# irenemizus/ArtStyleTransfer

Hardware: AMD Instinct MI355X
Metric: style-transfer iters/sec at L=2 (1024-px) (higher is better)
Workload: dtype f32 via f16x2 split (3 f16 MFMAs per product, f32 accumulate; the 14 large-channel conv launches of a closure as Winograd F(2,3) in that arithmetic); 1 GPU; pyramid style transfer, levels_num=3 (1536x1024+768x512+384x256), lbfgs as the reference constructs it (max_eval 1 under torch 2.10), content+noise init, seeded synthetic VGG19 weights, per-step image yield on; parallelism=1 GPU

## Files before the change

### artstyletransfer_amd/_lib.py

```python
from __future__ import annotations

import ctypes as C
import os
import subprocess
import threading

_HERE = os.path.dirname(os.path.abspath(__file__))
LIB_PATH = os.environ.get("NST_LIB") or os.path.join(_HERE, "libnst_hip.so")
CSRC = os.path.join(_HERE, "csrc")

NST_OK = 0
NST_E_ARG = -1
NST_E_STATE = -2
NST_E_UNAVAILABLE = -5
NST_VGG19_CONVS = 13
NST_MAX_LEVELS = 8
NST_LOSS_ROW = 4
NST_MAX_STYLES = 8
NST_OPT_ADAM = 0
NST_OPT_LBFGS = 1
NST_COLOR_RGB = 0
NST_COLOR_LUMINANCE = 1
NST_POOL_MAX = 0
NST_POOL_AVG = 1
NST_MAX_LAPLACIAN = 4
NST_MAX_FLOW_SCALES = 12
NST_MAX_ANCHOR_SOURCES = 8

c_float_p = C.POINTER(C.c_float)
REDUCE_HOOK = C.CFUNCTYPE(None, C.c_void_p)
c_void = C.c_void_p


NST_CONV_F32, NST_CONV_BF16X3, NST_CONV_F16X2 = 0, 1, 2
CONV_MODES = {"f32": NST_CONV_F32, "bf16x3": NST_CONV_BF16X3, "f16x2": NST_CONV_F16X2}
NST_COMM_ID_BYTES = 128


class StepInfo(C.Structure):
    _fields_ = [("closures", C.c_int), ("total_closures", C.c_int), ("accepted", C.c_int),
                ("loss", C.c_float), ("lr", C.c_float), ("t", C.c_float), ("history", C.c_int)]


class Options(C.Structure):
    _fields_ = [("struct_size", C.c_int), ("conv_mode", C.c_int), ("batched", C.c_int), ("single_stream", C.c_int),
                ("use_graph", C.c_int), ("h2_band_rows", C.c_int), ("lbfgs_gram", C.c_int), ("h2_mfma16", C.c_int),
                ("h2_wg256", C.c_int), ("h2_tile_rows", C.c_int), ("gram_overlap", C.c_int), ("h2_persist", C.c_int), ("level_split", C.c_int), ("h2_winograd", C.c_int)]


class LaunchInfo(C.Structure):
    _fields_ = [(n, C.c_int) for n in ("cls", "h", "w", "cin", "cout", "layer", "h2_rows", "h2_bn", "h2_ntw", "h2_chunk",
                                       "h2_mfma16", "h2_persist", "h2_second", "h2_unpool", "h2_bands")]


SYMBOLS = {
    "nst_version": (C.c_int, []),
    "nst_last_error": (C.c_char_p, [c_void]),
    "nst_device_count": (C.c_int, [C.POINTER(C.c_int)]),
    "nst_ctx_create": (C.c_int, [C.c_int, C.POINTER(c_void), C.POINTER(c_void), C.POINTER(c_void)]),
    "nst_options_default": (None, [C.POINTER(Options)]),
    "nst_ctx_create_ex": (C.c_int, [C.c_int, C.POINTER(c_void), C.POINTER(c_void), C.POINTER(Options), C.POINTER(c_void)]),
    "nst_ctx_destroy": (None, [c_void]),
    "nst_job_configure": (C.c_int, [c_void, C.c_int, C.c_int, C.c_int]),
    "nst_job_set_taps": (C.c_int, [c_void, C.c_int, C.c_uint, C.c_int]),
    "nst_job_set_color": (C.c_int, [c_void, C.c_int]),
    "nst_job_color": (C.c_int, [c_void]),
    "nst_job_set_pooling": (C.c_int, [c_void, C.c_int]),
    "nst_job_pooling": (C.c_int, [c_void]),
    "nst_job_set_laplacian": (C.c_int, [c_void, C.c_int, C.POINTER(C.c_int), c_float_p]),
    "nst_job_laplacian": (C.c_int, [c_void, C.POINTER(C.c_int), C.POINTER(C.c_int), c_float_p]),
    "nst_job_laplacian_losses": (C.c_int, [c_void, c_void, c_void]),
    "nst_laplacian_loss": (C.c_int, [c_void, c_void, c_void, C.c_int, C.c_int, C.c_int, C.c_int, c_void, c_void, c_void]),
    "nst_job_set_matting": (C.c_int, [c_void, C.c_float, C.c_double]),
    "nst_job_matting": (C.c_int, [c_void, c_float_p, C.POINTER(C.c_double)]),
    "nst_job_matting_losses": (C.c_int, [c_void, c_void, c_void]),
    "nst_matting_loss": (C.c_int, [c_void, c_void, c_void, C.c_int, C.c_int, C.c_int, C.c_double, c_void, c_void, c_void]),
    "nst_level_set_anchor": (C.c_int, [c_void, C.c_int, c_void, c_void, C.c_float, c_void]),
    "nst_level_anchor": (C.c_int, [c_void, C.c_int, c_float_p, C.POINTER(C.c_int)]),
    "nst_job_temporal_losses": (C.c_int, [c_void, c_void, c_void]),
    "nst_anchor_loss": (C.c_int, [c_void, c_void, c_void, c_void, C.c_int, C.c_int, C.c_int, c_void, c_void, c_void]),
    "nst_anchor_geometry": (C.c_int, [C.POINTER(C.c_int), C.POINTER(C.c_int)]),
    "nst_level_set_patches": (C.c_int, [c_void, C.c_int, c_void, C.c_int, C.c_int, c_float_p, C.c_int, C.c_double, c_void]),
    "nst_level_patches": (C.c_int, [c_void, C.c_int, c_float_p, C.POINTER(C.c_int), C.POINTER(C.c_double)]),
    "nst_job_patch_losses": (C.c_int, [c_void, c_void, c_void]),
    "nst_level_patch_matches": (C.c_int, [c_void, C.c_int, C.c_int, c_void, c_void]),
    "nst_patch_match": (C.c_int, [c_void, c_void, C.c_int, C.c_int, C.c_int, c_void, C.c_int, C.c_int, C.c_int, C.c_double, c_void,
                                  c_void, c_void]),
    "nst_patch_term": (C.c_int, [c_void, c_void, C.c_int, C.c_int, C.c_int, c_void, C.c_int, C.c_int, C.c_int, c_void, C.c_float,
                                 c_void, c_void, c_void]),
    "nst_warp_bilinear": (C.c_int, [c_void, c_void, c_void, C.c_int, C.c_int, C.c_int, c_void, c_void, c_void]),
    "nst_flow_weights": (C.c_int, [c_void, c_void, c_void, C.c_int, C.c_int, c_void, c_void]),
    "nst_anchor_fold": (C.c_int, [c_void, C.c_int, C.POINTER(c_void), C.POINTER(c_void), C.c_int, C.c_int, C.c_int, c_void, c_void,
                                  c_void, c_void]),
    "nst_flow_workspace": (C.c_int, [C.c_int, C.c_int, C.c_int, C.POINTER(C.c_size_t), C.POINTER(C.c_int)]),
    "nst_flow_estimate": (C.c_int, [c_void, c_void, c_void, C.c_int, C.c_int, C.c_float, C.c_int, C.c_int, C.c_int, c_void, c_void,
                                    C.c_size_t, c_void]),
    "nst_flow_reduce": (C.c_int, [c_void, c_void, C.c_int, C.c_int, c_void, c_void]),
    "nst_flow_prolong": (C.c_int, [c_void, c_void, C.c_int, C.c_int, c_void, c_void]),
    "nst_flow_linearize": (C.c_int, [c_void, c_void, c_void, c_void, C.c_int, C.c_int, c_void, c_void, c_void, c_void]),
    "nst_flow_sweeps": (C.c_int, [c_void, c_void, c_void, c_void, c_void, C.c_int, C.c_int, C.c_float, C.c_int, c_void, c_void,
                                  c_void]),
    "nst_flow_tvl1_workspace": (C.c_int, [C.c_int, C.c_int, C.c_int, C.POINTER(C.c_size_t), C.POINTER(C.c_int)]),
    "nst_flow_tvl1_estimate": (C.c_int, [c_void, c_void, c_void, C.c_int, C.c_int, C.c_float, C.c_float, C.c_float, C.c_int, C.c_int,
                                         C.c_int, c_void, c_void, C.c_size_t, c_void]),
    "nst_flow_tvl1_iterations": (C.c_int, [c_void, c_void, c_void, c_void, c_void, c_void, C.c_int, C.c_int, C.c_float, C.c_float,
                                           C.c_float, C.c_int, c_void, c_void, c_void, c_void]),
    "nst_job_set_gram_shift": (C.c_int, [c_void, c_float_p, C.c_uint]),
    "nst_job_gram_shift": (C.c_int, [c_void, c_float_p, C.POINTER(C.c_uint)]),
    "nst_level_gram_offsets": (C.c_int, [c_void, C.c_int, C.c_int, c_void, c_void]),
    "nst_gram_shifted": (C.c_int, [c_void, c_void, C.c_int, C.c_int, C.c_int, C.c_int, C.c_int, C.c_float, c_void, c_void, c_void]),
    "nst_job_set_moments": (C.c_int, [c_void, c_float_p, c_float_p, C.c_float]),
    "nst_job_moments": (C.c_int, [c_void, c_float_p, c_float_p, c_float_p]),
    "nst_job_moment_losses": (C.c_int, [c_void, c_void, c_void]),
    "nst_moments": (C.c_int, [c_void, c_void, C.c_int, C.c_int, C.c_int, C.c_float, c_void, c_void, c_void]),
    "nst_job_set_style_weights": (C.c_int, [c_void, c_float_p]),
    "nst_job_style_weights": (C.c_int, [c_void, c_float_p]),
    "nst_color_stats": (C.c_int, [c_void, c_void, C.c_int, C.c_int, C.POINTER(C.c_double), C.POINTER(C.c_double), c_void]),
    "nst_color_transfer_matrix": (C.c_int, [C.POINTER(C.c_double)] * 6),
    "nst_color_affine": (C.c_int, [c_void, c_void, C.c_int, C.c_int, C.POINTER(C.c_double), C.POINTER(C.c_double), c_void, c_void]),
    "nst_luminance": (C.c_int, [c_void, c_void, C.c_int, C.c_int, C.c_double, C.c_double, c_void, c_void]),
    "nst_luminance_recombine": (C.c_int, [c_void, c_void, c_void, C.c_int, C.c_int, c_void, c_void]),
    "nst_level_set_targets": (C.c_int, [c_void, C.c_int, c_void, c_void, C.c_int, C.c_int, c_void]),
    "nst_level_set_targets_blend": (C.c_int, [c_void, C.c_int, c_void, C.c_int, C.POINTER(c_void), C.POINTER(C.c_int),
                                              C.POINTER(C.c_int), c_float_p, c_void]),
    "nst_level_set_guidance": (C.c_int, [c_void, C.c_int, C.c_int, c_void, c_float_p, c_void]),
    "nst_level_set_targets_guided": (C.c_int, [c_void, C.c_int, c_void, c_void, C.c_int, C.c_int, c_void, c_void]),
    "nst_level_guidance": (C.c_int, [c_void, C.c_int, C.POINTER(C.c_int), c_float_p, C.POINTER(C.c_double)]),
    "nst_level_guidance_planes": (C.c_int, [c_void, C.c_int, C.c_int, c_void, c_void]),
    "nst_closure": (C.c_int, [c_void, c_void, C.c_float, C.c_float, C.c_float, c_void, c_void, c_void]),
    "nst_closure_levels": (C.c_int, [c_void, c_void, C.c_float, C.c_float, C.c_float, C.c_uint, c_void, c_void, c_void]),
    "nst_closure_forward": (C.c_int, [c_void, c_void, C.c_float, C.c_float, C.c_float, C.c_uint, c_void, c_void]),
    "nst_closure_backward": (C.c_int, [c_void, c_void, C.c_float, C.c_float, C.c_float, C.c_uint, c_void, c_void]),
    "nst_opt_shard_levels": (C.c_int, [c_void, C.c_uint, c_void, c_void, c_void, c_void]),
    "nst_opt_shard_levels_comm": (C.c_int, [c_void, C.c_uint, c_void]),
    "nst_opt_history": (C.c_int, [c_void, C.POINTER(C.c_int), C.POINTER(C.c_int)]),
    "nst_opt_set_closure_reuse": (C.c_int, [c_void, C.c_int]),
    "nst_opt_closure_stats": (C.c_int, [c_void, C.POINTER(C.c_long), C.POINTER(C.c_long)]),
    "nst_opt_set_lazy_backward": (C.c_int, [c_void, C.c_int]),
    "nst_opt_backward_stats": (C.c_int, [c_void, C.POINTER(C.c_long), C.POINTER(C.c_long)]),
    "nst_comm_unique_id": (C.c_int, [c_void]),
    "nst_comm_create": (C.c_int, [C.c_int, C.c_int, C.c_int, c_void, C.POINTER(c_void)]),
    "nst_comm_destroy": (None, [c_void]),
    "nst_comm_info": (C.c_int, [c_void, C.POINTER(C.c_int), C.POINTER(C.c_int), C.POINTER(C.c_long), C.POINTER(C.c_double)]),
    "nst_comm_allreduce_sum": (C.c_int, [c_void, c_void, C.c_size_t, c_void]),
    "nst_adam_step": (C.c_int, [c_void, c_void, c_void, c_void, c_void, C.c_size_t, C.c_int, C.c_double, c_void]),
    "nst_lbfgs_direction": (C.c_int, [c_void, c_void, C.POINTER(c_void), C.POINTER(c_void), C.POINTER(C.c_float), C.c_int,
                                      C.c_float, C.c_size_t, C.c_int, c_void, c_void]),
    "nst_opt_create": (C.c_int, [c_void, C.c_int, C.c_float, C.c_int, C.POINTER(c_void)]),
    "nst_opt_destroy": (None, [c_void]),
    "nst_opt_step": (C.c_int, [c_void, c_void, C.c_float, C.c_float, C.c_float, c_void, C.c_int,
                               C.POINTER(StepInfo), c_void]),
    "nst_vgg_features": (C.c_int, [c_void, c_void, C.c_int, C.c_int, C.POINTER(c_void), c_void]),
    "nst_vgg_features_backward": (C.c_int, [c_void, c_void, C.c_int, C.c_int, C.POINTER(c_void), c_void, c_void]),
    "nst_vgg_activations": (C.c_int, [c_void, c_void, C.c_int, C.c_int, C.POINTER(c_void), c_void]),
    "nst_level_activation": (C.c_int, [c_void, C.c_int, C.c_int, c_void, c_void]),
    "nst_job_map_stats": (C.c_int, [c_void, C.c_int, C.POINTER(C.c_uint)]),
    "nst_ctx_set_keep_all_maps": (C.c_int, [c_void, C.c_int]),
    "nst_ctx_keep_all_maps": (C.c_int, [c_void]),
    "nst_ctx_set_forward_pack": (C.c_int, [c_void, C.c_int]),
    "nst_ctx_forward_pack": (C.c_int, [c_void]),
    "nst_ctx_set_gram_pack": (C.c_int, [c_void, C.c_int]),
    "nst_ctx_gram_pack": (C.c_int, [c_void]),
    "nst_level_image": (C.c_int, [c_void, C.c_int, c_void, c_void]),
    "nst_gram": (C.c_int, [c_void, c_void, C.c_int, C.c_int, C.c_int, C.c_int, c_void, c_void]),
    "nst_guided_gram_backward": (C.c_int, [c_void, c_void, C.c_size_t, C.c_int, C.c_int, c_void, c_void, c_void, c_void, c_void,
                                            c_void, c_void]),
    "nst_total_variation": (C.c_int, [c_void, c_void, C.c_int, C.c_int, C.c_int, c_void, c_void, c_void]),
    "nst_bicubic_half": (C.c_int, [c_void, c_void, C.c_int, C.c_int, C.c_int, c_void, c_void]),
    "nst_bicubic_half_backward": (C.c_int, [c_void, c_void, C.c_int, C.c_int, C.c_int, c_void, c_void]),
    "nst_prepare_img": (C.c_int, [c_void, c_void, C.c_int, C.c_int, c_void, c_void]),
    "nst_unprepare_img": (C.c_int, [c_void, c_void, C.c_int, C.c_int, c_void, c_void]),
    "nst_resize_bicubic": (C.c_int, [c_void, c_void, C.c_int, C.c_int, C.c_int, c_void, C.c_int, C.c_int, c_void]),
    "nst_gather_rows": (C.c_int, [c_void, c_void, c_void, C.c_size_t, C.c_int, c_void, c_void]),
    "nst_gaussian_mask_accumulate": (C.c_int, [c_void, c_void, c_void, C.c_int, C.c_int, C.c_int, C.c_double, C.c_double,
                                               C.c_double, c_void]),
    "nst_noise_blend": (C.c_int, [c_void, c_void, c_void, C.c_int, C.c_int, C.c_int, C.c_double, c_void, c_void]),
    "nst_scale": (C.c_int, [c_void, c_void, C.c_float, C.c_size_t, c_void, c_void]),
    "nst_window_sums_count": (C.c_int, [C.POINTER(C.c_size_t)]),
    "nst_window_begin": (C.c_int, [c_void, c_void, C.c_int, C.c_int, C.c_int, c_void, c_void]),
    "nst_window_end": (C.c_int, [c_void, c_void, C.c_int, C.c_int, C.c_int, C.c_float, C.c_float, C.c_float, c_void, c_void,
                                 c_void, c_void]),
    "nst_conv_mode": (C.c_int, [c_void]),
    "nst_ctx_bytes": (C.c_int, [c_void, C.POINTER(C.c_size_t)]),
    "nst_set_timing": (C.c_int, [c_void, C.c_int]),
    "nst_last_closure_ms": (C.c_int, [c_void, C.POINTER(C.c_float)]),
    "nst_last_closure_class": (C.c_int, [c_void, C.c_int, C.POINTER(C.c_float), C.POINTER(C.c_int),
                                         C.POINTER(C.c_double)]),
    "nst_last_closure_launches": (C.c_int, [c_void, C.POINTER(LaunchInfo), C.c_int, C.POINTER(C.c_int)]),
    "nst_last_closure_schedule": (C.c_int, [c_void, C.POINTER(C.c_int), C.POINTER(C.c_int), C.POINTER(C.c_int)]),
    "nst_dump_last_closure": (C.c_int, [c_void]),
    "nst_timing_totals": (C.c_int, [c_void, C.c_int, C.POINTER(C.c_double), C.POINTER(C.c_long),
                                    C.POINTER(C.c_double), C.c_int]),
    "nst_timing_mfma_flops": (C.c_int, [c_void, C.c_int, C.POINTER(C.c_double)]),
}

_lib = None
_lock = threading.Lock()


class NstError(RuntimeError):
    pass


def build(force: bool = False) -> str:
    if force:
        subprocess.run(["make", "-C", CSRC, "clean"], check=True, stdout=subprocess.DEVNULL)
    subprocess.run(["make", "-C", CSRC, "-j8"], check=True)
    return LIB_PATH


def load():
    global _lib
    with _lock:
        if _lib is not None:
            return _lib
        if not os.path.exists(LIB_PATH):
            raise NstError(
                f"{LIB_PATH} is missing: the HIP extension is the only implementation of the style-transfer "
                f"hot path (no CPU fallback). Build it with `python -c 'import __graft_entry__ as g; g.build()'` "
                f"or `make -C {CSRC}`.")
        try:
            lib = C.CDLL(LIB_PATH)
        except OSError as e:
            raise NstError(f"cannot load {LIB_PATH}: {e}") from e
        for name, (res, args) in SYMBOLS.items():
            try:
                fn = getattr(lib, name)
            except AttributeError as e:
                raise NstError(f"{LIB_PATH} does not export {name}; rebuild it") from e
            fn.restype = res
            fn.argtypes = args
        _lib = lib
        return lib


def check(ctx, code: int, what: str) -> None:
    if code != NST_OK:
        msg = load().nst_last_error(ctx)
        raise NstError(f"{what} failed ({code}): {msg.decode() if msg else '?'}")
```

### artstyletransfer_amd/csrc/conv_h2.hip

```cpp
#include <hip/hip_runtime.h>

#include <cstdlib>
#include <type_traits>

#include "nst_kernels.h"

namespace nst {

typedef float f32x4 __attribute__((ext_vector_type(4)));
typedef float f32x2 __attribute__((ext_vector_type(2)));
typedef float f32x16 __attribute__((ext_vector_type(16)));
typedef unsigned int u32x2 __attribute__((ext_vector_type(2)));
typedef unsigned int u32x4 __attribute__((ext_vector_type(4)));
typedef _Float16 f16x2 __attribute__((ext_vector_type(2)));
typedef _Float16 f16x8 __attribute__((ext_vector_type(8)));

namespace {

#ifndef NST_H2_DEEP_WEIGHT_PREFETCH
#define NST_H2_DEEP_WEIGHT_PREFETCH 1
#endif
#ifndef NST_H2_WEIGHT_SETS4
#define NST_H2_WEIGHT_SETS4 1
#endif
#ifndef NST_H2_ABLATE
#define NST_H2_ABLATE 0
#endif
constexpr unsigned ABL_IN = (NST_H2_ABLATE & 1) ? 0u : 1u, ABL_W = (NST_H2_ABLATE & 2) ? 0u : 1u, ABL_ST = (NST_H2_ABLATE & 4) ? 0u : 1u,
                   ABL_EL = (NST_H2_ABLATE & 8) ? 0u : 1u, ABL_G = (NST_H2_ABLATE & 16) ? 0u : 1u;
constexpr float LO_UP = 2048.f;
constexpr float LO_DOWN = 1.f / 2048.f;

template <int TH, int BN, int NTW, int KC_>
struct H2Cfg {
    static constexpr int KC = KC_;
    static constexpr int KS = KC / 16;
    static constexpr int QP = KC / 4;
    static constexpr int PIECEB = KC * 2;
    static constexpr int ROWB = 2 * PIECEB + 16;
    static constexpr int WROWB = 2 * PIECEB;
    static constexpr int TW = 16;
    static constexpr int PH = TH + 2, PW = TW + 2;
    static constexpr int WM = TH / 4;
    static constexpr int WN = BN / (32 * NTW);
    static constexpr int NT = 64 * WM * WN;
    static constexpr int A_UNITS = PH * PW * QP;
    static constexpr int A_PER_T = (A_UNITS + NT - 1) / NT;
    static constexpr int B_UNITS = BN * QP;
    static constexpr int B_PER_T = (B_UNITS + NT - 1) / NT;
    static constexpr int PROWB = ((PW * ROWB + 255) / 256) * 256;
    static constexpr int A_BYTES = PH * PROWB;
    static constexpr int B_BYTES = BN * ROWB;
    static constexpr int LDS_BYTES = 2 * A_BYTES + 3 * B_BYTES;
    static_assert(KC == 16 || KC == 32, "one or two k-steps per stage");
    static_assert(NT == 512 || NT == 256, "eight or four waves per workgroup");
    static_assert(B_UNITS % NT == 0, "every lane stages the same number of weight units (no predication)");
    static_assert(LDS_BYTES <= ((NT == 512 || TH == 4 || NTW == 4) ? 160 : 80) * 1024, "LDS budget (two 256-thread workgroups share a CU)");
    static constexpr int WAVES_PER_EU = (NTW == 4) ? 1 : 2;
};

__device__ __forceinline__ void tensor_scale(const unsigned* __restrict__ slots, int lane, float& s, float& inv) {
    unsigned m = slots[lane];
#pragma unroll
    for (int off = 32; off > 0; off >>= 1) {
        const unsigned o = (unsigned)__shfl_xor((int)m, off);
        m = o > m ? o : m;
    }
    int e = (int)((m >> 23) & 0xFFu);
    e = e < 32 ? 32 : (e > 250 ? 250 : e);
    s = __uint_as_float((unsigned)(268 - e) << 23);
    inv = __uint_as_float((unsigned)(e - 14) << 23);
}

__device__ __forceinline__ void cut2x4(const f32x4 v, const float s, u32x2& hi, u32x2& lo) {
    const f32x2 x01 = {v[0] * s, v[1] * s}, x23 = {v[2] * s, v[3] * s};
    const f16x2 h01 = __builtin_convertvector(x01, f16x2), h23 = __builtin_convertvector(x23, f16x2);
    const f32x2 b01 = __builtin_convertvector(h01, f32x2), b23 = __builtin_convertvector(h23, f32x2);
    const f32x2 r01 = (x01 - b01) * LO_UP, r23 = (x23 - b23) * LO_UP;
    const f16x2 l01 = __builtin_convertvector(r01, f16x2), l23 = __builtin_convertvector(r23, f16x2);
    hi = u32x2{__builtin_bit_cast(unsigned, h01), __builtin_bit_cast(unsigned, h23)};
    lo = u32x2{__builtin_bit_cast(unsigned, l01), __builtin_bit_cast(unsigned, l23)};
}

}

template <int TH, int BN, int NTW, int KC, bool UNPOOL, bool M16, class Tiles>
__device__ __forceinline__ void conv_h2_body(const Tiles& tiles, const int slot_seed) {
    static_assert(!M16 || KC == 32, "the 16x16x32 form takes a whole 32-channel chunk per MFMA");
    using C = H2Cfg<TH, BN, NTW, KC>;
    constexpr int ROWB = C::ROWB, WROWB = C::WROWB, QP = C::QP, PIECEB = C::PIECEB, KS = C::KS;
    extern __shared__ __attribute__((aligned(16))) unsigned char smem[];
    unsigned char* ldsB = smem;
    unsigned char* ldsA = smem + 3 * C::B_BYTES;

    const int tid = threadIdx.x;
    const int lane = tid & 63;
    const int wave = tid >> 6;
    const int wm = wave % C::WM;
    const int wn = wave / C::WM;
    const int half = lane >> 5;
    const int l31 = lane & 31;

    u32x4 rb[C::B_PER_T];
    constexpr bool DEEPB = (KC == 16) && NST_H2_DEEP_WEIGHT_PREFETCH;
    u32x4 rb2[DEEPB ? C::B_PER_T : 1];
    constexpr bool DEEPB4 = DEEPB && C::B_PER_T == 1 && NST_H2_WEIGHT_SETS4;
    u32x4 rb3[DEEPB4 ? C::B_PER_T : 1], rb4[DEEPB4 ? C::B_PER_T : 1];

    ConvParams p;
    int sp = 0, ct = 0;
    (void)tiles.get(0, p, sp, ct);
    bool primed = false;
  for (int tile_k = 0;; ++tile_k) {
    const int ty_rel = sp / p.tiles_x;
    const int tx = sp - ty_rel * p.tiles_x;
    const int ty = ty_rel + p.ty0;
    const int y0 = ty * TH;
    const int x0 = tx * C::TW;
    const int n0 = ct * BN;
    auto opaque_s = [](int v) { asm volatile("" : "+s"(v)); return v; };
    float nx_sa = 1.f;
    bool chain = false;
    {
        ConvParams pn;
        int spn = 0, ctn = 0;
        if (tiles.get(tile_k + 1, pn, spn, ctn) && p.Cin > 0 && !p.in2 && !pn.in2) {
            chain = true;
            float unused_inv;
            tensor_scale(pn.amax_in, lane, nx_sa, unused_inv);
        }
    }

    f32x4 ra[C::A_PER_T];

    auto a_lds_of = [&](int i, int to) -> int {
        const int u = to + i * C::NT;
        const int pix = u / QP;
        const int pr = pix / C::PW;
        const int pc = pix - pr * C::PW;
        return (u < C::A_UNITS) ? pr * C::PROWB + pc * ROWB + (u % QP) * 8 : -1;
    };
    auto a_voff_of = [&](int i, int to, int cin, const bool pooled, const int gH, const int gW, const int gy0, const int gx0) -> unsigned {
        const int u = to + i * C::NT;
        const int pix = u / QP;
        const int pr = pix / C::PW;
        const int pc = pix - pr * C::PW;
        const int gy = gy0 - 1 + pr;
        const int gx = gx0 - 1 + pc;
        bool ok = (u < C::A_UNITS) & ((unsigned)gy < (unsigned)gH) & ((unsigned)gx < (unsigned)gW);
        if (!pooled) return ok ? ((unsigned)(gy * gW + gx) * (unsigned)cin + (unsigned)(u % QP) * 4u) * 4u : 0xFFFFFF00u;
        const int PH2 = gH >> 1, PW2 = gW >> 1;
        ok = ok & ((gy >> 1) < PH2) & ((gx >> 1) < PW2);
        return ok ? ((unsigned)((gy >> 1) * PW2 + (gx >> 1)) * (unsigned)cin + (unsigned)(u % QP) * 4u) * 4u : 0xFFFFFF00u;
    };
    auto a_coff_of = [&](int i, int to, int cin, const int gH, const int gW, const int gy0, const int gx0) -> unsigned {
        const int u = to + i * C::NT;
        const int pix = u / QP;
        const int pr = pix / C::PW;
        const int pc = pix - pr * C::PW;
        const int gy = gy0 - 1 + pr;
        const int gx = gx0 - 1 + pc;
        const int PH2 = gH >> 1, PW2 = gW >> 1;
        const bool ok = (u < C::A_UNITS) & ((unsigned)gy < (unsigned)gH) & ((unsigned)gx < (unsigned)gW) &
                        ((gy >> 1) < PH2) & ((gx >> 1) < PW2);
        return ok ? (((unsigned)((gy >> 1) * PW2 + (gx >> 1)) * (unsigned)(cin >> 5)) * 4u + (unsigned)((gy & 1) * 2 + (gx & 1))) * 4u : 0xFFFFFF00u;
    };
    auto b_ok = [&](int, int) -> bool { return true; };
    auto b_lds_of = [&](int i, int to) -> int { const int u = to + i * C::NT; return (u / QP) * ROWB + (u % QP) * 16; };

    auto store_a = [&](unsigned char* dstA, const float s, const f32x4* r, const int i0, const int i1, const int to,
                       const unsigned* code = nullptr, const int bit0 = 0) {
#pragma unroll
        for (int i = i0; i < i1; ++i) {
            const int off = a_lds_of(i, to);
            if (off >= 0) {
                u32x2 hi, lo;
                f32x4 v = r[i - i0];
                if (code) {
                    const unsigned bits = code[i - i0] >> (bit0 + ((to + i * C::NT) % QP) * 4);
#pragma unroll
                    for (int k = 0; k < 4; ++k) v[k] = ((bits >> k) & 1u) ? v[k] : 0.f;
                }
                cut2x4(v, s, hi, lo);
                unsigned char* row = dstA + off;
                *reinterpret_cast<u32x2*>(row) = hi;
                *reinterpret_cast<u32x2*>(row + PIECEB) = lo;
            }
        }
    };
    auto store_b = [&](unsigned char* dst, const u32x4 (&r)[C::B_PER_T], const int to) {
#pragma unroll
        for (int i = 0; i < C::B_PER_T; ++i)
            if (b_ok(i, to)) *reinterpret_cast<u32x4*>(dst + b_lds_of(i, to)) = r[i];
    };
    auto store_b_f32 = [&](unsigned char* dst, const float s, const int to) {
#pragma unroll
        for (int i = 0; i < C::B_PER_T; ++i)
            if (b_ok(i, to)) {
                u32x2 hi, lo;
                cut2x4(__builtin_bit_cast(f32x4, rb[i]), s, hi, lo);
                const int u = to + i * C::NT;
                unsigned char* row = dst + (u / QP) * ROWB + (u % QP) * 8;
                *reinterpret_cast<u32x2*>(row) = hi;
                *reinterpret_cast<u32x2*>(row + PIECEB) = lo;
            }
    };
    auto opaque = [](int v) { asm volatile("" : "+v"(v)); return v; };

    f32x16 accm[2][NTW], accx[2][NTW];
#pragma unroll
    for (int a = 0; a < 2; ++a)
#pragma unroll
        for (int b = 0; b < NTW; ++b)
#pragma unroll
            for (int r = 0; r < 16; ++r) { accm[a][b][r] = 0.f; accx[a][b][r] = 0.f; }

    const int prow = wm * 4 + (l31 >> 4);
    const int pcol = l31 & 15;
    const int a_off0 = (prow + 0) * C::PROWB + pcol * ROWB + half * 16;
    const int a_off1 = (prow + 2) * C::PROWB + pcol * ROWB + half * 16;
    const int b_off0 = (wn * 32 * NTW + l31) * ROWB + half * 16;

    struct Frags { f16x8 a[2][2]; f16x8 b[NTW][2]; };
    auto request = [&](Frags& f, const unsigned char* abase, const unsigned char* bbase, const int ks) {
#pragma unroll
        for (int s = 0; s < 2; ++s) {
            f.a[0][s] = *reinterpret_cast<const f16x8*>(abase + a_off0 + s * PIECEB + ks * 32);
            f.a[1][s] = *reinterpret_cast<const f16x8*>(abase + a_off1 + s * PIECEB + ks * 32);
#pragma unroll
            for (int nt = 0; nt < NTW; ++nt)
                f.b[nt][s] = *reinterpret_cast<const f16x8*>(bbase + b_off0 + nt * 32 * ROWB + s * PIECEB + ks * 32);
        }
    };
    auto multiply = [&](const Frags& f) {
#pragma unroll
        for (int mt = 0; mt < 2; ++mt)
#pragma unroll
            for (int nt = 0; nt < NTW; ++nt) {
                accx[mt][nt] = __builtin_amdgcn_mfma_f32_32x32x16_f16(f.a[mt][1], f.b[nt][0], accx[mt][nt], 0, 0, 0);
                accm[mt][nt] = __builtin_amdgcn_mfma_f32_32x32x16_f16(f.a[mt][0], f.b[nt][0], accm[mt][nt], 0, 0, 0);
                accx[mt][nt] = __builtin_amdgcn_mfma_f32_32x32x16_f16(f.a[mt][0], f.b[nt][1], accx[mt][nt], 0, 0, 0);
            }
    };
    constexpr int READS = 4 + 2 * NTW, MFMAS = 6 * NTW;
    auto pin_kstep = [&]() {
#pragma unroll
// ... 40 lines not shown
#pragma unroll
                for (int j = 0; j < 2; ++j)
                    ax16[2 * mp + i][2 * np + j] = __builtin_amdgcn_mfma_f32_16x16x32_f16(a.v[i][1], b.v[j][0], ax16[2 * mp + i][2 * np + j], 0, 0, 0);
#pragma unroll
            for (int i = 0; i < 2; ++i)
#pragma unroll
                for (int j = 0; j < 2; ++j)
                    am16[2 * mp + i][2 * np + j] = __builtin_amdgcn_mfma_f32_16x16x32_f16(a.v[i][0], b.v[j][0], am16[2 * mp + i][2 * np + j], 0, 0, 0);
#pragma unroll
            for (int i = 0; i < 2; ++i)
#pragma unroll
                for (int j = 0; j < 2; ++j)
                    ax16[2 * mp + i][2 * np + j] = __builtin_amdgcn_mfma_f32_16x16x32_f16(a.v[i][0], b.v[j][1], ax16[2 * mp + i][2 * np + j], 0, 0, 0);
        }
    };
    auto pin_quad = [&](const int reads) {
        if (reads == 4) {
#pragma unroll
            for (int g = 0; g < 4; ++g) {
                __builtin_amdgcn_sched_group_barrier(0x008, 3, 0);
                __builtin_amdgcn_sched_group_barrier(0x100, 1, 0);
            }
        } else {
#pragma unroll
            for (int g = 0; g < 8; ++g) {
                __builtin_amdgcn_sched_group_barrier(0x008, 1, 0);
                __builtin_amdgcn_sched_group_barrier(0x100, 1, 0);
            }
            __builtin_amdgcn_sched_group_barrier(0x008, 4, 0);
        }
    };
    Pair RA[2], RB[2];

    auto gram_source = [&](const float* src, const int cin, const float* wts, const float sa, const float sw) {
        const int nch = cin / KC;
        const __amdgpu_buffer_rsrc_t rsrc_in = __builtin_amdgcn_make_buffer_rsrc(
            const_cast<float*>(src), 0, (unsigned)((size_t)p.H * p.W * cin * 4) * ABL_G, 0x00020000);
        const __amdgpu_buffer_rsrc_t rsrc_w = __builtin_amdgcn_make_buffer_rsrc(
            const_cast<float*>(wts), 0, (unsigned)((size_t)p.Cout * cin * 4) * ABL_G, 0x00020000);
        constexpr int G_PER_T = TH * C::TW * QP / C::NT;
        static_assert(TH * C::TW * QP % C::NT == 0 && G_PER_T <= C::A_PER_T, "centre units divide evenly");
        unsigned a_voff[G_PER_T], b_voff[C::B_PER_T];
        int g_lds[G_PER_T];
#pragma unroll
        for (int i = 0; i < G_PER_T; ++i) {
            const int u = tid + i * C::NT;
            const int pix = u / QP, q = u % QP;
            const int py = pix >> 4, px = pix & 15;
            const int gy = y0 + py, gx = x0 + px;
            bool ok = (gy < p.H) & (gx < p.W);
            if (p.in2_rows > 0) ok = ok & ((unsigned)(gy - p.in2_row0) < (unsigned)p.in2_rows);
            a_voff[i] = ok ? ((unsigned)(gy * p.W + gx) * (unsigned)cin + (unsigned)q * 4u) * 4u : 0xFFFFFF00u;
            g_lds[i] = (py + 1) * C::PROWB + (px + 1) * ROWB + q * 8;
        }
#pragma unroll
        for (int i = 0; i < C::B_PER_T; ++i) {
            const int u = tid + i * C::NT;
            b_voff[i] = b_ok(i, tid) ? (unsigned)(((u / QP) * cin + (u % QP) * 4) * 4) : 0xFFFFFF00u;
        }
        auto load = [&](int chunk) {
#pragma unroll
            for (int i = 0; i < G_PER_T; ++i)
                ra[i] = __builtin_bit_cast(f32x4, __builtin_amdgcn_raw_buffer_load_b128(rsrc_in, a_voff[i], chunk * KC * 4, 0));
#pragma unroll
            for (int i = 0; i < C::B_PER_T; ++i)
                rb[i] = __builtin_amdgcn_raw_buffer_load_b128(rsrc_w, b_voff[i], (n0 * cin + chunk * KC) * 4, 0);
        };
        auto store_centre = [&](unsigned char* dstA) {
#pragma unroll
            for (int i = 0; i < G_PER_T; ++i) {
                u32x2 hi, lo;
                cut2x4(ra[i], sa, hi, lo);
                unsigned char* row = dstA + g_lds[i];
                *reinterpret_cast<u32x2*>(row) = hi;
                *reinterpret_cast<u32x2*>(row + PIECEB) = lo;
            }
        };
        load(0);
        store_centre(ldsA);
        store_b_f32(ldsB, sw, tid);
        if (nch > 1) load(1);
        __syncthreads();
        for (int c = 0; c < nch; ++c) {
            const int cb = c & 1;
            if (c + 1 < nch) {
                store_centre(ldsA + (cb ^ 1) * C::A_BYTES);
                store_b_f32(ldsB + (cb ^ 1) * C::B_BYTES, sw, tid);
                if (c + 2 < nch) load(c + 2);
            }
            const unsigned char* centre = ldsA + cb * C::A_BYTES + C::PROWB + ROWB;
            const unsigned char* bcur = ldsB + cb * C::B_BYTES;
            if constexpr (M16) {
                read_a(RA[0], centre, 0);
                read_a(RA[1], centre, 1);
#pragma unroll
                for (int np = 0; np < NP; ++np) {
                    read_b(RB[0], bcur, np);
                    quad(RA[0], RB[0], 0, np);
                    quad(RA[1], RB[0], 1, np);
                }
            } else {
#pragma unroll
                for (int ks = 0; ks < KS; ++ks) request(F[ks], centre, bcur, ks);
#pragma unroll
                for (int ks = 0; ks < KS; ++ks) multiply(F[ks]);
            }
            __syncthreads();
        }
    };

    auto main_source = [&](const float* src, const int cin, const void* wts, const float sa) {
        const int nch = cin / KC;
        const size_t in_px = UNPOOL ? (size_t)(p.H >> 1) * (p.W >> 1) : (size_t)p.H * p.W;
        const __amdgpu_buffer_rsrc_t rsrc_in = __builtin_amdgcn_make_buffer_rsrc(
            const_cast<float*>(src), 0, (unsigned)(in_px * cin * 4) * ABL_IN, 0x00020000);
        const __amdgpu_buffer_rsrc_t rsrc_w = __builtin_amdgcn_make_buffer_rsrc(
            const_cast<void*>(wts), 0, (unsigned)((size_t)9 * p.Cout * nch * WROWB) * ABL_W, 0x00020000);
        const __amdgpu_buffer_rsrc_t rsrc_code = __builtin_amdgcn_make_buffer_rsrc(
            const_cast<unsigned*>(UNPOOL ? p.pcode_in : nullptr), 0, UNPOOL ? (unsigned)(in_px * (cin >> 5) * 16) : 0u, 0x00020000);
        struct Look { __amdgpu_buffer_rsrc_t rs_in, rs_code; int H, W, y0, x0, n0; float sa; };
        const Look here{rsrc_in, rsrc_code, p.H, p.W, y0, x0, n0, sa};
        auto there = [&]() -> Look {
            ConvParams pn;
            int spn = 0, ctn = 0;
            (void)tiles.get(opaque_s(tile_k + 1), pn, spn, ctn);
            const size_t px = UNPOOL ? (size_t)(pn.H >> 1) * (pn.W >> 1) : (size_t)pn.H * pn.W;
            const int tyn = spn / pn.tiles_x;
            return Look{__builtin_amdgcn_make_buffer_rsrc(const_cast<float*>(pn.in), 0, (unsigned)(px * cin * 4), 0x00020000),
                        __builtin_amdgcn_make_buffer_rsrc(const_cast<unsigned*>(UNPOOL ? pn.pcode_in : nullptr), 0,
                                                          UNPOOL ? (unsigned)(px * (cin >> 5) * 16) : 0u, 0x00020000),
                        pn.H, pn.W, (tyn + pn.ty0) * TH, (spn - tyn * pn.tiles_x) * C::TW, ctn * BN, nx_sa};
        };
        unsigned rc[UNPOOL ? C::A_PER_T : 1];
        auto load_a = [&](f32x4* r, const Look& k, int chunk, const int i0, const int i1, const int to) {
#pragma unroll
            for (int i = i0; i < i1; ++i) {
                r[i - i0] = __builtin_bit_cast(f32x4, __builtin_amdgcn_raw_buffer_load_b128(
                                                          k.rs_in, a_voff_of(i, to, cin, UNPOOL, k.H, k.W, k.y0, k.x0), chunk * KC * 4, 0));
                if (UNPOOL)
                    rc[i - i0] = __builtin_amdgcn_raw_buffer_load_b32(k.rs_code, a_coff_of(i, to, cin, k.H, k.W, k.y0, k.x0), ((chunk * KC) >> 5) * 16, 0);
            }
        };
        auto bit0_of = [&](int chunk) { return (chunk * KC) & 31; };
        auto load_b = [&](u32x4 (&r)[C::B_PER_T], int chunk, int tap, const int to, const int cout0) {
            const int soff = ((tap * p.Cout + cout0) * nch + chunk) * WROWB;
#pragma unroll
            for (int i = 0; i < C::B_PER_T; ++i) {
                const int u = to + i * C::NT;
                const unsigned voff = b_ok(i, to) ? (unsigned)((u / QP) * nch * WROWB + (u % QP) * 16) : 0xFFFFFF00u;
                r[i] = __builtin_amdgcn_raw_buffer_load_b128(rsrc_w, voff, soff, 0);
            }
        };
        auto tap_off = [](int t) { return (t / 3) * C::PROWB + (t % 3) * ROWB; };

        if (!primed) {
            u32x4 r0[C::B_PER_T], r1[C::B_PER_T];
            load_a(ra, here, 0, 0, C::A_PER_T, tid);
            load_b(r0, 0, 0, tid, n0);
            load_b(r1, 0, 1, tid, n0);
            load_b(rb, 0, 2, tid, n0);
            if constexpr (DEEPB) load_b(rb2, 0, 3, tid, n0);
            if constexpr (DEEPB4) { load_b(rb3, 0, 4, tid, n0); load_b(rb4, 0, 5, tid, n0); }
            __syncthreads();
            store_a(ldsA, sa, ra, 0, C::A_PER_T, tid, UNPOOL ? rc : nullptr, bit0_of(0));
            store_b(ldsB, r0, tid);
            store_b(ldsB + C::B_BYTES, r1, tid);
            __syncthreads();
        }
        if constexpr (M16) {
            read_a(RA[0], ldsA + tap_off(0), 0);
            read_b(RB[0], ldsB, 0);
        } else {
            request(F[0], ldsA + tap_off(0), ldsB, 0);
        }
        if (C::NT == 512 && __builtin_amdgcn_readfirstlane(threadIdx.x) >= 256) __builtin_amdgcn_s_setprio(1);

        auto chunk = [&](const int c, auto par_c) {
            constexpr int PAR = decltype(par_c)::value;
            unsigned char* acur = ldsA + (c & 1) * C::A_BYTES;
            unsigned char* anext = ldsA + ((c + 1) & 1) * C::A_BYTES;
            const bool last = (c + 1 >= nch);
            const int cn = last ? (chain ? 0 : c) : c + 1;
            Look ahead = here;
            if (last && chain) ahead = there();
            const int to = opaque(tid);
#ifndef NST_H2_THIRDS_ALL
#define NST_H2_THIRDS_ALL 0
#endif
            constexpr int PARTS = ((NST_H2_THIRDS_ALL || (M16 && NTW == 2)) && C::A_PER_T % 3 == 0) ? 3 : 2;
            constexpr int AP = (C::A_PER_T + PARTS - 1) / PARTS;
            auto part_lo = [](int j) { return j * AP < C::A_PER_T ? j * AP : C::A_PER_T; };
#pragma unroll
            for (int t = 0; t < 9; ++t) {
                if constexpr (DEEPB4) {
                    store_b(ldsB + ((t + 2) % 3) * C::B_BYTES, rb, to);
#pragma unroll
                    for (int i = 0; i < C::B_PER_T; ++i) { rb[i] = rb2[i]; rb2[i] = rb3[i]; rb3[i] = rb4[i]; }
                    if (t + 6 < 9) load_b(rb4, c, t + 6, to, n0);
                    else load_b(rb4, cn, t + 6 - 9, to, ahead.n0);
                } else if constexpr (DEEPB) {
                    if (((PAR + t) & 1) == 0) {
                        store_b(ldsB + ((t + 2) % 3) * C::B_BYTES, rb, to);
                        if (t + 4 < 9) load_b(rb, c, t + 4, to, n0);
                        else load_b(rb, cn, t + 4 - 9, to, ahead.n0);
                    } else {
                        store_b(ldsB + ((t + 2) % 3) * C::B_BYTES, rb2, to);
                        if (t + 4 < 9) load_b(rb2, c, t + 4, to, n0);
                        else load_b(rb2, cn, t + 4 - 9, to, ahead.n0);
                    }
                } else {
                    store_b(ldsB + ((t + 2) % 3) * C::B_BYTES, rb, to);
                    if (t + 3 < 9) load_b(rb, c, t + 3, to, n0);
                    else load_b(rb, cn, t + 3 - 9, to, ahead.n0);
                }
                if constexpr (PARTS == 2) {
                    if (t == 0) load_a(ra, ahead, cn, 0, AP, to);
                    if (t == 4) load_a(ra, ahead, cn, AP, C::A_PER_T, to);
                } else {
                    if (t % 3 == 0) load_a(ra, ahead, cn, part_lo(t / 3), part_lo(t / 3 + 1), to);
                }
                __builtin_amdgcn_sched_barrier(0);
                if constexpr (PARTS == 2) {
                    if (t == 3) store_a(anext, ahead.sa, ra, 0, AP, to, UNPOOL ? rc : nullptr, bit0_of(cn));
                    if (t == 7) store_a(anext, ahead.sa, ra, AP, C::A_PER_T, to, UNPOOL ? rc : nullptr, bit0_of(cn));
                } else {
                    if (t % 3 == 2) store_a(anext, ahead.sa, ra, part_lo(t / 3), part_lo(t / 3 + 1), to, UNPOOL ? rc : nullptr, bit0_of(cn));
                }
                const unsigned char* bcur = ldsB + (t % 3) * C::B_BYTES;
                const unsigned char* anxt = (t + 1 < 9) ? acur + tap_off(t + 1) : anext + tap_off(0);
                const unsigned char* bnxt = ldsB + ((t + 1) % 3) * C::B_BYTES;
                if constexpr (M16) {
                    const unsigned char* aptr = acur + tap_off(t);
                    const int sp_ = (PAR + t) & 1;
                    if (NP == 2) {
                        const int b0 = sp_, b1 = sp_ ^ 1;
                        read_b(RB[b1], bcur, b1);
                        quad(RA[0], RB[b0], 0, b0);
                        pin_quad(4);
                        read_a(RA[1], aptr, 1);
                        quad(RA[0], RB[b1], 0, b1);
                        pin_quad(4);
                        read_a(RA[0], anxt, 0);
                        quad(RA[1], RB[b1], 1, b1);
                        pin_quad(4);
                        read_b(RB[b1], bnxt, b1);
                        quad(RA[1], RB[b0], 1, b0);
                        pin_quad(4);
                    } else {
                        read_a(RA[1], aptr, 1);
                        quad(RA[0], RB[sp_], 0, 0);
                        pin_quad(4);
                        read_a(RA[0], anxt, 0);
                        read_b(RB[sp_ ^ 1], bnxt, 0);
                        quad(RA[1], RB[sp_], 1, 0);
                        pin_quad(8);
                    }
                } else if (KS == 2) {
                    request(F[1], acur + tap_off(t), bcur, 1);
                    multiply(F[0]);
                    pin_kstep();
                    request(F[0], anxt, bnxt, 0);
                    multiply(F[1]);
                    pin_kstep();
                } else {
                    const int cur = (PAR + t) & 1;
                    request(F[cur ^ 1], anxt, bnxt, 0);
                    multiply(F[cur]);
                    pin_kstep();
                }
                __syncthreads();
            }
        };
        if (KS == 2 && !M16) {
            for (int c = 0; c < nch; ++c) chunk(c, std::integral_constant<int, 0>{});
        } else {
            for (int c = 0; c < nch; c += 2) {
                chunk(c, std::integral_constant<int, 0>{});
                chunk(c + 1, std::integral_constant<int, 1>{});
            }
        }
    };

    const bool has_main = p.Cin > 0;
    float sa1 = 1.f, ia1 = 1.f;
    if (has_main) tensor_scale(p.amax_in, lane, sa1, ia1);
    const float w1_inv = has_main ? p.wt_h2_inv : 1.f;
    const float inv = ia1 * w1_inv;
    if (p.in2) {
        float sa2, ia2, sw2, iw2;
        tensor_scale(p.amax_in2, lane, sa2, ia2);
        tensor_scale(p.amax_w2, lane, sw2, iw2);
        gram_source(p.in2, p.Cin2, p.wt2_f32, sa2, sw2);
        const float ratio = (ia2 * sa1) * (iw2 * (1.f / w1_inv));
        if constexpr (M16) {
#pragma unroll
            for (int a = 0; a < 4; ++a)
#pragma unroll
                for (int b = 0; b < NT16; ++b)
#pragma unroll
                    for (int r = 0; r < 4; ++r) { am16[a][b][r] *= ratio; ax16[a][b][r] *= ratio; }
        } else {
#pragma unroll
            for (int a = 0; a < 2; ++a)
#pragma unroll
                for (int b = 0; b < NTW; ++b)
#pragma unroll
                    for (int r = 0; r < 16; ++r) { accm[a][b][r] *= ratio; accx[a][b][r] *= ratio; }
        }
    }
    if (has_main) main_source(p.in, p.Cin, p.wt_h2, sa1);

    auto epilogue = [&, &p_loop = p]() {
    ConvParams p;
    {
        int sp_again, ct_again;
        if (Tiles::REFETCH) (void)tiles.get(opaque_s(tile_k), p, sp_again, ct_again);
        else p = p_loop;
    }
    const int words = p.Cout >> 5;
    const bool avg = p.pool_avg != 0;
    float amax = 0.f;
    auto record_amax = [&]() {
        if (p.amax_out) {
#pragma unroll
            for (int off = 32; off > 0; off >>= 1) amax = fmaxf(amax, __shfl_xor(amax, off));
            if (lane == 0) atomicMax(p.amax_out + ((slot_seed * (C::NT / 64) + wave) & (NST_AMAX_SLOTS - 1)), __float_as_uint(amax));
        }
    };

    if constexpr (M16) {
        const int cg0 = n0 + wn * 32 * NTW;
        const float lo_clamp = p.relu ? 0.f : -__builtin_inff();
        auto word_of = [&](const unsigned long long b_even, const unsigned long long b_odd) -> unsigned {
            return (unsigned)((b_even >> (16 * kg)) & 0xFFFFull) | ((unsigned)((b_odd >> (16 * kg)) & 0xFFFFull) << 16);
        };
        const bool interior = (y0 + TH <= p.H) && (x0 + C::TW <= p.W);
        const bool fwd_like = !p.bits_in && !p.addend;
        const bool bwd_like = p.bits_in && !p.bits_out && !p.pool_out && !p.pcode_out;
        if (interior && !p.mask && (fwd_like || bwd_like) && (size_t)p.H * p.W * p.Cout * 4 < 0xFFFFFF00ull) {
            const unsigned out_bytes = (unsigned)((size_t)p.H * p.W * p.Cout * 4);
            const unsigned bit_bytes = (unsigned)((size_t)p.H * p.W * words * 4);
            const int colB = p.Cout * 4, rowB = p.W * colB;
            const int wcolB = words * 4, wrowB = p.W * wcolB;
            const int pix0 = (y0 + wm * 4) * p.W + x0 + 4 * kg;
            const unsigned vbase = (unsigned)pix0 * (unsigned)colB + (unsigned)(cg0 + l15) * 4u;
            const unsigned wbase = (unsigned)pix0 * (unsigned)wcolB + (unsigned)(cg0 >> 5) * 4u;
            const __amdgpu_buffer_rsrc_t rs_out = __builtin_amdgcn_make_buffer_rsrc(p.out, 0, out_bytes * ABL_ST, 0x00020000);
            if (bwd_like) {
                const __amdgpu_buffer_rsrc_t rs_bits = __builtin_amdgcn_make_buffer_rsrc(const_cast<unsigned*>(p.bits_in), 0, bit_bytes * ABL_EL, 0x00020000);
                const __amdgpu_buffer_rsrc_t rs_add = __builtin_amdgcn_make_buffer_rsrc(const_cast<float*>(p.addend), 0, p.addend ? out_bytes * ABL_EL : 0u, 0x00020000);
                unsigned wv[4][4][NTW];
#pragma unroll
                for (int mt = 0; mt < 4; ++mt)
#pragma unroll
                    for (int i = 0; i < 4; ++i) {
                        if (NTW == 2) {
                            const u32x2 w2 = __builtin_bit_cast(u32x2, __builtin_amdgcn_raw_buffer_load_b64(rs_bits, wbase, mt * wrowB + i * wcolB, 0));
                            wv[mt][i][0] = w2[0];
                            wv[mt][i][NTW - 1] = w2[1];
                        } else {
                            wv[mt][i][0] = __builtin_amdgcn_raw_buffer_load_b32(rs_bits, wbase, mt * wrowB + i * wcolB, 0);
                        }
                    }
#pragma unroll
                for (int nt = 0; nt < NT16; ++nt) {
                    const float bv = p.bias ? p.bias[cg0 + nt * 16 + l15] : 0.f;
#pragma unroll
                    for (int mt = 0; mt < 4; ++mt) {
                        float ad[4] = {0.f, 0.f, 0.f, 0.f};
                        if (p.addend) {
#pragma unroll
                            for (int i = 0; i < 4; ++i)
                                ad[i] = __builtin_bit_cast(float, __builtin_amdgcn_raw_buffer_load_b32(rs_add, vbase, mt * rowB + i * colB + nt * 64, 0));
                        }
#pragma unroll
                        for (int i = 0; i < 4; ++i) {
                            float v = fmaf(ax16[mt][nt][i], LO_DOWN, am16[mt][nt][i]) * inv + bv;
                            v = fmaxf(v + ad[i], lo_clamp);
                            v = ((wv[mt][i][nt >> 1] >> ((nt & 1) * 16 + l15)) & 1u) ? v : 0.f;
                            __builtin_amdgcn_raw_buffer_store_b32(__builtin_bit_cast(unsigned, v), rs_out, vbase, mt * rowB + i * colB + nt * 64, 0);
                            amax = fmaxf(amax, fabsf(v));
                        }
                    }
                }
            } else {
                const int PW2 = p.W >> 1;
                const unsigned pool_bytes = (unsigned)((size_t)(p.H >> 1) * PW2 * p.Cout * 4);
                const __amdgpu_buffer_rsrc_t rs_bits = __builtin_amdgcn_make_buffer_rsrc(p.bits_out, 0, p.bits_out ? bit_bytes * ABL_ST : 0u, 0x00020000);
                const __amdgpu_buffer_rsrc_t rs_pool = __builtin_amdgcn_make_buffer_rsrc(p.pool_out, 0, p.pool_out ? pool_bytes * ABL_ST : 0u, 0x00020000);
                const __amdgpu_buffer_rsrc_t rs_code = __builtin_amdgcn_make_buffer_rsrc(
                    p.pcode_out, 0, p.pcode_out ? (unsigned)((size_t)(p.H >> 1) * PW2 * words * 16) * ABL_ST : 0u, 0x00020000);
                const unsigned wlane = (l15 == 0) ? wbase : 0xFFFFFF00u;
                const int ppix0 = ((y0 + wm * 4) >> 1) * PW2 + ((x0 + 4 * kg) >> 1);
                const unsigned pbase = (unsigned)ppix0 * (unsigned)colB + (unsigned)(cg0 + l15) * 4u;
                const unsigned cbase = (l15 == 0) ? ((unsigned)ppix0 * (unsigned)words + (unsigned)(cg0 >> 5)) * 16u : 0xFFFFFF00u;
                const bool full = UNPOOL || p.out != nullptr;
#pragma unroll
                for (int nt = 0; nt < NT16; ++nt) {
                    const float bv = p.bias ? p.bias[cg0 + nt * 16 + l15] : 0.f;
#pragma unroll
                    for (int mt = 0; mt < 4; ++mt)
#pragma unroll
                        for (int i = 0; i < 4; ++i) {
                            float v = fmaf(ax16[mt][nt][i], LO_DOWN, am16[mt][nt][i]) * inv + bv;
                            v = fmaxf(v, lo_clamp);
                            am16[mt][nt][i] = v;
                            if (full) __builtin_amdgcn_raw_buffer_store_b32(__builtin_bit_cast(unsigned, v), rs_out, vbase, mt * rowB + i * colB + nt * 64, 0);
                            amax = fmaxf(amax, fabsf(v));
                        }
                }
                if (p.bits_out) {
#pragma unroll
                    for (int mt = 0; mt < 4; ++mt)
#pragma unroll
                        for (int i = 0; i < 4; ++i)
#pragma unroll
                            for (int w = 0; w < NTW; ++w) {
                                const unsigned long long b0 = __ballot(am16[mt][2 * w][i] > 0.f), b1 = __ballot(am16[mt][2 * w + 1][i] > 0.f);
                                __builtin_amdgcn_raw_buffer_store_b32(word_of(b0, b1), rs_bits, wlane, mt * wrowB + i * wcolB + w * 4, 0);
                            }
                }
                if (p.pool_out) {
#pragma unroll
                    for (int mt = 0; mt < 4; mt += 2)
#pragma unroll
                        for (int i = 0; i < 4; i += 2) {
                            const int poff = (mt >> 1) * PW2 + (i >> 1);
                            unsigned long long code[NTW][4][2];
#pragma unroll
                            for (int nt = 0; nt < NT16; ++nt) {
                                const float e0 = am16[mt][nt][i], e1 = am16[mt][nt][i + 1], e2 = am16[mt + 1][nt][i], e3 = am16[mt + 1][nt][i + 1];
                                const float mx = avg ? (((e0 + e1) + e2) + e3) * 0.25f : fmaxf(fmaxf(e0, e1), fmaxf(e2, e3));
                                __builtin_amdgcn_raw_buffer_store_b32(__builtin_bit_cast(unsigned, mx), rs_pool, pbase, poff * colB + nt * 64, 0);
                                if (p.pcode_out) {
                                    if (avg) {
                                        code[nt >> 1][0][nt & 1] = __ballot(e0 > 0.f);
                                        code[nt >> 1][1][nt & 1] = __ballot(e1 > 0.f);
                                        code[nt >> 1][2][nt & 1] = __ballot(e2 > 0.f);
                                        code[nt >> 1][3][nt & 1] = __ballot(e3 > 0.f);
                                    } else {
                                        int pos = 0;
// ... 206 lines not shown
                        accm[mt][nt][r] = v;
                        if (full) __builtin_amdgcn_raw_buffer_store_b32(__builtin_bit_cast(unsigned, v), rs_out, vbase, soff(mt, r, rowB, colB) + nt * 128, 0);
                        amax = fmaxf(amax, fabsf(v));
                        if (p.bits_out) {
                            const unsigned long long bal = __ballot(v > 0.f);
                            __builtin_amdgcn_raw_buffer_store_b32(half ? (unsigned)(bal >> 32) : (unsigned)bal, rs_bits, wlane,
                                                                  soff(mt, r, wrowB, wcolB) + nt * 4, 0);
                        }
                    }
                    if (p.pool_out) {
#pragma unroll
                        for (int j = 0; j < 4; ++j) {
                            const int r = 2 * j;
                            const int pcol = (j & 1) + 4 * (j >> 1);
                            const float mx = avg ? (((accm[mt][nt][r] + accm[mt][nt][r + 1]) + accm[mt][nt][r + 8]) + accm[mt][nt][r + 9]) * 0.25f
                                                 : fmaxf(fmaxf(accm[mt][nt][r], accm[mt][nt][r + 1]),
                                                         fmaxf(accm[mt][nt][r + 8], accm[mt][nt][r + 9]));
                            __builtin_amdgcn_raw_buffer_store_b32(__builtin_bit_cast(unsigned, mx), rs_pool, pbase,
                                                                  (mt * PW2 + pcol) * colB + nt * 128, 0);
                            if (p.pcode_out) {
                                int pos = 0;
                                float best = accm[mt][nt][r];
                                if (accm[mt][nt][r + 1] > best) { best = accm[mt][nt][r + 1]; pos = 1; }
                                if (accm[mt][nt][r + 8] > best) { best = accm[mt][nt][r + 8]; pos = 2; }
                                if (accm[mt][nt][r + 9] > best) { best = accm[mt][nt][r + 9]; pos = 3; }
                                const bool live = best > 0.f;
                                constexpr int roff[4] = {0, 1, 8, 9};
#pragma unroll
                                for (int q = 0; q < 4; ++q) {
                                    const unsigned long long bal = __ballot(avg ? accm[mt][nt][r + roff[q]] > 0.f : (live && pos == q));
                                    __builtin_amdgcn_raw_buffer_store_b32(half ? (unsigned)(bal >> 32) : (unsigned)bal, rs_code, cbase,
                                                                          ((mt * PW2 + pcol) * words + nt) * 16 + q * 4, 0);
                                }
                            }
                        }
                    }
                }
            }
        }
        record_amax();
        return;
    }

#pragma unroll
    for (int nt = 0; nt < NTW; ++nt) {
        const int co = n0 + wn * 32 * NTW + nt * 32 + l31;
        const int cw = (n0 + wn * 32 * NTW + nt * 32) >> 5;
        const float bv = p.bias ? p.bias[co] : 0.f;
#pragma unroll
        for (int mt = 0; mt < 2; ++mt) {
#pragma unroll
            for (int r = 0; r < 16; ++r) {
                const int m = (r & 3) + 8 * (r >> 2) + 4 * half;
                const int y = y0 + wm * 4 + mt * 2 + (m >> 4);
                const int x = x0 + (m & 15);
                const bool inb = (y < p.H && x < p.W);
                const size_t pix = (size_t)y * p.W + x;
                const size_t idx = pix * p.Cout + co;
                float v = fmaf(accx[mt][nt][r], LO_DOWN, accm[mt][nt][r]) * inv + bv;
                if (p.addend && inb) v += p.addend[idx];
                if (p.relu) v = fmaxf(v, 0.f);
                if (p.bits_in) {
                    const unsigned wv = inb ? p.bits_in[pix * words + cw] : 0u;
                    v = ((wv >> l31) & 1u) ? v : 0.f;
                } else if (p.mask) {
                    v = (inb && p.mask[idx] > 0.f) ? v : 0.f;
                }
                if (p.bits_out) {
                    const unsigned long long bal = __ballot(v > 0.f);
                    if (l31 == 0 && inb) p.bits_out[pix * words + cw] = half ? (unsigned)(bal >> 32) : (unsigned)bal;
                }
                accm[mt][nt][r] = v;
                if (inb) {
                    if (UNPOOL || p.out) p.out[idx] = v;
                    amax = fmaxf(amax, fabsf(v));
                }
            }
            if (p.pool_out) {
                const int py = (y0 + wm * 4 + mt * 2) >> 1;
                const int PH2 = p.H >> 1, PW2 = p.W >> 1;
#pragma unroll
                for (int j = 0; j < 4; ++j) {
                    const int r = 2 * j;
                    const float mx = avg ? (((accm[mt][nt][r] + accm[mt][nt][r + 1]) + accm[mt][nt][r + 8]) + accm[mt][nt][r + 9]) * 0.25f
                                         : fmaxf(fmaxf(accm[mt][nt][r], accm[mt][nt][r + 1]),
                                                 fmaxf(accm[mt][nt][r + 8], accm[mt][nt][r + 9]));
                    const int mcol = (r & 3) + 8 * (r >> 2) + 4 * half;
                    const int px = (x0 + mcol) >> 1;
                    const bool inw = (py < PH2 && px < PW2);
                    if (inw) p.pool_out[((size_t)py * PW2 + px) * p.Cout + co] = mx;
                    if (p.pcode_out) {
                        int pos = 0;
                        float best = accm[mt][nt][r];
                        if (accm[mt][nt][r + 1] > best) { best = accm[mt][nt][r + 1]; pos = 1; }
                        if (accm[mt][nt][r + 8] > best) { best = accm[mt][nt][r + 8]; pos = 2; }
                        if (accm[mt][nt][r + 9] > best) { best = accm[mt][nt][r + 9]; pos = 3; }
                        const bool live = best > 0.f;
                        constexpr int roff[4] = {0, 1, 8, 9};
#pragma unroll
                        for (int q = 0; q < 4; ++q) {
                            const unsigned long long bal = __ballot(avg ? accm[mt][nt][r + roff[q]] > 0.f : (live && pos == q));
                            if (l31 == 0 && inw)
                                p.pcode_out[(((size_t)py * PW2 + px) * words + cw) * 4 + q] = half ? (unsigned)(bal >> 32) : (unsigned)bal;
                        }
                    }
                }
            }
        }
    }
    record_amax();
    };
    epilogue();
    if (!tiles.get(tile_k + 1, p, sp, ct)) break;
    primed = chain;
  }
}

__device__ __forceinline__ int xcd_contiguous(const int b, const int grid) {
#ifdef NST_NO_XCD_MAP
    return b;
#else
    const int x = b & 7, k = b >> 3;
    const int q = grid >> 3, r = grid & 7;
    return x * q + (x < r ? x : r) + k;
#endif
}

template <bool PERSIST>
struct H2BatchTiles {
    static constexpr bool REFETCH = PERSIST;
    const ConvBatch& b;
    int n_ct;
    __device__ __forceinline__ bool get(const int k, ConvParams& p, int& sp, int& ct) const {
        int t;
        if (!PERSIST) {
            if (k > 0) return false;
            t = xcd_contiguous((int)blockIdx.x, (int)gridDim.x);
        } else {
            const int x = (int)blockIdx.x & 7, j = ((int)blockIdx.x >> 3) + k * ((int)gridDim.x >> 3);
            const int q = b.total_tiles >> 3, r = b.total_tiles & 7;
            if (j >= q + (x < r ? 1 : 0)) return false;
            t = x * q + (x < r ? x : r) + j;
        }
        const int sp_all = t / n_ct;
        ct = t - sp_all * n_ct;
        int i = 0;
        while (i + 1 < b.n && sp_all >= b.img[i].tile_end) ++i;
        const ConvImage& im = b.img[i];
        p.in = im.in; p.wt = nullptr; p.wt_bf = nullptr; p.bias = im.bias ? im.bias : b.bias; p.addend = im.addend; p.mask = im.mask; p.out = im.out;
        p.H = im.H; p.W = im.W; p.Cin = b.Cin; p.Cout = b.Cout; p.relu = b.relu;
        p.tiles_x = im.tiles_x; p.tiles_y = 0; p.partial = nullptr; p.partial_floats = 0; p.ksplit = 1;
        p.in2 = im.in2; p.Cin2 = b.Cin2; p.wt2_bf = nullptr; p.bits_out = im.bits_out; p.bits_in = im.bits_in;
        p.pool_out = im.pool_out;
        p.wt_h2 = b.wt_h2; p.wt_h2_inv = b.wt_h2_inv; p.wt2_f32 = im.wt2_f32;
        p.amax_in = im.amax_in; p.amax_in2 = im.amax_in2; p.amax_w2 = im.amax_w2; p.amax_out = im.amax_out;
        p.pcode_in = im.pcode_in; p.pcode_out = im.pcode_out; p.pool_avg = b.pool_avg;
        p.in2_row0 = im.in2_row0; p.in2_rows = im.in2_rows; p.ty0 = im.ty0;
        sp = sp_all - (i ? b.img[i - 1].tile_end : 0);
        return true;
    }
};

template <int TH, int BN, int NTW, int KC, bool UNPOOL, bool M16, bool PERSIST>
__global__ __launch_bounds__((H2Cfg<TH, BN, NTW, KC>::NT), (H2Cfg<TH, BN, NTW, KC>::WAVES_PER_EU)) void conv_h2_batch_kernel(ConvBatch b) {
    conv_h2_body<TH, BN, NTW, KC, UNPOOL, M16>(H2BatchTiles<PERSIST>{b, b.Cout / BN}, blockIdx.x);
}
template <int TH, int BN, int NTW, int KC>
constexpr bool h2_persist_shape = (KC == 16) || (TH == 16 && NTW == 2 && KC == 32);
template <int NTW, int KC>
constexpr bool h2_m16_built = (KC == 32 && NTW <= 2);

template <int TH, int BN, int NTW, int KC, bool UNPOOL, bool M16>
static hipError_t init_form() {
    constexpr int lds = H2Cfg<TH, BN, NTW, KC>::LDS_BYTES;
    hipError_t e = hipFuncSetAttribute(reinterpret_cast<const void*>(&conv_h2_batch_kernel<TH, BN, NTW, KC, UNPOOL, M16, false>),
                                       hipFuncAttributeMaxDynamicSharedMemorySize, lds);
    if constexpr (h2_persist_shape<TH, BN, NTW, KC> && !M16) {
        if (e == hipSuccess)
            e = hipFuncSetAttribute(reinterpret_cast<const void*>(&conv_h2_batch_kernel<TH, BN, NTW, KC, UNPOOL, false, true>),
                                    hipFuncAttributeMaxDynamicSharedMemorySize, lds);
    }
    return e;
}
template <int TH, int BN, int NTW, int KC, bool UNPOOL>
static hipError_t init_one() {
    hipError_t e = init_form<TH, BN, NTW, KC, UNPOOL, false>();
    if constexpr (h2_m16_built<NTW, KC>) {
        if (e == hipSuccess) e = init_form<TH, BN, NTW, KC, UNPOOL, true>();
    }
    return e;
}

hipError_t conv_h2_init_device() {
    hipError_t e = init_one<16, 128, 2, 32, false>();
    if (e == hipSuccess) e = init_one<8, 128, 1, 32, false>();
    if (e == hipSuccess) e = init_one<16, 64, 2, 16, false>();
    if (e == hipSuccess) e = init_one<16, 128, 2, 32, true>();
    if (e == hipSuccess) e = init_one<8, 128, 1, 32, true>();
    if (e == hipSuccess) e = init_one<16, 64, 2, 16, true>();
    if (e == hipSuccess) e = init_one<8, 128, 2, 16, false>();
    if (e == hipSuccess) e = init_one<8, 128, 2, 16, true>();
    if (e == hipSuccess) e = init_one<4, 128, 1, 32, false>();
    if (e == hipSuccess) e = init_one<4, 128, 1, 32, true>();
    if (e == hipSuccess) e = init_one<16, 128, 4, 32, false>();
    if (e == hipSuccess) e = init_one<16, 128, 4, 32, true>();
    return e;
}

static int h2_tile_rows(int Cout, long blocks16, int forced = 0) {
    if (Cout % 128 != 0) return 16;
    if (forced == 4 || forced == 8 || forced == 16) return forced;
    if (blocks16 < 100) return 4;
    return blocks16 < 400 ? 8 : 16;
}

static bool h2_use_m16(int mfma16, int th, int ntw, bool unpool) {
    if (mfma16 >= 3) return true;
    if (mfma16 == 2) return th == 8 || (th == 16 && ntw == 2 && !unpool);
    return mfma16 == 1 && th == 8;
}
static int h2_resident(const H2Shape& sh) { return 256 * ((sh.chunk == 16 || sh.rows == 4) ? 2 : 1); }

static H2Shape h2_launch_shape(const int* H, const int* W, int n, int Cin, int Cout, bool unpool, bool second, int tile_rows,
                               int mfma16, int wg256, int persist_opt, int* blocks) {
    H2Shape sh{};
    const bool wide = (Cout % 128 == 0);
    long blocks16 = 0;
    for (int i = 0; i < n; ++i) blocks16 += (long)((H[i] + 15) / 16) * ((W[i] + 15) / 16) * (Cout / 128);
    const bool shortk = wide && Cin > 0 && Cin <= NST_H2_SHORTK_CIN;
    sh.rows = shortk ? 8 : h2_tile_rows(Cout, blocks16, tile_rows);
    sh.bn = wide ? 128 : 64;
    sh.chunk = (!wide || shortk) ? 16 : 32;
    sh.ntw = (sh.chunk == 16) ? 2 : (sh.rows < 16 ? 1 : (wg256 ? 4 : 2));
    sh.m16 = (sh.chunk == 32 && sh.ntw <= 2 && h2_use_m16(mfma16, sh.rows, sh.ntw, unpool)) ? 1 : 0;
    sh.second = second ? 1 : 0;
    sh.unpool = unpool ? 1 : 0;
    sh.bands = 1;
    int tiles = 0;
    for (int i = 0; i < n; ++i) tiles += ((W[i] + 15) / 16) * ((H[i] + sh.rows - 1) / sh.rows);
    *blocks = tiles * (Cout / sh.bn);
    const bool pshape = sh.chunk == 16 || (sh.rows == 16 && sh.ntw == 2);
    sh.persist = (persist_opt && !second && Cin > 0 && *blocks > h2_resident(sh) && pshape && !sh.m16) ? 1 : 0;
    return sh;
}

template <int TH, int BN, int NTW, int KC>
static void launch_batch_cfg(const ConvBatch& b, const H2Shape& sh, int blocks, hipStream_t stream) {
    constexpr int lds = H2Cfg<TH, BN, NTW, KC>::LDS_BYTES;
    constexpr int nt = H2Cfg<TH, BN, NTW, KC>::NT;
    if constexpr (h2_m16_built<NTW, KC>) {
        if (sh.m16) {
            if (b.unpool) hipLaunchKernelGGL((conv_h2_batch_kernel<TH, BN, NTW, KC, true, true, false>), dim3(blocks), dim3(nt), lds, stream, b);
            else hipLaunchKernelGGL((conv_h2_batch_kernel<TH, BN, NTW, KC, false, true, false>), dim3(blocks), dim3(nt), lds, stream, b);
            return;
        }
    }
    if constexpr (h2_persist_shape<TH, BN, NTW, KC>) {
        if (sh.persist) {
            if (b.unpool) hipLaunchKernelGGL((conv_h2_batch_kernel<TH, BN, NTW, KC, true, false, true>), dim3(blocks), dim3(nt), lds, stream, b);
            else hipLaunchKernelGGL((conv_h2_batch_kernel<TH, BN, NTW, KC, false, false, true>), dim3(blocks), dim3(nt), lds, stream, b);
            return;
        }
    }
    if (b.unpool) hipLaunchKernelGGL((conv_h2_batch_kernel<TH, BN, NTW, KC, true, false, false>), dim3(blocks), dim3(nt), lds, stream, b);
    else hipLaunchKernelGGL((conv_h2_batch_kernel<TH, BN, NTW, KC, false, false, false>), dim3(blocks), dim3(nt), lds, stream, b);
}
static bool h2_operands_ok(const void* wt, const unsigned* amax_in, int Cin, int Cout, const float* in2, const float* wt2,
                           const unsigned* a2, const unsigned* w2, int Cin2) {
    if (Cin % 32 != 0 || Cout % 64 != 0) return false;
    if (Cin > 0 ? (!wt || !amax_in) : !in2) return false;
    if (in2 && (!wt2 || !a2 || !w2 || Cin2 % 32 != 0 || Cin2 != Cout)) return false;
    return true;
}

template <int TH, int BN, int NTW, int KC>
struct H2Tag { static constexpr int th = TH, bn = BN, ntw = NTW, kc = KC; };
template <typename Launch>
static void h2_dispatch(const H2Shape& sh, Launch&& go) {
    if (sh.bn == 64) go(H2Tag<16, 64, 2, 16>{});
    else if (sh.chunk == 16) go(H2Tag<8, 128, 2, 16>{});
    else if (sh.rows == 4) go(H2Tag<4, 128, 1, 32>{});
    else if (sh.rows == 8) go(H2Tag<8, 128, 1, 32>{});
    else if (sh.ntw == 4) go(H2Tag<16, 128, 4, 32>{});
    else go(H2Tag<16, 128, 2, 32>{});
}

hipError_t launch_conv_h2_batch(const ConvBatch& b0, hipStream_t stream, H2Shape* shape) {
    if (b0.n < 1 || b0.n > 8) return hipErrorInvalidValue;
    ConvBatch b = b0;
    int H[8], W[8];
    bool second = false;
    for (int i = 0; i < b.n; ++i) {
        const ConvImage& im = b.img[i];
        if (!h2_operands_ok(b.wt_h2, im.amax_in, b.Cin, b.Cout, im.in2, im.wt2_f32, im.amax_in2, im.amax_w2, b.Cin2))
            return hipErrorInvalidValue;
        if ((size_t)im.H * im.W * (b.Cin > b.Cin2 ? b.Cin : b.Cin2) * 4 >= 0xFFFFFF00ull) return hipErrorInvalidValue;
        if ((b.unpool != 0) != (im.pcode_in != nullptr)) return hipErrorInvalidValue;
        if (!im.out && !im.pool_out) return hipErrorInvalidValue;
        H[i] = im.H; W[i] = im.W;
        second = second || (im.in2 != nullptr);
    }
    int blocks = 0;
    const H2Shape sh = h2_launch_shape(H, W, b.n, b.Cin, b.Cout, b.unpool != 0, second, b.tile_rows, b.mfma16, b.wg256, b.persist, &blocks);
    int tiles = 0;
    for (int i = 0; i < b.n; ++i) {
        b.img[i].tiles_x = (b.img[i].W + 15) / 16;
        b.img[i].ty0 = 0;
        tiles += b.img[i].tiles_x * ((b.img[i].H + sh.rows - 1) / sh.rows);
        b.img[i].tile_end = tiles;
    }
    b.total_tiles = blocks;
    b.persist = sh.persist;
    if (sh.persist) blocks = h2_resident(sh);
    if (shape) *shape = sh;
    h2_dispatch(sh, [&](auto cfg) { launch_batch_cfg<decltype(cfg)::th, decltype(cfg)::bn, decltype(cfg)::ntw, decltype(cfg)::kc>(b, sh, blocks, stream); });
    return hipGetLastError();
}

hipError_t launch_conv_h2(const ConvParams& p, hipStream_t stream, H2Shape* shape) {
    if (!h2_operands_ok(p.wt_h2, p.amax_in, p.Cin, p.Cout, p.in2, p.wt2_f32, p.amax_in2, p.amax_w2, p.Cin2))
        return hipErrorInvalidValue;
    if (!p.out && !p.pool_out) return hipErrorInvalidValue;
    int all_blocks = 0;
    H2Shape sh = h2_launch_shape(&p.H, &p.W, 1, p.Cin, p.Cout, p.pcode_in != nullptr, p.in2 != nullptr, p.tile_rows, p.mfma16, p.wg256, 0, &all_blocks);
    const int th = sh.rows;
    const int cmax = p.Cin > p.Cout ? (p.Cin > p.Cin2 ? p.Cin : p.Cin2) : (p.Cout > p.Cin2 ? p.Cout : p.Cin2);
    const size_t row_bytes = (size_t)p.W * cmax * 4;
    int band_rows = p.H;
    if ((size_t)p.H * row_bytes >= 0xFFFFFF00ull) {
        const long fit = (long)(0xFFFFFF00ull / row_bytes) - 32;
        band_rows = (int)(fit / 16) * 16;
        if (band_rows < 16) return hipErrorInvalidValue;
    }
    const int forced_band = p.band_rows;
    if (forced_band >= 16 && forced_band / 16 * 16 < band_rows) band_rows = forced_band / 16 * 16;
    const int PW2 = p.W >> 1, wi = p.Cin >> 5, wo = p.Cout >> 5;
    ConvBatch b{};
    b.n = 1;
    b.bias = p.bias;
    b.Cin = p.Cin; b.Cout = p.Cout; b.Cin2 = p.Cin2; b.relu = p.relu;
    b.wt_h2 = p.wt_h2; b.wt_h2_inv = p.wt_h2_inv;
    b.unpool = (p.pcode_in != nullptr);
    b.persist = 0;
    b.pool_avg = p.pool_avg;
    int bands = 0;
    for (int r0 = 0; r0 < p.H; r0 += band_rows) {
        const int r1 = (r0 + band_rows < p.H) ? r0 + band_rows : p.H;
        const int b0 = (r0 >= 16) ? r0 - 16 : 0, b1 = (r1 + 16 < p.H) ? r1 + 16 : p.H;
        const size_t px0 = (size_t)b0 * p.W, pp0 = (size_t)(b0 >> 1) * PW2;
        ConvImage& q = b.img[0];
        q = ConvImage{};
        if (p.pcode_in) { q.in = p.in + pp0 * p.Cin; q.pcode_in = p.pcode_in + pp0 * wi * 4; }
        else if (p.in) q.in = p.in + px0 * p.Cin;
        q.in2_row0 = p.in2_row0; q.in2_rows = p.in2_rows;
        if (p.in2) { q.in2 = p.in2 + px0 * p.Cin2; if (q.in2_rows > 0) q.in2_row0 -= b0; }
        if (p.out) q.out = p.out + px0 * p.Cout;
        if (p.addend) q.addend = p.addend + px0 * p.Cout;
        if (p.mask) q.mask = p.mask + px0 * p.Cout;
        if (p.bits_in) q.bits_in = p.bits_in + px0 * wo;
        if (p.bits_out) q.bits_out = p.bits_out + px0 * wo;
        if (p.pool_out) q.pool_out = p.pool_out + pp0 * p.Cout;
        if (p.pcode_out) q.pcode_out = p.pcode_out + pp0 * wo * 4;
        q.wt2_f32 = p.wt2_f32;
        q.amax_in = p.amax_in; q.amax_in2 = p.amax_in2; q.amax_w2 = p.amax_w2; q.amax_out = p.amax_out;
        q.H = b1 - b0; q.W = p.W;
        q.ty0 = (r0 - b0) / th;
        const int tiles_y = (r1 - r0 + th - 1) / th;
        q.tiles_x = (p.W + 15) / 16;
        q.tile_end = q.tiles_x * tiles_y;
        const int blocks = q.tile_end * (p.Cout / sh.bn);
        b.total_tiles = blocks;
        h2_dispatch(sh, [&](auto cfg) { launch_batch_cfg<decltype(cfg)::th, decltype(cfg)::bn, decltype(cfg)::ntw, decltype(cfg)::kc>(b, sh, blocks, stream); });
        const hipError_t e = hipGetLastError();
        if (e != hipSuccess) return e;
        ++bands;
    }
    sh.bands = bands;
    if (shape) *shape = sh;
    return hipSuccess;
}

__global__ __launch_bounds__(256) void absmax_slots_kernel(const float* __restrict__ x, size_t n, unsigned* __restrict__ slots) {
    float m = 0.f;
    const size_t n4 = n / 4;
    for (size_t i = (size_t)blockIdx.x * blockDim.x + threadIdx.x; i < n4; i += (size_t)gridDim.x * blockDim.x) {
        const f32x4 v = reinterpret_cast<const f32x4*>(x)[i];
        m = fmaxf(fmaxf(m, fmaxf(fabsf(v[0]), fabsf(v[1]))), fmaxf(fabsf(v[2]), fabsf(v[3])));
    }
    if (blockIdx.x == 0 && threadIdx.x < (n & 3)) m = fmaxf(m, fabsf(x[n4 * 4 + threadIdx.x]));
#pragma unroll
    for (int off = 32; off > 0; off >>= 1) m = fmaxf(m, __shfl_xor(m, off));
    if ((threadIdx.x & 63) == 0)
        atomicMax(slots + ((blockIdx.x * 4 + (threadIdx.x >> 6)) & (NST_AMAX_SLOTS - 1)), __float_as_uint(m));
}
hipError_t launch_absmax_slots(const float* x, size_t n, unsigned* slots, hipStream_t stream) {
    size_t blocks = (n / 4 + 255) / 256;
    if (blocks > 1024) blocks = 1024;
    if (blocks < 1) blocks = 1;
    hipLaunchKernelGGL(absmax_slots_kernel, dim3((unsigned)blocks), dim3(256), 0, stream, x, n, slots);
    return hipGetLastError();
}

}
```

### artstyletransfer_amd/csrc/nst_closure.cpp

```cpp
#include <algorithm>
#include <cmath>
#include <cstring>

#include "nst_ctx.h"

using namespace nst;

namespace {

double conv_flops(int h, int w, int cin, int cout, int taps) { return 2.0 * h * w * (double)cin * cout * taps; }

bool uses_pieces(const nst_ctx* ctx, const ConvParams& p) {
    if (ctx->conv_mode == 2) return true;
    return ctx->conv_mode != 0 && (size_t)p.H * p.W * p.Cin * 4 < 0xFFFFFF00ull;
}
hipError_t launch_conv3(nst_ctx* ctx, const ConvParams& p, Timer& t) {
    hipStream_t s = t.s;
    if (uses_pieces(ctx, p)) {
        if (ctx->conv_mode != 2) return launch_conv_bf3(p, s);
        H2Shape sh{};
        const hipError_t e = launch_conv_h2(p, s, &sh);
        t.shape(sh);
        return e;
    }
    hipError_t e = launch_conv_mfma(p, 9, s);
    if (e == hipSuccess && ctx->conv_mode == 2 && p.amax_out)
        e = launch_absmax_slots(p.out, (size_t)p.H * p.W * p.Cout, p.amax_out, s);
    return e;
}
bool bf3_unsplit(const nst_ctx* ctx, const ConvParams& p) {
    if (!uses_pieces(ctx, p)) return false;
    if (ctx->conv_mode == 2) return true;
    const int S = conv_bf3_ksplit(p.H, p.W, p.Cin, p.Cout);
    return !(p.partial && S > 1 && (size_t)S * p.H * p.W * p.Cout <= p.partial_floats);
}

void conv_setup(const nst_ctx* ctx, ConvParams& p, const ActSet& a, int l, bool dgrad) {
    p.wt = dgrad ? ctx->wd[l] : ctx->wf[l]; p.wt_bf = dgrad ? ctx->wd_bf[l] : ctx->wf_bf[l];
    p.partial = a.splitk; p.partial_floats = a.splitk_floats;
    if (ctx->conv_mode != 2) return;
    p.wt_h2 = dgrad ? ctx->wd_h2[l] : ctx->wf_h2[l]; p.wt_h2_inv = dgrad ? ctx->wd_h2_inv[l] : ctx->wf_h2_inv[l];
    p.band_rows = ctx->band_rows; p.mfma16 = ctx->mfma16; p.wg256 = ctx->wg256; p.tile_rows = ctx->tile_rows;
}
void conv_setup(const nst_ctx* ctx, ConvBatch& b, int l, bool dgrad) {
    b.mfma16 = ctx->mfma16; b.wg256 = ctx->wg256; b.tile_rows = ctx->tile_rows; b.persist = ctx->persist;
    if (l < 1) { b.wt_h2_inv = 1.f; return; }
    b.wt_bf = dgrad ? ctx->wd_bf[l] : ctx->wf_bf[l];
    b.wt_h2 = dgrad ? ctx->wd_h2[l] : ctx->wf_h2[l]; b.wt_h2_inv = dgrad ? ctx->wd_h2_inv[l] : ctx->wf_h2_inv[l];
    b.wt_wino = dgrad ? ctx->wd_wino[l] : ctx->wf_wino[l]; b.wt_wino_inv = dgrad ? ctx->wd_wino_inv[l] : ctx->wf_wino_inv[l];
}
int launch_conv_batch(nst_ctx* ctx, const ConvBatch& b, hipStream_t s, Timer* t, bool allow_wino) {
    const bool h2 = ctx->conv_mode == 2;
    if (h2 && allow_wino && b.wt_wino && conv_wino_eligible(b)) { if (t) t->mfma_factor(2.0); HIPCHK(ctx, launch_conv_wino_batch(b, s)); }
    else if (h2) {
        H2Shape sh{};
        const hipError_t e = launch_conv_h2_batch(b, s, &sh);
        if (t) t->shape(sh);
        HIPCHK(ctx, e);
    } else HIPCHK(ctx, launch_conv_bf3_batch(b, s));
    return NST_OK;
}
int launch_conv_batch(nst_ctx* ctx, const ConvBatch& b, Timer& t, bool allow_wino) { return launch_conv_batch(ctx, b, t.s, &t, allow_wino); }

hipError_t launch_pool_fwd(const nst_ctx* ctx, const float* in, int H, int W, int C, float* out, hipStream_t s) {
    return (ctx->pool_avg ? launch_avgpool_fwd : launch_maxpool_fwd)(in, H, W, C, out, s);
}
hipError_t launch_pool_bwd_relu(const nst_ctx* ctx, const float* a, const float* gpool, int H, int W, int C, float* gin, hipStream_t s) {
    return (ctx->pool_avg ? launch_avgpool_bwd_relu : launch_maxpool_bwd_relu)(a, gpool, H, W, C, gin, s);
}

struct StyleTerm { int C; size_t N; double divisor; float coef; };
StyleTerm style_term(const Taps& tp, int q, const ActSet& a, float sw, float w, int norm_rows = 0) {
    const int l = tp.style[q], C = kCout[l];
    const size_t N = (size_t)(norm_rows > 0 ? norm_rows >> kScale[l] : a.h[l]) * a.w[l];
    const double chw = (double)C * (double)N;
    return {C, N, chw, (float)((double)sw * (double)w * 4.0 / ((double)tp.nstyle * (double)C * C * chw))};
}
float content_coef(float cw, double n) { return (float)((double)cw * 2.0 / n); }

constexpr bool taps_avoid_pools() {
    for (int t : kTapLayer)
        for (int p : kPoolAfter) if (t == p) return false;
    return true;
}
static_assert(taps_avoid_pools(), "a map in front of a pooling layer became a tap: map_stored must keep it where a job reads it");
bool map_stored(const nst_ctx* ctx, int l) {
    if (ctx->conv_mode != 2 || ctx->keep_all_maps || ctx->use_graph) return true;
    return pool_index_after(l) < 0;
}

size_t gram_part_offset(const Taps& tp, int h, int w, int k) {
    size_t off = 0;
    for (int q = 0; q < k; ++q) {
        const int l = tp.style[q];
        const size_t N = (size_t)(h >> kScale[l]) * (w >> kScale[l]);
        off += (size_t)gram_nsplit(kCout[l], N) * kCout[l] * kCout[l];
    }
    return off;
}

StyleTerm guided_term(const Taps& tp, int q, const ActSet& a, float sw, float w, const Guidance& g, int r) {
    const int l = tp.style[q], C = kCout[l];
    const size_t N = (size_t)a.h[l] * a.w[l];
    const double cn = (double)C * g.mass[kScale[l]][r];
    return {C, N, cn, (float)((double)sw * (double)w * (double)g.lambda[r] * 4.0 / ((double)tp.nstyle * (double)C * C * cn))};
}
bool guided_levels(const nst_ctx* ctx, const int* lv, int n) { return n > 0 && ctx->lv[lv[0]].guide.R > 0; }
GuidedBwd guided_bwd_of(const nst_ctx* ctx, const LevelWs& L, int q) {
    const int l = ctx->taps.style[q], C = kCout[l];
    GuidedBwd gb{};
    gb.R = L.guide.R; gb.C = C; gb.N = (size_t)L.acts.h[l] * L.acts.w[l]; gb.F = L.acts.act[l];
    for (int r = 0; r < gb.R; ++r) {
        gb.t[r] = L.guide.plane(kScale[l], r, L.h, L.w);
        gb.S[r] = L.guide.S[q] + (size_t)r * C * C;
    }
    return gb;
}
int launch_guided_backward(nst_ctx* ctx, const GuidedBwd& gb, hipStream_t s) {
    Timer t(ctx, s, K_GRAM, 2.0 * (double)gb.N * gb.C * gb.C * gb.R);
    HIPCHK(ctx, launch_guided_bwd(gb, s));
    return NST_OK;
}
int guided_fold(nst_ctx* ctx, LevelWs& L, int q, hipStream_t s) {
    Timer t(ctx, s, K_OTHER, 0);
    HIPCHK(ctx, launch_guided_fold(L.guide.partial[q], L.guide.R, gram_finish_blocks(kCout[ctx->taps.style[q]]), L.guide.lambda,
                                   L.style_partial[q], s));
    return NST_OK;
}

int lap_forward(nst_ctx* ctx, LevelWs& L, const float* y, bool as_target, hipStream_t s) {
    for (int k = 0; k < ctx->lap_k; ++k) {
        const int p = ctx->lap_pool[k];
        {
            Timer t(ctx, s, K_OTHER, 0);
            HIPCHK(ctx, launch_lap_pool(y, ctx->channels, L.h, L.w, p, L.lap.s[k], s));
        }
        Timer t(ctx, s, K_OTHER, 0);
        if (as_target) HIPCHK(ctx, launch_lap_stencil(L.lap.s[k], L.h / p, L.w / p, nullptr, L.lap.target[k], nullptr, nullptr, s));
        else HIPCHK(ctx, launch_lap_stencil(L.lap.s[k], L.h / p, L.w / p, L.lap.target[k], nullptr, L.lap.r[k], L.lap.partial[k], s));
    }
    return NST_OK;
}
double lap_n(const LevelWs& L, int p) { return (double)(L.h / p - 2) * (double)(L.w / p - 2); }
float lap_coef(float gamma, double n, int p, int channels) {
    return (float)((double)gamma * 2.0 * (channels == 1 ? 3.0 : 1.0) / (n * (double)p * (double)p));
}
int lap_backward(nst_ctx* ctx, LevelWs& L, float* grad, hipStream_t s) {
    if (ctx->lap_k < 1) return NST_OK;
    LapBackward lb{};
    lb.K = ctx->lap_k;
    for (int k = 0; k < lb.K; ++k) {
        lb.p[k] = ctx->lap_pool[k];
        lb.coef[k] = lap_coef(ctx->lap_gamma[k], lap_n(L, lb.p[k]), lb.p[k], ctx->channels);
        lb.r[k] = L.lap.r[k];
    }
    Timer t(ctx, s, K_OTHER, 0);
    HIPCHK(ctx, launch_lap_backward(lb, ctx->channels, L.h, L.w, grad, 1, s));
    return NST_OK;
}

double mat_n(const nst_ctx* ctx, const LevelWs& L) { return (ctx->channels == 1 ? 1.0 : 3.0) * (double)(L.h - 2) * (double)(L.w - 2); }
float mat_coef(float gamma, double n) { return (float)((double)gamma * 2.0 / (255.0 * n)); }
int mat_forward(nst_ctx* ctx, LevelWs& L, const float* y, hipStream_t s) {
    if (!(ctx->mat_gamma > 0.f)) return NST_OK;
    Timer t(ctx, s, K_OTHER, 0);
    HIPCHK(ctx, launch_mat_forward(y, L.mat.guide, ctx->channels, L.h, L.w, 1.0 / 255.0, ctx->mat_eps, L.mat.partial, s));
    return NST_OK;
}
int mat_backward(nst_ctx* ctx, LevelWs& L, const float* y, float* grad, hipStream_t s) {
    if (!(ctx->mat_gamma > 0.f)) return NST_OK;
    Timer t(ctx, s, K_OTHER, 0);
    HIPCHK(ctx, launch_mat_backward(y, L.mat.guide, ctx->channels, L.h, L.w, 1.0 / 255.0, ctx->mat_eps,
                                    mat_coef(ctx->mat_gamma, mat_n(ctx, L)), grad, 1, s));
    return NST_OK;
}
int mat_set_guide(nst_ctx* ctx, LevelWs& L, const float* content, hipStream_t s) {
    if (!(ctx->mat_gamma > 0.f)) return NST_OK;
    HIPCHK(ctx, hipMemcpyAsync(L.mat.guide, content, (size_t)ctx->channels * L.h * L.w * sizeof(float), hipMemcpyDeviceToDevice, s));
    return NST_OK;
}

double anchor_n(const nst_ctx* ctx, const LevelWs& L) { return (double)ctx->channels * (double)L.h * (double)L.w; }
float anchor_coef(float gamma, double n) { return (float)((double)gamma * 2.0 / n); }
int anchor_forward(nst_ctx* ctx, LevelWs& L, const float* y, hipStream_t s) {
    if (!(L.anc.gamma > 0.f)) return NST_OK;
    Timer t(ctx, s, K_OTHER, 0);
    HIPCHK(ctx, launch_anchor_forward(y, L.anc.anchor, L.anc.weights, ctx->channels, L.h, L.w, L.anc.partial, s));
    return NST_OK;
}
int anchor_backward(nst_ctx* ctx, LevelWs& L, const float* y, float* grad, hipStream_t s) {
    if (!(L.anc.gamma > 0.f)) return NST_OK;
    Timer t(ctx, s, K_OTHER, 0);
    HIPCHK(ctx, launch_anchor_backward(y, L.anc.anchor, L.anc.weights, ctx->channels, L.h, L.w,
                                       anchor_coef(L.anc.gamma, anchor_n(ctx, L)), grad, 1, s));
    return NST_OK;
}

PatchTerm patch_term_of(const LevelWs& L, int i) {
    const int l = kTapLayer[i];
    return PatchTerm{L.acts.act[l], L.acts.h[l], L.acts.w[l], L.pm.nn[i], L.pm.d[i]};
}
double patch_denom(const LevelWs& L, int i) {
    const int l = kTapLayer[i];
    return 9.0 * (double)kCout[l] * (double)(L.acts.h[l] - 2) * (double)(L.acts.w[l] - 2);
}
float patch_coef(float w, double denom) { return (float)((double)w * 2.0 / denom); }
int patch_forward(nst_ctx* ctx, LevelWs& L, hipStream_t s) {
    for (int i = 0; i < 6 && L.pm.on(); ++i) {
        if (!(L.pm.w[i] > 0.f)) continue;
        const int l = kTapLayer[i];
// ... 1389 lines not shown
```

### artstyletransfer_amd/csrc/nst_ctx.cpp

```cpp
#include <algorithm>
#include <atomic>
#include <climits>
#include <cmath>
#include <cstdint>
#include <cstdio>
#include <cstdlib>
#include <cstring>

#include "nst_ctx.h"

using namespace nst;

namespace {
thread_local std::string g_err;
}

int nst::fail(nst_ctx* ctx, int code, const std::string& msg) {
    if (ctx) ctx->err = msg; else g_err = msg;
    return code;
}

namespace nst {

void poison_if_asked(void* p, size_t bytes) {
    static const char* spec = getenv("NST_POISON_ALLOC");
    static std::atomic<long> seq{0};
    if (!spec || !*spec) return;
    const long k = seq++;
    long lo = 0, hi = -1;
    if (strcmp(spec, "all") == 0) hi = LONG_MAX;
    else if (sscanf(spec, "%ld-%ld", &lo, &hi) != 2) return;
    if (k >= lo && k <= hi) { (void)hipMemset(p, 0xFF, bytes); (void)hipStreamSynchronize(nullptr); }
    if (getenv("NST_POISON_TRACE")) fprintf(stderr, "nst alloc #%ld: %zu bytes%s\n", k, bytes, (k >= lo && k <= hi) ? " (poisoned)" : "");
}
int zero_now(void* p, size_t bytes) {
    hipStream_t zs = nullptr;
    hipError_t e = hipStreamCreateWithFlags(&zs, hipStreamNonBlocking);
    if (e != hipSuccess) return 1;
    e = hipMemsetAsync(p, 0, bytes, zs);
    if (e == hipSuccess) e = hipStreamSynchronize(zs);
    (void)hipStreamDestroy(zs);
    return e == hipSuccess ? 0 : 1;
}

int dev_alloc(nst_ctx* ctx, void** p, size_t bytes, size_t* charged) {
    if (bytes == 0) bytes = 16;
    hipError_t e = hipMalloc(p, bytes);
    if (e != hipSuccess) return fail(ctx, NST_E_NOMEM, std::string("hipMalloc(") + std::to_string(bytes) + "): " + hipGetErrorString(e));
    poison_if_asked(*p, bytes);
    ctx->bytes += bytes;
    if (charged) *charged = bytes;
    return NST_OK;
}
void dev_release(nst_ctx* ctx, void* p, size_t bytes) {
    (void)hipFree(p);
    ctx->bytes -= bytes;
}

int alloc_acts(nst_ctx* ctx, ActSet& a, int h, int w) {
    for (int l = 0; l < NL; ++l) {
        a.h[l] = h >> kScale[l];
        a.w[l] = w >> kScale[l];
        if (a.h[l] < 1 || a.w[l] < 1) return fail(ctx, NST_E_ARG, "image too small for VGG19 (needs >= 16 px per side)");
        const size_t n = (size_t)a.h[l] * a.w[l] * kCout[l];
        NSTCHK(a.mem.alloc(ctx, &a.act[l], n));
    }
    for (int k = 0; k < 4; ++k) {
        const int l = kPoolAfter[k];
        const size_t n = (size_t)(a.h[l] / 2) * (a.w[l] / 2) * kCout[l];
        NSTCHK(a.mem.alloc(ctx, &a.pool[k], n));
        NSTCHK(a.mem.alloc(ctx, &a.pcode[k], n / 8));
    }
    size_t need = 0;
    for (int l = 1; l < NL; ++l) {
        const size_t px = (size_t)a.h[l] * a.w[l];
        const int sf = std::max(conv_ksplit(a.h[l], a.w[l], kCin[l], kCout[l]), conv_bf3_ksplit(a.h[l], a.w[l], kCin[l], kCout[l]));
        const int sb = std::max(conv_ksplit(a.h[l], a.w[l], kCout[l], kCin[l]), conv_bf3_ksplit(a.h[l], a.w[l], kCout[l], kCin[l]));
        const size_t fwd = (size_t)sf * px * kCout[l];
        const size_t bwd = (size_t)sb * px * kCin[l];
        if (fwd > px * kCout[l] && fwd > need) need = fwd;
        if (bwd > px * kCin[l] && bwd > need) need = bwd;
    }
    const int mask_layers[9] = {0, 2, 4, 5, 6, 8, 9, 10, 12};
    for (int k = 0; k < 9; ++k) {
        const int m = mask_layers[k];
        const size_t nw = (size_t)a.h[m] * a.w[m] * (kCout[m] / 32);
        NSTCHK(a.mem.alloc(ctx, &a.bits[m], nw));
    }
    NSTCHK(a.mem.alloc(ctx, &a.amax, (size_t)AMAX_IDS * NST_AMAX_SLOTS));
    if (zero_now(a.amax, (size_t)AMAX_IDS * NST_AMAX_SLOTS * 4)) return fail(ctx, NST_E_HIP, "hipMemset failed");
    a.splitk_floats = need;
    if (need) NSTCHK(a.mem.alloc(ctx, &a.splitk, need));
    return NST_OK;
}

}

namespace {

void cut3_host(float a, uint16_t& h, uint16_t& m, uint16_t& l) {
    uint32_t u; std::memcpy(&u, &a, 4);
    const uint32_t uh = u & 0xFFFF0000u;
    float fh; std::memcpy(&fh, &uh, 4);
    const float r1 = a - fh;
    uint32_t u1; std::memcpy(&u1, &r1, 4);
    const uint32_t um = u1 & 0xFFFF0000u;
    float fm; std::memcpy(&fm, &um, 4);
    const float r2 = r1 - fm;
    uint32_t u2; std::memcpy(&u2, &r2, 4);
    h = (uint16_t)(uh >> 16); m = (uint16_t)(um >> 16); l = (uint16_t)(u2 >> 16);
}
void make_bf3(const float* w, int taps, int rows, int K, std::vector<uint16_t>& out) {
    const int nch = K / 32;
    out.assign((size_t)taps * rows * nch * 96, 0);
    for (int t = 0; t < taps; ++t)
        for (int r = 0; r < rows; ++r)
            for (int k = 0; k < K; ++k) {
                uint16_t h, m, l;
                cut3_host(w[((size_t)t * rows + r) * K + k], h, m, l);
                const size_t base = (((size_t)t * rows + r) * nch + k / 32) * 96 + (k % 32);
                out[base] = h; out[base + 32] = m; out[base + 64] = l;
            }
}

static inline uint16_t f32_to_f16(float f) {
    uint32_t x; std::memcpy(&x, &f, 4);
    const uint32_t sign = (x >> 16) & 0x8000u;
    x &= 0x7FFFFFFFu;
    uint32_t o;
    if (x >= 0x47800000u) {
        o = (x > 0x7F800000u) ? 0x7E00u : 0x7C00u;
    } else if (x < 0x38800000u) {
        float a; std::memcpy(&a, &x, 4);
        const uint32_t magic_bits = (uint32_t)((127 - 15) + (23 - 10) + 1) << 23;
        float magic; std::memcpy(&magic, &magic_bits, 4);
        a += magic;
        uint32_t ab; std::memcpy(&ab, &a, 4);
        o = ab - magic_bits;
    } else {
        const uint32_t odd = (x >> 13) & 1u;
        x += 0xC8000FFFu + odd;
        o = x >> 13;
    }
    return (uint16_t)(sign | o);
}
static inline float f16_to_f32(uint16_t h) {
    const uint32_t sign = (uint32_t)(h & 0x8000u) << 16, e = (h >> 10) & 31u, m = h & 0x3FFu;
    uint32_t b;
    if (e == 0) { const float f = (float)m * 5.9604644775390625e-8f; std::memcpy(&b, &f, 4); b |= sign; }
    else if (e == 31) b = sign | 0x7F800000u | (m << 13);
    else b = sign | ((e + 112u) << 23) | (m << 13);
    float r; std::memcpy(&r, &b, 4);
    return r;
}

void make_h2(const float* w, int taps, int rows, int K, std::vector<uint16_t>& out, float* inv) {
    const int kc = (rows % 128 == 0 && K > NST_H2_SHORTK_CIN) ? 32 : 16;
    const size_t n = (size_t)taps * rows * K;
    float mx = 0.f;
    for (size_t i = 0; i < n; ++i) mx = std::max(mx, std::fabs(w[i]));
    int ex = 0;
    if (mx > 0.f) (void)std::frexp(mx, &ex);
    const float s = std::ldexp(1.f, 15 - ex);
    *inv = std::ldexp(1.f, ex - 15);
    const int nch = K / kc;
    out.assign((size_t)taps * rows * nch * 2 * kc, 0);
    for (int t = 0; t < taps; ++t)
        for (int r = 0; r < rows; ++r)
            for (int k = 0; k < K; ++k) {
                const float x = w[((size_t)t * rows + r) * K + k] * s;
                const uint16_t uh = f32_to_f16(x);
                const uint16_t ul = f32_to_f16((x - f16_to_f32(uh)) * 2048.f);
                const size_t base = (((size_t)t * rows + r) * nch + k / kc) * 2 * kc + (k % kc);
                out[base] = uh; out[base + kc] = ul;
            }
}

void make_wino(const float* w, int rows, int K, std::vector<uint16_t>& out, float* inv) {
    const int nct = rows / 128, nch = K / 32;
    std::vector<float> U((size_t)12 * rows * K);
    float mx = 0.f;
    for (int ky = 0; ky < 3; ++ky)
        for (int o = 0; o < rows; ++o) {
            const float* g0 = w + ((size_t)(ky * 3 + 0) * rows + o) * K;
            const float* g1 = w + ((size_t)(ky * 3 + 1) * rows + o) * K;
            const float* g2 = w + ((size_t)(ky * 3 + 2) * rows + o) * K;
            float* u0 = U.data() + ((size_t)(ky * 4 + 0) * rows + o) * K;
            float* u1 = U.data() + ((size_t)(ky * 4 + 1) * rows + o) * K;
            float* u2 = U.data() + ((size_t)(ky * 4 + 2) * rows + o) * K;
            float* u3 = U.data() + ((size_t)(ky * 4 + 3) * rows + o) * K;
            for (int c = 0; c < K; ++c) {
                const double a = g0[c], b = g1[c], d = g2[c];
                u0[c] = (float)a;
                u1[c] = (float)(0.5 * (a + b + d));
                u2[c] = (float)(0.5 * (a - b + d));
                u3[c] = (float)d;
                mx = std::max(std::max(mx, std::fabs(u0[c])), std::max(std::fabs(u1[c]), std::max(std::fabs(u2[c]), std::fabs(u3[c]))));
            }
        }
    int ex = 0;
    if (mx > 0.f) (void)std::frexp(mx, &ex);
    const float s = std::ldexp(1.f, 15 - ex);
    *inv = std::ldexp(1.f, ex - 15);
    out.assign((size_t)nct * nch * 3 * 8 * 2 * 2 * 2 * 64 * 8, 0);
    for (int ct = 0; ct < nct; ++ct)
        for (int ch = 0; ch < nch; ++ch)
            for (int ky = 0; ky < 3; ++ky)
                for (int wave = 0; wave < 8; ++wave)
                    for (int ks = 0; ks < 2; ++ks)
                        for (int nt = 0; nt < 2; ++nt) {
                            const int x = wave & 3, wn = wave >> 2;
                            const size_t unit0 = ((((((size_t)(ct * nch + ch) * 3 + ky) * 8 + wave) * 2 + ks) * 2 + nt) * 2) * 64;
                            for (int lane = 0; lane < 64; ++lane) {
                                const int r = lane & 31, h = lane >> 5;
                                const int o = ct * 128 + wn * 64 + nt * 32 + r;
                                const float* src = U.data() + ((size_t)(ky * 4 + x) * rows + o) * K + ch * 32 + ks * 16 + 8 * h;
                                uint16_t* hi_dst = out.data() + (unit0 + lane) * 8;
                                uint16_t* lo_dst = out.data() + (unit0 + 64 + lane) * 8;
                                for (int j = 0; j < 8; ++j) {
                                    const float v = src[j] * s;
                                    hi_dst[j] = f32_to_f16(v);
                                    lo_dst[j] = f32_to_f16((v - f16_to_f32(hi_dst[j])) * 2048.f);
                                }
                            }
                        }
}

void free_tap_buffers(LevelWs& L) {
    L.tap_mem.release();
    L.content_t = nullptr; L.content_n = 0;
    for (int k = 0; k < kMaxStyle; ++k) { L.gram_t[k] = nullptr; L.S[k] = nullptr; L.S_bf[k] = nullptr; L.style_partial[k] = nullptr; }
    L.gram_part = nullptr; L.gram_part_floats = 0;
}
int alloc_tap_buffers(nst_ctx* ctx, LevelWs& L) {
    const Taps& tp = ctx->taps;
    const int m = tp.content;
    L.content_n = (size_t)L.acts.h[m] * L.acts.w[m] * kCout[m];
    NSTCHK(L.tap_mem.alloc(ctx, &L.content_t, L.content_n));
    for (int k = 0; k < tp.nstyle; ++k) {
        const int C = kCout[tp.style[k]];
        NSTCHK(L.tap_mem.alloc(ctx, &L.gram_t[k], (size_t)C * C));
        NSTCHK(L.tap_mem.alloc(ctx, &L.S[k], (size_t)C * C));
        NSTCHK(L.tap_mem.alloc(ctx, &L.S_bf[k], (size_t)C * C * 3));
        NSTCHK(L.tap_mem.alloc(ctx, &L.style_partial[k], gram_finish_blocks(C)));
    }
    L.gram_part_floats = gram_part_floats_for(tp, L.h, L.w);
    NSTCHK(L.tap_mem.alloc(ctx, &L.gram_part, L.gram_part_floats));
    return NST_OK;
}

int alloc_level_image(nst_ctx* ctx, LevelImage& im, int channels, int h, int w) {
    const size_t n = (size_t)channels * h * w;
    NSTCHK(im.mem.alloc(ctx, &im.xl, n));
    NSTCHK(im.mem.alloc(ctx, &im.gxl, n));
    return NST_OK;
}

void free_level(LevelWs& L) {
    if (L.stream) (void)hipStreamDestroy(L.stream);
    if (L.done) (void)hipEventDestroy(L.done);
    L = LevelWs();
}

}

namespace nst {

void drop_closure_state(nst_ctx* ctx, bool drop_targets) {
    if (ctx->gexec) { (void)hipGraphExecDestroy(ctx->gexec); ctx->gexec = nullptr; }
    ctx->gkey = {}; ctx->glast = {};
    for (int i = 0; drop_targets && i < ctx->levels; ++i) { ctx->lv[i].targets = false; ctx->lv[i].guide.targets = false; }
    if (drop_targets) forget_forward_pass(ctx);
}
void forget_forward_pass(nst_ctx* ctx) {
    for (int i = 0; i < NST_MAX_LEVELS; ++i) {
        ctx->lv[i].acts.pass = 0; ctx->lv[i].acts.pass_n = 0;
        for (bool& st : ctx->lv[i].acts.stored) st = false;
    }
}

int fold_timed(nst_ctx* ctx) {
    if (!ctx->timed_valid) return NST_OK;
    HIPCHK(ctx, hipEventSynchronize(ctx->t1));
    float ms = 0.f;
    HIPCHK(ctx, hipEventElapsedTime(&ms, ctx->t0, ctx->t1));
    ctx->acc_closure_ms += ms;
    if (!ctx->timed_backward) {
        ctx->acc_closures += 1;
        if (!ctx->timed.empty()) ctx->acc_sampled += 1;
    }
    ctx->timed_backward = false;
    for (const TimedLaunch& t : ctx->timed) {
        float d = 0.f;
        HIPCHK(ctx, hipEventSynchronize(t.b));
        HIPCHK(ctx, hipEventElapsedTime(&d, t.a, t.b));
        ctx->acc_ms[t.cls] += d;
        ctx->acc_flops[t.cls] += t.flops;
        {
            const double mode = (t.cls == K_CONV3 || t.cls == K_GRAM) ? (ctx->conv_mode == 2 ? 3.0 : ctx->conv_mode == 1 ? 6.0 : 1.0) : 1.0;
            ctx->acc_mfma[t.cls] += t.flops * (t.mfma_factor >= 0.0 ? t.mfma_factor : mode);
        }
        ctx->acc_launches[t.cls] += 1;
    }
    ctx->timed.clear();
    ctx->ev_used = 0;
    ctx->timed_valid = false;
    return NST_OK;
}

int bind(nst_ctx* ctx) {
    if (!ctx) return fail(nullptr, NST_E_ARG, "null context");
    HIPCHK(ctx, hipSetDevice(ctx->device));
    return NST_OK;
}

void mark(nst_ctx* ctx, hipStream_t s) {
    if (ctx && ctx->tail && hipEventRecord(ctx->tail, s) == hipSuccess) { ctx->tail_stream = s; ctx->tail_set = true; }
}
hipStream_t enter(nst_ctx* ctx, void* stream) {
    hipStream_t s = static_cast<hipStream_t>(stream);
    if (ctx->tail_set && s != ctx->tail_stream) (void)hipStreamWaitEvent(s, ctx->tail, 0);
    return s;
}
void quiesce(nst_ctx* ctx) {
    if (ctx->tail) (void)hipEventSynchronize(ctx->tail);
    for (int i = 0; i < NST_MAX_LEVELS; ++i)
        if (ctx->lv[i].stream) (void)hipStreamSynchronize(ctx->lv[i].stream);
    if (ctx->gstream) (void)hipStreamSynchronize(ctx->gstream);
    if (ctx->side) (void)hipStreamSynchronize(ctx->side);
}

}

namespace {

int env_flag(const char* name, int dflt) {
    const char* e = getenv(name);
    if (!e || !e[0]) return dflt;
    return std::atoi(e);
}

unsigned positive_weight_mask(const float* w) {
    unsigned m = 0;
    for (int i = 0; i < 6; ++i) if (w[i] > 0.f) m |= 1u << i;
    return m;
}
unsigned style_mask_of(const Taps& tp) {
    unsigned m = 0;
    for (int q = 0; q < tp.nstyle; ++q) m |= 1u << tap_index_of(tp.style[q]);
    return m;
}

template <typename Block, typename Fill>
int replace_term(nst_ctx* ctx, Block LevelWs::*member, Fill fill) {
    return replace_blocks(ctx->lv, ctx->levels, member, fill, [&] { quiesce(ctx); drop_closure_state(ctx, true); });
}

}

extern "C" {

int nst_version(void) { return 200; }

const char* nst_last_error(const nst_ctx* ctx) { return ctx ? ctx->err.c_str() : g_err.c_str(); }

int nst_device_count(int* count) {
    if (!count) return fail(nullptr, NST_E_ARG, "count is null");
    int n = 0;
    hipError_t e = hipGetDeviceCount(&n);
    if (e != hipSuccess) { *count = 0; return fail(nullptr, NST_E_HIP, hipGetErrorString(e)); }
    *count = n;
    return NST_OK;
}

void nst_options_default(nst_options* o) {
    if (!o) return;
    o->struct_size = (int)sizeof(nst_options);
    o->conv_mode = -1; o->batched = -1; o->single_stream = -1; o->use_graph = -1; o->h2_band_rows = -1; o->lbfgs_gram = -1;
    o->h2_mfma16 = -1; o->h2_wg256 = -1; o->h2_tile_rows = -1; o->gram_overlap = -1; o->h2_persist = -1; o->level_split = -1; o->h2_winograd = -1;
}

int nst_ctx_create(int device, const float* const* weights, const float* const* biases, nst_ctx** out) {
    return nst_ctx_create_ex(device, weights, biases, nullptr, out);
}

int nst_ctx_create_ex(int device, const float* const* weights, const float* const* biases, const nst_options* opts_in,
                      nst_ctx** out) {
    if (!weights || !biases || !out) return fail(nullptr, NST_E_ARG, "null argument");
    nst_options opts;
    nst_options_default(&opts);
    if (opts_in) {
        if (opts_in->struct_size != (int)sizeof(nst_options)) return fail(nullptr, NST_E_ARG, "nst_options.struct_size mismatch (use nst_options_default)");
        opts = *opts_in;
    }
    for (int l = 0; l < NL; ++l)
        if (!weights[l] || !biases[l]) return fail(nullptr, NST_E_ARG, "null weight/bias pointer");
    int ndev = 0;
    if (hipGetDeviceCount(&ndev) != hipSuccess || ndev < 1) return fail(nullptr, NST_E_HIP, "no HIP device visible");
    if (device < 0 || device >= ndev) return fail(nullptr, NST_E_ARG, "device index out of range");
    nst_ctx* ctx = new (std::nothrow) nst_ctx();
    if (!ctx) return fail(nullptr, NST_E_NOMEM, "out of host memory");
    ctx->device = device;
    auto bail = [&](int code) { g_err = ctx->err; nst_ctx_destroy(ctx); return code; };
    if (hipSetDevice(device) != hipSuccess) { ctx->err = "hipSetDevice failed"; return bail(NST_E_HIP); }
    hipError_t e = conv_mfma_init_device();
    if (e == hipSuccess) e = conv_bf3_init_device();
    if (e == hipSuccess) e = conv_h2_init_device();
    if (e == hipSuccess) e = conv_wino_init_device();
    if (e == hipSuccess) e = gram_init_device();
    if (e == hipSuccess) e = pm_init_device();
    if (opts.conv_mode >= 0) {
        if (opts.conv_mode > NST_CONV_F16X2) { ctx->err = "nst_options.conv_mode must be NST_CONV_F32, NST_CONV_BF16X3 or NST_CONV_F16X2"; return bail(NST_E_ARG); }
        ctx->conv_mode = opts.conv_mode;
    } else {
        const char* cm = getenv("NST_CONV");
        if (cm && std::strcmp(cm, "f32") == 0) ctx->conv_mode = 0;
        else if (cm && std::strcmp(cm, "bf16x3") == 0) ctx->conv_mode = 1;
        else if (cm && std::strcmp(cm, "f16x2") == 0) ctx->conv_mode = 2;
        else if (cm && cm[0]) { ctx->err = "NST_CONV must be f32, bf16x3 or f16x2"; return bail(NST_E_ARG); }
    }
    ctx->batched = (opts.batched >= 0 ? opts.batched : env_flag("NST_BATCH", 1)) ? 1 : 0;
    ctx->use_graph = (opts.use_graph >= 0 ? opts.use_graph : env_flag("NST_GRAPH", 0)) ? 1 : 0;
    ctx->single_stream = (opts.single_stream >= 0 ? opts.single_stream : env_flag("NST_SINGLE_STREAM", 0)) != 0;
    ctx->band_rows = opts.h2_band_rows >= 0 ? opts.h2_band_rows : env_flag("NST_H2_BAND_ROWS", 0);
    ctx->lbfgs_gram = (opts.lbfgs_gram >= 0 ? opts.lbfgs_gram : env_flag("NST_LBFGS_GRAM", 1)) ? 1 : 0;
    ctx->mfma16 = opts.h2_mfma16 >= 0 ? opts.h2_mfma16 : env_flag("NST_H2_MFMA16", 1);
    ctx->wg256 = (opts.h2_wg256 >= 0 ? opts.h2_wg256 : env_flag("NST_H2_WG256", 0)) ? 1 : 0;
    ctx->tile_rows = opts.h2_tile_rows >= 0 ? opts.h2_tile_rows : env_flag("NST_H2_TILE_ROWS", 0);
    ctx->persist = (opts.h2_persist >= 0 ? opts.h2_persist : env_flag("NST_H2_PERSIST", 0)) ? 1 : 0;
    ctx->winograd = (opts.h2_winograd >= 0 ? opts.h2_winograd : env_flag("NST_H2_WINOGRAD", 1)) ? 1 : 0;
    ctx->level_split = (opts.level_split >= 0 ? opts.level_split : env_flag("NST_LEVEL_SPLIT", 0)) ? 1 : 0;
    ctx->gram_overlap = (opts.gram_overlap >= 0 ? opts.gram_overlap : env_flag("NST_GRAM_OVERLAP", 0)) ? 1 : 0;
    ctx->keep_all_maps = env_flag("NST_KEEP_ALL_MAPS", 0) ? 1 : 0;
    ctx->forward_pack = env_flag("NST_FORWARD_PACK", 1) ? 1 : 0;
    ctx->gram_pack = env_flag("NST_GRAM_PACK", 1) ? 1 : 0;
    if (ctx->use_graph && hipStreamCreateWithFlags(&ctx->gstream, hipStreamNonBlocking) != hipSuccess) { ctx->err = "stream creation failed"; return bail(NST_E_HIP); }
    if (e != hipSuccess) { ctx->err = std::string("kernel attribute setup: ") + hipGetErrorString(e); return bail(NST_E_HIP); }

    std::vector<float> tmp;
    std::vector<uint16_t> tmp16;
    auto upload = [&](auto& dst, const void* src, size_t bytes, const char* what) -> int {
        if (ctx->mem.alloc_bytes(ctx, reinterpret_cast<void**>(&dst), bytes) != NST_OK) return NST_E_NOMEM;
        if (hipMemcpy(dst, src, bytes, hipMemcpyHostToDevice) != hipSuccess) { ctx->err = std::string(what) + " upload failed"; return NST_E_HIP; }
        return NST_OK;
    };
    auto pieces = [&](int rows, int K, void*& bf, void*& h2, float& h2_inv, void*& wino, float& wino_inv) -> int {
        if (ctx->conv_mode == 1) {
            make_bf3(tmp.data(), 9, rows, K, tmp16);
            return upload(bf, tmp16.data(), tmp16.size() * 2, "weight");
        }
        if (ctx->conv_mode != 2) return NST_OK;
        make_h2(tmp.data(), 9, rows, K, tmp16, &h2_inv);
        NSTCHK(upload(h2, tmp16.data(), tmp16.size() * 2, "weight"));
        if (ctx->winograd && K >= 256 && K % 64 == 0 && rows % 128 == 0) {
            make_wino(tmp.data(), rows, K, tmp16, &wino_inv);
            NSTCHK(upload(wino, tmp16.data(), tmp16.size() * 2, "weight"));
        }
        return NST_OK;
    };
    for (int l = 0; l < NL; ++l) {
        const int ci = kCin[l], co = kCout[l];
        const float* W = weights[l];
        if (int r = upload(ctx->bias[l], biases[l], co * 4, "bias")) return bail(r);
        if (l == 0) {
            tmp.assign(28 * 64, 0.f);
            for (int o = 0; o < 64; ++o)
                for (int c = 0; c < 3; ++c)
                    for (int t = 0; t < 9; ++t) tmp[(c * 9 + t) * 64 + o] = W[(o * 3 + c) * 9 + t];
            if (int r = upload(ctx->w11k, tmp.data(), tmp.size() * 4, "weight")) return bail(r);
            tmp.assign(9 * 64 * 4, 0.f);
            for (int t = 0; t < 9; ++t) {
                const int ky = 2 - t / 3, kx = 2 - t % 3;
                for (int o = 0; o < 64; ++o)
                    for (int c = 0; c < 3; ++c) tmp[(t * 64 + o) * 4 + c] = W[(o * 3 + c) * 9 + ky * 3 + kx];
            }
            if (int r = upload(ctx->w11d, tmp.data(), tmp.size() * 4, "weight")) return bail(r);
            continue;
        }
        const size_t n = (size_t)9 * ci * co;
        tmp.resize(n);
        for (int t = 0; t < 9; ++t)
            for (int o = 0; o < co; ++o)
                for (int c = 0; c < ci; ++c) tmp[((size_t)t * co + o) * ci + c] = W[((size_t)o * ci + c) * 9 + t];
        if (int r = upload(ctx->wf[l], tmp.data(), n * 4, "weight")) return bail(r);
        if (int r = pieces(co, ci, ctx->wf_bf[l], ctx->wf_h2[l], ctx->wf_h2_inv[l], ctx->wf_wino[l], ctx->wf_wino_inv[l])) return bail(r);
        for (int t = 0; t < 9; ++t) {
            const int ky = 2 - t / 3, kx = 2 - t % 3;
            for (int c = 0; c < ci; ++c)
                for (int o = 0; o < co; ++o) tmp[((size_t)t * ci + c) * co + o] = W[((size_t)o * ci + c) * 9 + ky * 3 + kx];
        }
        if (int r = upload(ctx->wd[l], tmp.data(), n * 4, "weight")) return bail(r);
        if (int r = pieces(ci, co, ctx->wd_bf[l], ctx->wd_h2[l], ctx->wd_h2_inv[l], ctx->wd_wino[l], ctx->wd_wino_inv[l])) return bail(r);
    }
    if (ctx->level_split) ctx->gram_overlap = 0;
    if ((ctx->gram_overlap || ctx->level_split) && ctx->conv_mode == 2 &&
        (hipStreamCreateWithFlags(&ctx->side, hipStreamNonBlocking) != hipSuccess ||
         hipEventCreateWithFlags(&ctx->side_fork, hipEventDisableTiming) != hipSuccess ||
         hipEventCreateWithFlags(&ctx->side_join, hipEventDisableTiming) != hipSuccess)) {
        ctx->err = "side stream creation failed";
        return bail(NST_E_HIP);
    }
    if (hipEventCreateWithFlags(&ctx->fork, hipEventDisableTiming) != hipSuccess ||
        hipEventCreateWithFlags(&ctx->tail, hipEventDisableTiming) != hipSuccess ||
        hipEventCreate(&ctx->t0) != hipSuccess || hipEventCreate(&ctx->t1) != hipSuccess) {
        ctx->err = "event creation failed";
        return bail(NST_E_HIP);
    }
    *out = ctx;
    return NST_OK;
}

void nst_ctx_destroy(nst_ctx* ctx) {
    if (!ctx) return;
    (void)hipSetDevice(ctx->device);
    quiesce(ctx);
    for (int i = 0; i < NST_MAX_LEVELS; ++i) free_level(ctx->lv[i]);
    if (ctx->tail) (void)hipEventDestroy(ctx->tail);
    ctx->mem.release();
    drop_closure_state(ctx, false);
    if (ctx->gstream) (void)hipStreamDestroy(ctx->gstream);
    if (ctx->side) (void)hipStreamDestroy(ctx->side);
    if (ctx->side_fork) (void)hipEventDestroy(ctx->side_fork);
    if (ctx->side_join) (void)hipEventDestroy(ctx->side_join);
    if (ctx->fork) (void)hipEventDestroy(ctx->fork);
    if (ctx->t0) (void)hipEventDestroy(ctx->t0);
    if (ctx->t1) (void)hipEventDestroy(ctx->t1);
    for (hipEvent_t e : ctx->ev_pool) (void)hipEventDestroy(e);
    delete ctx;
}

int nst_conv_mode(const nst_ctx* ctx) { return ctx ? ctx->conv_mode : -1; }

int nst_ctx_bytes(const nst_ctx* ctx, size_t* bytes) {
    if (!ctx || !bytes) return fail(nullptr, NST_E_ARG, "null argument");
    *bytes = ctx->bytes;
    return NST_OK;
}

int nst_job_configure(nst_ctx* ctx, int levels_num, int H0, int W0) {
    if (ctx) { ++ctx->closure_epoch; ++ctx->ws_seq; }
    NSTCHK(bind(ctx));
    if (levels_num < 1 || levels_num > NST_MAX_LEVELS) return fail(ctx, NST_E_ARG, "levels_num out of range");
    if ((H0 >> (levels_num - 1)) < 16 || (W0 >> (levels_num - 1)) < 16)
        return fail(ctx, NST_E_ARG, "coarsest pyramid level must be at least 16x16");
    quiesce(ctx);
    for (int i = 0; i < NST_MAX_LEVELS; ++i) free_level(ctx->lv[i]);
    drop_closure_state(ctx, false);
    forget_forward_pass(ctx);
    ctx->levels = 0;
    ctx->lap_k = 0;
    ctx->mat_gamma = 0.f; ctx->mat_eps = 1e-7;
    for (float& v : ctx->gs_shift) v = 0.f;
    ctx->gs_center = 0u;
    for (int i = 0; i < 6; ++i) { ctx->mom_wm[i] = 0.f; ctx->mom_ws[i] = 0.f; }
    ctx->mom_eps = 1e-5f;
    int h = H0, w = W0;
    for (int i = 0; i < levels_num; ++i) {
        LevelWs& L = ctx->lv[i];
        L.h = h; L.w = w;
        NSTCHK(alloc_acts(ctx, L.acts, h, w));
        L.gbuf_floats = (size_t)h * w * 64;
        NSTCHK(L.mem.alloc(ctx, &L.gbuf[0], L.gbuf_floats));
        NSTCHK(L.mem.alloc(ctx, &L.gbuf[1], L.gbuf_floats));
        if (i > 0) NSTCHK(alloc_level_image(ctx, L.img, ctx->channels, h, w));
        NSTCHK(alloc_tap_buffers(ctx, L));
        NSTCHK(L.mem.alloc(ctx, &L.content_partial, MSE_BLOCKS));
        NSTCHK(L.mem.alloc(ctx, &L.tv_partial, 2 * TV_BLOCKS));
        NSTCHK(L.mem.alloc(ctx, &L.tv_means, 2));
        h /= 2; w /= 2;
    }
    ctx->levels = levels_num;
    return NST_OK;
}

int nst_job_set_taps(nst_ctx* ctx, int content_index, unsigned style_mask, int use_relu) {
    if (ctx) { ++ctx->closure_epoch; ++ctx->ws_seq; }
    NSTCHK(bind(ctx));
    if (content_index < 0 || content_index > 5) return fail(ctx, NST_E_ARG, "content_index must be 0 .. 5");
    if (style_mask == 0u || (style_mask & ~0x3Fu) != 0u)
        return fail(ctx, NST_E_ARG, "style_mask must be a non-empty set of bits 0 .. 5");
    if (use_relu != 0 && use_relu != 1) return fail(ctx, NST_E_ARG, "use_relu must be 0 or 1");
    Taps tp;
    tp.content = kTapLayer[content_index];
    tp.nstyle = 0;
    for (int i = 0; i < 6; ++i)
        if ((style_mask >> i) & 1u) tp.style[tp.nstyle++] = kTapLayer[i];
    tp.top = std::max(tp.content, tp.style[tp.nstyle - 1]);
    tp.use_relu = use_relu;
    tp.is_default = content_index == 4 && style_mask == 0x2Fu && use_relu == 1;
    if ((style_mask & positive_weight_mask(ctx->style_w)) == 0u)
        return fail(ctx, NST_E_ARG, "no map of style_mask has a positive style layer weight (nst_job_set_style_weights)");
    quiesce(ctx);
    drop_closure_state(ctx, true);
    ctx->taps = tp;
    for (int i = 0; i < ctx->levels; ++i) {
        LevelWs& L = ctx->lv[i];
        L.guide = Guidance();
        L.pm = PatchLevel();
        free_tap_buffers(L);
        NSTCHK(alloc_tap_buffers(ctx, L));
    }
    return NST_OK;
}

int nst_job_set_color(nst_ctx* ctx, int mode) {
    if (ctx) { ++ctx->closure_epoch; ++ctx->ws_seq; }
    NSTCHK(bind(ctx));
    if (mode != NST_COLOR_RGB && mode != NST_COLOR_LUMINANCE) return fail(ctx, NST_E_ARG, "mode must be NST_COLOR_RGB or NST_COLOR_LUMINANCE");
    const int channels = mode == NST_COLOR_LUMINANCE ? 1 : 3;
    quiesce(ctx);
    LevelWs* lv = ctx->lv + 1;
    NSTCHK(replace_blocks(lv, ctx->levels - 1, &LevelWs::img,
                          [&](int i, LevelImage& im) { return alloc_level_image(ctx, im, channels, lv[i].h, lv[i].w); },
                          [&] { drop_closure_state(ctx, true); }));
    for (int i = 0; i < ctx->levels && channels != ctx->channels; ++i) ctx->lv[i].anc = AnchorLevel();
    for (int i = 0; i < ctx->levels; ++i) ctx->lv[i].pm = PatchLevel();
    ctx->channels = channels;
    return NST_OK;
}

int nst_job_color(const nst_ctx* ctx) { return ctx ? (ctx->channels == 1 ? NST_COLOR_LUMINANCE : NST_COLOR_RGB) : -1; }

int nst_job_set_pooling(nst_ctx* ctx, int mode) {
    if (ctx) { ++ctx->closure_epoch; ++ctx->ws_seq; }
    NSTCHK(bind(ctx));
    if (mode != NST_POOL_MAX && mode != NST_POOL_AVG) return fail(ctx, NST_E_ARG, "mode must be NST_POOL_MAX or NST_POOL_AVG");
    quiesce(ctx);
    drop_closure_state(ctx, true);
    for (int i = 0; i < ctx->levels; ++i) ctx->lv[i].pm = PatchLevel();
    ctx->pool_avg = mode == NST_POOL_AVG ? 1 : 0;
    return NST_OK;
}

int nst_ctx_set_keep_all_maps(nst_ctx* ctx, int enabled) {
    NSTCHK(bind(ctx));
    ++ctx->ws_seq;
    drop_closure_state(ctx, false);
    ctx->keep_all_maps = enabled ? 1 : 0;
    return NST_OK;
}
int nst_ctx_keep_all_maps(const nst_ctx* ctx) { return ctx ? ctx->keep_all_maps : -1; }

int nst_ctx_set_forward_pack(nst_ctx* ctx, int enabled) {
    NSTCHK(bind(ctx));
    ++ctx->ws_seq;
    drop_closure_state(ctx, false);
    ctx->forward_pack = enabled ? 1 : 0;
    return NST_OK;
}
int nst_ctx_forward_pack(const nst_ctx* ctx) { return ctx ? ctx->forward_pack : -1; }

int nst_ctx_set_gram_pack(nst_ctx* ctx, int enabled) {
    NSTCHK(bind(ctx));
    ++ctx->ws_seq;
    drop_closure_state(ctx, false);
    ctx->gram_pack = enabled ? 1 : 0;
    return NST_OK;
}
int nst_ctx_gram_pack(const nst_ctx* ctx) { return ctx ? ctx->gram_pack : -1; }

int nst_job_map_stats(nst_ctx* ctx, int level, unsigned* stored_mask) {
    NSTCHK(bind(ctx));
    if (level < 0 || level >= ctx->levels) return fail(ctx, NST_E_STATE, "level not configured");
    if (!stored_mask) return fail(ctx, NST_E_ARG, "null argument");
    unsigned m = 0;
    for (int l = 0; l < NL; ++l) m |= (ctx->lv[level].acts.stored[l] ? 1u : 0u) << l;
    *stored_mask = m;
    return NST_OK;
}

int nst_job_pooling(const nst_ctx* ctx) { return ctx ? (ctx->pool_avg ? NST_POOL_AVG : NST_POOL_MAX) : -1; }

int nst_job_set_laplacian(nst_ctx* ctx, int K, const int* pool, const float* gamma) {
    if (ctx) { ++ctx->closure_epoch; ++ctx->ws_seq; }
    NSTCHK(bind(ctx));
    if (ctx->levels < 1) return fail(ctx, NST_E_STATE, "nst_job_configure has not been called");
    if (K < 0 || K > NST_MAX_LAPLACIAN) return fail(ctx, NST_E_ARG, "the number of Laplacian entries must be 0 .. NST_MAX_LAPLACIAN");
    if (K > 0 && (!pool || !gamma)) return fail(ctx, NST_E_ARG, "null argument");
    bool positive = false;
    for (int k = 0; k < K; ++k) {
        if (pool[k] < 1 || pool[k] > 32) return fail(ctx, NST_E_ARG, "a Laplacian pool size must be 1 .. 32");
        for (int j = 0; j < k; ++j)
            if (pool[j] == pool[k]) return fail(ctx, NST_E_ARG, "the Laplacian entries must have distinct pool sizes");
        if (!(gamma[k] >= 0.f) || std::isinf(gamma[k])) return fail(ctx, NST_E_ARG, "Laplacian weights must be finite and >= 0");
        positive = positive || gamma[k] > 0.f;
        for (int i = 0; i < ctx->levels; ++i)
            if (ctx->lv[i].h / pool[k] < 3 || ctx->lv[i].w / pool[k] < 3)
                return fail(ctx, NST_E_ARG, "level " + std::to_string(i) + " is too small for Laplacian pool size " + std::to_string(pool[k]) +
                                            ": the pooled image must be at least 3x3");
    }
    if (K > 0 && !positive) return fail(ctx, NST_E_ARG, "at least one Laplacian weight must be positive");
    NSTCHK(replace_term(ctx, &LevelWs::lap, [&](int i, LapLevel& q) {
        if (K > 0 && i == 0) NSTCHK(q.mem.alloc(ctx, &q.vals, (size_t)NST_MAX_LEVELS * NST_LAP_MAX));
        for (int k = 0; k < K; ++k) {
            const size_t hk = (size_t)(ctx->lv[i].h / pool[k]), wk = (size_t)(ctx->lv[i].w / pool[k]);
            NSTCHK(q.mem.alloc(ctx, &q.s[k], hk * wk));
            NSTCHK(q.mem.alloc(ctx, &q.r[k], (hk - 2) * (wk - 2)));
            NSTCHK(q.mem.alloc(ctx, &q.target[k], (hk - 2) * (wk - 2)));
            NSTCHK(q.mem.alloc(ctx, &q.partial[k], LAP_BLOCKS));
        }
        return NST_OK;
    }));
    ctx->lap_k = K;
    for (int k = 0; k < NST_LAP_MAX; ++k) {
        ctx->lap_pool[k] = k < K ? pool[k] : 0;
        ctx->lap_gamma[k] = k < K ? gamma[k] : 0.f;
    }
    if (K > 0) HIPCHK(ctx, hipMemset(ctx->lv[0].lap.vals, 0, (size_t)NST_MAX_LEVELS * NST_LAP_MAX * sizeof(float)));
    return NST_OK;
}

int nst_job_laplacian(const nst_ctx* ctx, int* K, int* pool, float* gamma) {
    if (!ctx) return fail(nullptr, NST_E_ARG, "null context");
    if (K) *K = ctx->lap_k;
    for (int k = 0; k < NST_LAP_MAX; ++k) {
        if (pool) pool[k] = ctx->lap_pool[k];
        if (gamma) gamma[k] = ctx->lap_gamma[k];
    }
    return NST_OK;
}

int nst_job_laplacian_losses(nst_ctx* ctx, float* out, void* stream) {
    NSTCHK(bind(ctx));
    if (ctx->levels < 1) return fail(ctx, NST_E_STATE, "nst_job_configure has not been called");
    if (!out) return fail(ctx, NST_E_ARG, "null argument");
    hipStream_t s = enter(ctx, stream);
    const size_t bytes = (size_t)ctx->levels * NST_LAP_MAX * sizeof(float);
    if (ctx->lap_k > 0) HIPCHK(ctx, hipMemcpyAsync(out, ctx->lv[0].lap.vals, bytes, hipMemcpyDeviceToDevice, s));
    else HIPCHK(ctx, hipMemsetAsync(out, 0, bytes, s));
    mark(ctx, s);
    return NST_OK;
}

int nst_job_set_matting(nst_ctx* ctx, float gamma, double epsilon) {
    if (ctx) { ++ctx->closure_epoch; ++ctx->ws_seq; }
    NSTCHK(bind(ctx));
    if (ctx->levels < 1) return fail(ctx, NST_E_STATE, "nst_job_configure has not been called");
    if (!(gamma >= 0.f) || std::isinf(gamma)) return fail(ctx, NST_E_ARG, "the matting weight must be finite and >= 0");
    if (!(epsilon > 0.0) || std::isinf(epsilon)) return fail(ctx, NST_E_ARG, "the matting epsilon must be finite and > 0");
    const bool on = gamma > 0.f;
    NSTCHK(replace_term(ctx, &LevelWs::mat, [&](int i, MatLevel& q) {
        if (!on) return NST_OK;
        if (i == 0) NSTCHK(q.mem.alloc(ctx, &q.vals, (size_t)NST_MAX_LEVELS));
        const size_t px = (size_t)ctx->lv[i].h * ctx->lv[i].w;
        q.tiles = mat_tiles(ctx->lv[i].h, ctx->lv[i].w);
        NSTCHK(q.mem.alloc(ctx, &q.guide, 3 * px));
        NSTCHK(q.mem.alloc(ctx, &q.partial, (size_t)q.tiles));
        return NST_OK;
    }));
    ctx->mat_gamma = gamma;
    ctx->mat_eps = epsilon;
    if (on) HIPCHK(ctx, hipMemset(ctx->lv[0].mat.vals, 0, (size_t)NST_MAX_LEVELS * sizeof(float)));
    return NST_OK;
}

int nst_job_matting(const nst_ctx* ctx, float* gamma, double* epsilon) {
    if (!ctx) return fail(nullptr, NST_E_ARG, "null context");
    if (gamma) *gamma = ctx->mat_gamma;
    if (epsilon) *epsilon = ctx->mat_eps;
    return NST_OK;
}

int nst_job_matting_losses(nst_ctx* ctx, float* out, void* stream) {
    NSTCHK(bind(ctx));
    if (ctx->levels < 1) return fail(ctx, NST_E_STATE, "nst_job_configure has not been called");
    if (!out) return fail(ctx, NST_E_ARG, "null argument");
    hipStream_t s = enter(ctx, stream);
    const size_t bytes = (size_t)ctx->levels * sizeof(float);
    if (ctx->mat_gamma > 0.f) HIPCHK(ctx, hipMemcpyAsync(out, ctx->lv[0].mat.vals, bytes, hipMemcpyDeviceToDevice, s));
    else HIPCHK(ctx, hipMemsetAsync(out, 0, bytes, s));
    mark(ctx, s);
    return NST_OK;
}

int nst_job_set_gram_shift(nst_ctx* ctx, const float* shift, unsigned center_mask) {
    if (ctx) { ++ctx->closure_epoch; ++ctx->ws_seq; }
    NSTCHK(bind(ctx));
    if (!shift) return fail(ctx, NST_E_ARG, "null argument");
    if ((center_mask & ~0x3Fu) != 0u) return fail(ctx, NST_E_ARG, "center_mask must be a set of bits 0 .. 5");
    bool on = center_mask != 0u;
    for (int i = 0; i < 6; ++i) {
        if (!std::isfinite(shift[i])) return fail(ctx, NST_E_ARG, "Gram shifts must be finite");
        if (((center_mask >> i) & 1u) && shift[i] != 0.f) return fail(ctx, NST_E_ARG, "a centred map takes no constant shift: its entry must be 0");
        on = on || shift[i] != 0.f;
    }
    if (on) {
        if (ctx->levels < 1) return fail(ctx, NST_E_STATE, "nst_job_configure has not been called");
        if (ctx->conv_mode != 2) return fail(ctx, NST_E_STATE, "the shifted Gram runs in the f16x2 arithmetic only (NST_CONV unset)");
        for (int i = 0; i < ctx->levels; ++i)
            if (ctx->lv[i].guide.R > 0)
                return fail(ctx, NST_E_STATE, "guided Gram matrices take the plain statistic only (nst_level_set_guidance(ctx, level, 0, ...) clears the guidance)");
    }
    NSTCHK(replace_term(ctx, &LevelWs::gs, [&](int, GramShiftLevel& q) {
        if (!on) return NST_OK;
        NSTCHK(q.mem.alloc(ctx, &q.words, (size_t)kMaxStyle * GS_STRIDE));
        if (center_mask) NSTCHK(q.mem.alloc(ctx, &q.sums, (size_t)kMaxStyle * GS_PART_DOUBLES));
        if (hipMemset(q.words, 0, (size_t)kMaxStyle * GS_STRIDE * sizeof(float)) != hipSuccess)
            return fail(ctx, NST_E_HIP, "hipMemset of the Gram offsets failed");
        return NST_OK;
    }));
    for (int i = 0; i < 6; ++i) ctx->gs_shift[i] = shift[i];
    ctx->gs_center = center_mask;
    return NST_OK;
}

int nst_job_gram_shift(const nst_ctx* ctx, float* shift, unsigned* center_mask) {
    if (!ctx) return fail(nullptr, NST_E_ARG, "null context");
    for (int i = 0; i < 6 && shift; ++i) shift[i] = ctx->gs_shift[i];
    if (center_mask) *center_mask = ctx->gs_center;
    return NST_OK;
}

// ... 377 lines not shown
```

### artstyletransfer_amd/csrc/nst_ctx.h

```cpp
#pragma once
#include <hip/hip_runtime.h>

#include <cstddef>
#include <optional>
#include <string>
#include <utility>
#include <vector>

#include "../../include/nst_hip.h"
#include "nst_kernels.h"

#pragma GCC visibility push(hidden)
#include "nst_devmem.h"
namespace nst {

constexpr int NL = NST_VGG19_CONVS;
constexpr int kCin[NL] = {3, 64, 64, 128, 128, 256, 256, 256, 256, 512, 512, 512, 512};
constexpr int kCout[NL] = {64, 64, 128, 128, 256, 256, 256, 256, 512, 512, 512, 512, 512};
constexpr int kScale[NL] = {0, 0, 1, 1, 2, 2, 2, 2, 3, 3, 3, 3, 4};
constexpr int kPoolAfter[4] = {1, 3, 7, 11};
constexpr int kTapLayer[6] = {0, 2, 4, 8, 9, 12};
constexpr int kMaxStyle = 6;
inline int tap_index_of(int layer) {
    for (int i = 0; i < 6; ++i) if (kTapLayer[i] == layer) return i;
// ... 60 lines not shown
    float* gram_t[kMaxStyle] = {};
    float* S[kMaxStyle] = {};
    double* partial[kMaxStyle] = {};
    float* part = nullptr;
    size_t part_floats_r = 0;
    bool targets = false;
    int targets_R = 0;
    DevMem mem;
    const float* plane(int scale, int r, int h, int w) const { return planes + plane_off[scale] + (size_t)r * (h >> scale) * (w >> scale); }
};

struct LapLevel {
    double* s[NST_LAP_MAX] = {};
    float* r[NST_LAP_MAX] = {};
    double* target[NST_LAP_MAX] = {};
    double* partial[NST_LAP_MAX] = {};
    float* vals = nullptr;
    DevMem mem;
};

struct MatLevel {
    float* guide = nullptr;
    double* partial = nullptr;
    int tiles = 0;
    float* vals = nullptr;
    DevMem mem;
};

constexpr int GS_MAX_C = 512;
constexpr int GS_STRIDE = 2 * GS_MAX_C + NST_AMAX_SLOTS;
constexpr bool maps_fit_gram_shift() {
    for (int c : kCout) if (c > GS_MAX_C) return false;
    return true;
}
static_assert(maps_fit_gram_shift(), "a map wider than GS_MAX_C: the per-slot buffers of GramShiftLevel are sized by it");
struct GramShiftLevel {
    float* words = nullptr;
    double* sums = nullptr;
    DevMem mem;
    float* offset(int q) const { return words + (size_t)q * GS_STRIDE; }
    float* row_bias(int q) const { return words + (size_t)q * GS_STRIDE + GS_MAX_C; }
    unsigned* amax(int q) const { return reinterpret_cast<unsigned*>(words + (size_t)q * GS_STRIDE + 2 * GS_MAX_C); }
    double* part(int q) const { return sums ? sums + (size_t)q * GS_PART_DOUBLES : nullptr; }
};

constexpr int MOM_STRIDE = 3 * GS_MAX_C;
constexpr int MOM_STAT_STRIDE = 2 * GS_MAX_C + 2;
struct MomentLevel {
    float* words = nullptr;
    double* stats = nullptr;
    double* sums = nullptr;
    float* vals = nullptr;
    DevMem mem;
    float* mean_t(int q) const { return words + (size_t)q * MOM_STRIDE; }
    float* std_t(int q) const { return words + (size_t)q * MOM_STRIDE + GS_MAX_C; }
    float* row_bias(int q) const { return words + (size_t)q * MOM_STRIDE + 2 * GS_MAX_C; }
    double* stat(int q) const { return stats + (size_t)q * MOM_STAT_STRIDE; }
    double* loss(int q) const { return stats + (size_t)q * MOM_STAT_STRIDE + 2 * GS_MAX_C; }
    double* part(int q) const { return sums + (size_t)q * MOM_PART_DOUBLES; }
};

struct AnchorLevel {
    float gamma = 0.f;
    float* anchor = nullptr;
    float* weights = nullptr;
    double* partial = nullptr;
    float* val = nullptr;
    DevMem mem;
};

struct PatchLevel {
    float w[6] = {};
    int stride = 1;
    double eps = 1e-5;
    PatchDict d[6] = {};
    unsigned long long* keys[6] = {};
    int* nn[6] = {};
    double* partial[6] = {};
    float* vals = nullptr;
    DevMem mem;
    bool on() const {
        for (float v : w) if (v > 0.f) return true;
        return false;
    }
};

struct LevelImage {
    float* xl = nullptr;
    float* gxl = nullptr;
    DevMem mem;
};

struct LevelWs {
    int h = 0, w = 0;
    Guidance guide;
    LapLevel lap;
    MatLevel mat;
    GramShiftLevel gs;
    MomentLevel mom;
    AnchorLevel anc;
    PatchLevel pm;
    ActSet acts;
    float* gbuf[2] = {};
    size_t gbuf_floats = 0;
    LevelImage img;
    float* content_t = nullptr;
    size_t content_n = 0;
    float* gram_t[kMaxStyle] = {};
    float* S[kMaxStyle] = {};
    unsigned short* S_bf[kMaxStyle] = {};
    float* gram_part = nullptr;
    size_t gram_part_floats = 0;
    double* style_partial[kMaxStyle] = {};
    DevMem tap_mem;
    double* content_partial = nullptr;
    double* tv_partial = nullptr;
    float* tv_means = nullptr;
    bool targets = false;
    hipStream_t stream = nullptr;
    hipEvent_t done = nullptr;
    DevMem mem;
};

}

struct nst_ctx {
    int device = 0;
    std::string err;
    float* wf[nst::NL] = {};
    float* wd[nst::NL] = {};
    void* wf_bf[nst::NL] = {};
    void* wd_bf[nst::NL] = {};
    void* wd_wino[nst::NL] = {};
    float wd_wino_inv[nst::NL] = {};
    void* wf_wino[nst::NL] = {};
    float wf_wino_inv[nst::NL] = {};
    int winograd = 0;
    void* wf_h2[nst::NL] = {};
    void* wd_h2[nst::NL] = {};
    float wf_h2_inv[nst::NL] = {};
    float wd_h2_inv[nst::NL] = {};
    int conv_mode = 2;
    int band_rows = 0;
    int lbfgs_gram = 1;
    int mfma16 = 1;
    int wg256 = 0;
    int tile_rows = 0;
    int gram_overlap = 0;
    int persist = 1;
    int level_split = 0;
    int keep_all_maps = 0;
    int forward_pack = 1;
    int gram_pack = 1;
    unsigned long long fwd_pass = 0;
    hipStream_t side = nullptr;
    hipEvent_t side_fork = nullptr, side_join = nullptr;
    hipStream_t tail_stream = nullptr;
    bool tail_set = false;
    hipEvent_t tail = nullptr;
    int batched = 1;
    int use_graph = 0;
    hipStream_t gstream = nullptr;
    hipGraphExec_t gexec = nullptr;
    struct GraphKey { const float* x; float* grad; float* losses; float cw, sw, tvw; unsigned mask; } gkey{}, glast{};
    float* bias[nst::NL] = {};
    float* w11k = nullptr;
    float* w11d = nullptr;
    int levels = 0;
    nst::Taps taps;
    int channels = 3;
    int pool_avg = 0;
    float style_w[6] = {1.f, 1.f, 1.f, 1.f, 1.f, 1.f};
    float style_weight(int q) const { return style_w[nst::tap_index_of(taps.style[q])]; }
    bool unit_style_weights() const {
        for (float w : style_w) if (w != 1.f) return false;
        return true;
    }
    int lap_k = 0;
    int lap_pool[nst::NST_LAP_MAX] = {};
    float lap_gamma[nst::NST_LAP_MAX] = {};
    float mat_gamma = 0.f;
    double mat_eps = 1e-7;
    float gs_shift[6] = {};
    unsigned gs_center = 0;
    bool gs_on() const {
        for (float v : gs_shift) if (v != 0.f) return true;
        return gs_center != 0u;
    }
    float gs_shift_of(int q) const { return gs_shift[nst::tap_index_of(taps.style[q])]; }
    int gs_center_of(int q) const { return (int)((gs_center >> nst::tap_index_of(taps.style[q])) & 1u); }
    float mom_wm[6] = {};
    float mom_ws[6] = {};
    float mom_eps = 1e-5f;
    bool mom_on() const {
        for (int i = 0; i < 6; ++i) if (mom_wm[i] > 0.f || mom_ws[i] > 0.f) return true;
        return false;
    }
    float mom_wm_of(int q) const { return mom_wm[nst::tap_index_of(taps.style[q])]; }
    float mom_ws_of(int q) const { return mom_ws[nst::tap_index_of(taps.style[q])]; }
    bool mom_slot(int q) const { return mom_wm_of(q) > 0.f || mom_ws_of(q) > 0.f; }
    const float* row_bias_of(const nst::LevelWs& L, int q) const {
        if (mom_on() && mom_slot(q)) return L.mom.row_bias(q);
        return gs_on() ? L.gs.row_bias(q) : nullptr;
    }
    unsigned long long closure_epoch = 0;
    unsigned long long ws_seq = 0;
    struct ForwardToken {
        bool valid = false;
        const float* x = nullptr;
        float cw = 0.f, sw = 0.f, tvw = 0.f;
        unsigned mask = 0;
        unsigned long long epoch = 0, seq = 0;
    } fwd_token;
    double* color_scratch = nullptr;
    nst::LevelWs lv[NST_MAX_LEVELS];
    hipEvent_t fork = nullptr;
    size_t bytes = 0;
    nst::DevMem mem;
    bool single_stream = false;
    struct ClosureSchedule { int side_forks = 0, level_streams = 0, graph_replay = 0; } sched;
    int timing = 0;
    hipEvent_t t0 = nullptr, t1 = nullptr;
    std::vector<hipEvent_t> ev_pool;
    size_t ev_used = 0;
    std::vector<nst::TimedLaunch> timed;
    bool timed_valid = false;
    bool timed_backward = false;
    double acc_ms[4] = {0, 0, 0, 0};
    double acc_flops[4] = {0, 0, 0, 0};
    double acc_mfma[4] = {0, 0, 0, 0};
    long acc_launches[4] = {0, 0, 0, 0};
    double acc_closure_ms = 0;
    long acc_closures = 0;
    long acc_sampled = 0;
    long closure_seq = 0;
    bool sample_now = true;
};

namespace nst {

int fail(nst_ctx* ctx, int code, const std::string& msg);

#define HIPCHK(ctx, expr)                                                                         \
    do {                                                                                          \
        hipError_t _e = (expr);                                                                   \
        if (_e != hipSuccess)                                                                     \
            return fail(ctx, NST_E_HIP, std::string(#expr) + ": " + hipGetErrorString(_e));       \
    } while (0)

#define NSTCHK(expr)                 \
    do {                             \
        int _r = (expr);             \
        if (_r != NST_OK) return _r; \
    } while (0)

struct Timer {
    nst_ctx* ctx; hipStream_t s; bool on; size_t slot;
    Timer(nst_ctx* c, hipStream_t st, int cls, double flops, int t0 = 0, int t1 = 0, int t2 = 0, int t3 = 0, int t4 = 0,
          int t5 = 0)
        : ctx(c), s(st), on(false), slot(0) {
        if (c->timing >= 2 && (c->timing < 3 || cls == K_CONV3) && c->sample_now && c->ev_used + 2 <= c->ev_pool.size()) {
            on = true;
            TimedLaunch t{c->ev_pool[c->ev_used], c->ev_pool[c->ev_used + 1], cls, flops, {t0, t1, t2, t3, t4, t5}, -1.0, H2Shape{}};
            c->ev_used += 2;
            slot = c->timed.size();
            c->timed.push_back(t);
            (void)hipEventRecord(t.a, st);
        }
    }
    ~Timer() { if (on) (void)hipEventRecord(ctx->timed[slot].b, s); }
    void mfma_factor(double f) { if (on) ctx->timed[slot].mfma_factor = f; }
    void shape(const H2Shape& sh) { if (on) ctx->timed[slot].shape = sh; }
};
int fold_timed(nst_ctx* ctx);

void poison_if_asked(void* p, size_t bytes);
int zero_now(void* p, size_t bytes);
int alloc_acts(nst_ctx* ctx, ActSet& a, int h, int w);
int bind(nst_ctx* ctx);
void drop_closure_state(nst_ctx* ctx, bool drop_targets);
hipStream_t enter(nst_ctx* ctx, void* stream);
void mark(nst_ctx* ctx, hipStream_t s);
void quiesce(nst_ctx* ctx);

struct Scratch {
    nst_ctx* ctx; hipStream_t s; ActSet acts; DevMem bufs; bool open = true;
    Scratch(nst_ctx* c, hipStream_t st) : ctx(c), s(st) {}
    ~Scratch() { (void)release(); }
    template <typename T>
    int alloc(T** p, size_t count) { return bufs.alloc(ctx, p, count); }
    hipError_t release() {
        if (!open) return hipSuccess;
        open = false;
        const hipError_t e = hipStreamSynchronize(s);
        acts = ActSet();
        bufs.release();
        return e;
    }
    int finish() { const hipError_t e = release(); HIPCHK(ctx, e); return NST_OK; }
};

struct Inject {
    const float* S = nullptr;
    const void* S_bf = nullptr;
    const unsigned* S_amax = nullptr;
    const float* direct = nullptr;
// ... 34 lines not shown
```

### artstyletransfer_amd/csrc/nst_kernels.h

```cpp
#pragma once
#include <hip/hip_runtime.h>
#include <stddef.h>

namespace nst {

struct ConvParams {
    const float* in;
    const float* wt;
    const void* wt_bf;
    const float* bias;
    const float* addend;
    const float* mask;
    float* out;
    int H, W, Cin, Cout;
    int relu;
    int tiles_x, tiles_y;
    float* partial;
    size_t partial_floats;
    int ksplit;
    const float* in2;
    int Cin2;
    const void* wt2_bf;
    unsigned* bits_out;
    const unsigned* bits_in;
    float* pool_out;
    const void* wt_h2;
    float wt_h2_inv;
    const float* wt2_f32;
    const unsigned* amax_in;
    const unsigned* amax_in2;
    const unsigned* amax_w2;
    unsigned* amax_out;
    const unsigned* pcode_in;
    unsigned* pcode_out;
    int in2_row0, in2_rows;
    int ty0;
    int band_rows;
    int mfma16;
    int wg256;
    int tile_rows;
    int pool_avg;
};

constexpr int NST_AMAX_SLOTS = 64;
#ifndef NST_H2_SHORTK_CIN_VALUE
#define NST_H2_SHORTK_CIN_VALUE 128
#endif
constexpr int NST_H2_SHORTK_CIN = NST_H2_SHORTK_CIN_VALUE;

struct ConvImage {
    const float* in;
    const float* addend;
    const float* mask;
    float* out;
    const float* in2;
    const void* wt2_bf;
    unsigned* bits_out;
    const unsigned* bits_in;
    float* pool_out;
    int H, W;
    int tiles_x, tile_end;
    int ty0;
    const float* wt2_f32;
    const unsigned* amax_in;
    const unsigned* amax_in2;
    const unsigned* amax_w2;
    unsigned* amax_out;
    const unsigned* pcode_in;
    unsigned* pcode_out;
    int in2_row0, in2_rows;
    const float* bias;
};
struct ConvBatch {
    ConvImage img[8];
    int n;
    const void* wt_bf;
    const float* bias;
    int Cin, Cout, Cin2, relu;
    const void* wt_h2;
    float wt_h2_inv;
    int unpool;
    int mfma16, wg256, tile_rows;
    int persist;
    int total_tiles;
    const void* wt_wino;
    float wt_wino_inv;
    int pool_avg;
};

hipError_t conv_wino_init_device();
bool conv_wino_eligible(const ConvBatch& b);
hipError_t launch_conv_wino_batch(const ConvBatch& b, hipStream_t stream);

hipError_t conv_mfma_init_device();
hipError_t launch_conv_mfma(const ConvParams& p, int taps, hipStream_t stream);
int conv_ksplit(int H, int W, int Cin, int Cout);

hipError_t launch_conv_splitk_finish(const ConvParams& p, hipStream_t stream);

hipError_t conv_bf3_init_device();
hipError_t launch_conv_bf3(const ConvParams& p, hipStream_t stream);
hipError_t launch_conv_bf3_batch(const ConvBatch& b, hipStream_t stream);
int conv_bf3_ksplit(int H, int W, int Cin, int Cout);

hipError_t conv_h2_init_device();
struct H2Shape {
    int rows, bn, ntw, chunk;
    int m16;
    int persist;
    int second, unpool;
    int bands;
};
hipError_t launch_conv_h2(const ConvParams& p, hipStream_t stream, H2Shape* shape = nullptr);
hipError_t launch_conv_h2_batch(const ConvBatch& b, hipStream_t stream, H2Shape* shape = nullptr);
hipError_t launch_absmax_slots(const float* x, size_t n, unsigned* slots, hipStream_t stream);

hipError_t launch_conv1_1_fwd(const float* x, int H, int W, const float* wk, const float* bias, float* out,
                              unsigned* bits_out, unsigned* amax_out, hipStream_t stream, int channels = 3);
struct Conv1Image {
    const float* x; float* out; unsigned* bits_out; unsigned* amax_out;
    int H, W;
    int tiles_x, tile_end;
};
struct Conv1Batch { Conv1Image img[8]; int n; const float* wk; const float* bias; int channels; };
hipError_t launch_conv1_1_fwd_batch(const Conv1Batch& b, hipStream_t stream);
hipError_t launch_conv1_1_dgrad(const float* g, int H, int W, const float* wd, const unsigned* amax_g, float* gx,
                                hipStream_t stream, int channels = 3);

hipError_t launch_maxpool_fwd(const float* in, int H, int W, int C, float* out, hipStream_t stream);
hipError_t launch_maxpool_bwd_relu(const float* a, const float* gpool, int H, int W, int C, float* gin,
                                   hipStream_t stream);
hipError_t launch_avgpool_fwd(const float* in, int H, int W, int C, float* out, hipStream_t stream);
hipError_t launch_avgpool_bwd_relu(const float* a, const float* gpool, int H, int W, int C, float* gin,
                                   hipStream_t stream);
hipError_t launch_chw_to_hwc(const float* src, int C, int H, int W, float* dst, hipStream_t stream);
hipError_t launch_hwc_to_chw(const float* src, int C, int H, int W, float* dst, hipStream_t stream);
hipError_t launch_relu_mask(const float* act, const float* g, size_t n, float* dst, hipStream_t stream);
hipError_t launch_add_inplace(float* dst, const float* src, size_t n, hipStream_t stream);

hipError_t launch_bicubic_down(const float* x, int C, int h, int w, int oh, int ow, float* y, hipStream_t stream);
hipError_t launch_bicubic_down_bwd(const float* gy, int C, int h, int w, int oh, int ow, float* gx, int accumulate,
                                   hipStream_t stream);

constexpr int TV_BLOCKS = 1024;
hipError_t launch_tv_partial(const float* y, int C, int h, int w, double* partial, hipStream_t stream, int row0 = 0,
                             int rows = 0);
struct TvBatch { const float* y[8]; int h[8], w[8]; double* partial[8]; float* means[8]; int n; int C; };
hipError_t launch_tv_partial_batch(const TvBatch& b, hipStream_t stream);
hipError_t launch_tv_means_batch(const TvBatch& b, hipStream_t stream);
hipError_t launch_tv_finish(const float* y, int C, int h, int w, const double* partial, float weight, float* grad,
                            int accumulate, float* means, hipStream_t stream, int row0 = 0, int rows = 0,
                            const float* given_means = nullptr, double nx = 0, double ny = 0);

constexpr int MSE_BLOCKS = 256;
hipError_t launch_mse_grad(const float* a, const float* t, size_t n, float coef, float* g, double* partial,
                           hipStream_t stream);

struct MseBatch { const float* a[8]; const float* t[8]; size_t cnt[8]; double* partial[8]; int n; };
hipError_t launch_mse_partial_batch(const MseBatch& b, hipStream_t stream);

hipError_t launch_sum_doubles(const double* p, int n, int stride, int offset, float* out, hipStream_t stream);
hipError_t launch_window_scalars(const float* sums, double nx, double ny, float* means, double* partial, int n,
                                 hipStream_t stream);

hipError_t launch_prepare_img(const float* hwc, int h, int w, float* chw, hipStream_t stream);
hipError_t launch_unprepare_img(const float* chw, int h, int w, float* hwc, hipStream_t stream);

constexpr int NST_LAP_MAX = 4;
constexpr int LAP_BLOCKS = 256;
hipError_t launch_lap_pool(const float* y, int C, int h, int w, int p, double* s, hipStream_t stream);
hipError_t launch_lap_stencil(const double* s, int hk, int wk, const double* target, double* target_out, float* r, double* partial,
                              hipStream_t stream);
hipError_t launch_lap_value(const double* partial, double n, float* out, hipStream_t stream);
struct LapBackward {
    int K;
    int p[NST_LAP_MAX];
    float coef[NST_LAP_MAX];
    const float* r[NST_LAP_MAX];
    int hk[NST_LAP_MAX], wk[NST_LAP_MAX];
    unsigned magic[NST_LAP_MAX];
};
hipError_t launch_lap_backward(const LapBackward& lb, int C, int h, int w, float* grad, int accumulate, hipStream_t stream);

int mat_tiles(int h, int w);
hipError_t launch_mat_forward(const float* y, const float* guide, int C, int h, int w, double gscale, double eps, double* partial,
                              hipStream_t stream);
hipError_t launch_mat_backward(const float* y, const float* guide, int C, int h, int w, double gscale, double eps, float coef,
                               float* grad, int accumulate, hipStream_t stream);
hipError_t launch_mat_value(const double* partial, int tiles, double n, float* out, hipStream_t stream);

constexpr int ANCHOR_BLOCKS = 256;
int anchor_block_elems();
hipError_t launch_anchor_forward(const float* y, const float* a, const float* c, int C, int h, int w, double* partial,
                                 hipStream_t stream);
hipError_t launch_anchor_value(const double* partial, int blocks, double n, float* out, hipStream_t stream);
hipError_t launch_anchor_backward(const float* y, const float* a, const float* c, int C, int h, int w, float coef, float* grad,
                                  int accumulate, hipStream_t stream);
hipError_t launch_warp_bilinear(const float* src, const float* flow, int C, int h, int w, float* out, float* valid,
                                hipStream_t stream);
hipError_t launch_flow_weights(const float* fwd, const float* bwd, int h, int w, float* out, hipStream_t stream);
constexpr int NST_FOLD_MAX_SOURCES = 8;
struct AnchorFoldArgs {
    const float* sources[NST_FOLD_MAX_SOURCES];
    const float* weights[NST_FOLD_MAX_SOURCES];
};
hipError_t launch_anchor_fold(const AnchorFoldArgs& a, int J, int C, int h, int w, float* anchor, float* weight,
                              float* parts , hipStream_t stream);
unsigned anchor_fold_vec_mask(const AnchorFoldArgs& a, int J, int C, size_t hw, const float* anchor, const float* weight,
                              const float* parts);

constexpr int NST_FLOW_MAX_SCALES = 12;
struct FlowLayout {
    int scales;
    int h[NST_FLOW_MAX_SCALES], w[NST_FLOW_MAX_SCALES];
    size_t from[NST_FLOW_MAX_SCALES], to[NST_FLOW_MAX_SCALES];
    size_t ix, iy, rho;
    size_t other;
    size_t floats;
};
int flow_layout(int h, int w, int scales, FlowLayout* out);
hipError_t launch_flow_reduce(const float* in, int h, int w, float* out, hipStream_t stream);
hipError_t launch_flow_prolong(const float* coarse, int h, int w, float* fine, hipStream_t stream);
hipError_t launch_flow_linearize(const float* from, const float* to, const float* u, const float* v, int h, int w, float* Ix,
                                 float* Iy, float* rho, hipStream_t stream);
hipError_t launch_flow_sweeps(const float* Ix, const float* Iy, const float* rho, const float* in, int h, int w, float alpha2, int n,
                              float* out, float* tmp, hipStream_t stream);
hipError_t launch_flow_estimate(const float* from, const float* to, const FlowLayout& l, float alpha2, int warps, int iterations,
                                float* flow, float* ws, hipStream_t stream);

struct FlowTvl1Layout {
    FlowLayout hs;
    size_t dual[2];
    size_t floats;
};
int flow_tvl1_layout(int h, int w, int scales, FlowTvl1Layout* out);
hipError_t launch_flow_tvl1_iterations(const float* Ix, const float* Iy, const float* rho, const float* fin, const float* pin, int h,
                                       int w, float lt, float theta, float taut, int n, float* fout, float* pout, float* ftmp,
                                       float* ptmp, hipStream_t stream);
hipError_t launch_flow_tvl1_estimate(const float* from, const float* to, const FlowTvl1Layout& t, float lt, float theta, float taut,
                                     int warps, int iterations, float* flow, float* ws, hipStream_t stream);

struct LevelLossInputs {
    const double* content_partial;
    size_t content_n;
    const double* style_partial[6];
    int style_c[6];
    float style_w[6];
    const float* tv_means;
    int owned;
    const double* lap_partial[NST_LAP_MAX];
    double lap_n[NST_LAP_MAX];
    const double* mat_partial;
    int mat_tiles;
    double mat_n;
    const double* mom_loss;
    const double* tmp_partial;
    float tmp_gamma;
    double tmp_n;
    float* tmp_out;
    float* mrf_vals;
    float mrf_w[6];
};
struct LossAssembly {
    LevelLossInputs lv[8];
// ... 163 lines not shown
```

### artstyletransfer_amd/engine.py

```python
from __future__ import annotations

import ctypes as C
from typing import List, Optional, Sequence, Tuple

import numpy as np
import torch

from . import _lib
from . import taps as _taps
from .pooling_modes import check_pooling
from . import style_modes as _style
from . import regions as _regions
from . import gram_modes as _gram
from . import moment_modes as _mom
from . import laplacian_modes as _lap
from . import matting_modes as _mat
from . import flow_modes as _flow
from . import mrf_modes as _mrf
from ._lib import NST_LOSS_ROW, NstError, StepInfo

TAP_CHANNELS = (64, 128, 256, 512, 512, 512)
TAP_SCALE = (0, 1, 2, 3, 3, 4)
DEFAULT_TAPS = (_taps.DEFAULT_CONTENT_INDEX, _taps.DEFAULT_STYLE_INDICES, True)


_JOB_SETTINGS = (
    ("layer_weights", "style_weights", "reset_style_weights", False),
    ("taps", None, "reset_taps", False),
    ("channels", "_channels", "reset_color", False),
    ("pooling", "_pooling", "reset_pooling", False),
    ("laplacian", "laplacian_setting", "reset_laplacian", True),
    ("gram_shift", "gram_shift_setting", "reset_gram_shift", True),
    ("matting", "matting_setting", "reset_matting", True),
    ("moment_loss", "moments_setting", "reset_moments", True),
)
_READER = {attr: reader for attr, reader, _, _ in _JOB_SETTINGS}


def _ptr(t: Optional[torch.Tensor]):
    return C.c_void_p(t.data_ptr()) if t is not None else C.c_void_p(0)


def _stream(device) -> C.c_void_p:
    return C.c_void_p(torch.cuda.current_stream(device).cuda_stream)


def _chk_dev(t: torch.Tensor, device, shape=None):
    if not (t.is_cuda and t.dtype == torch.float32 and t.is_contiguous()):
        raise NstError("expected a contiguous float32 CUDA tensor")
    if t.device != device:
        raise NstError(f"tensor is on {t.device}, context on {device}")
    if shape is not None and tuple(t.shape) != tuple(shape):
        raise NstError(f"expected shape {tuple(shape)}, got {tuple(t.shape)}")


def flow_workspace(h: int, w: int, scales: int = 0) -> Tuple[int, int]:
    floats, used = C.c_size_t(), C.c_int()
    if _lib.load().nst_flow_workspace(int(h), int(w), int(scales), C.byref(floats), C.byref(used)) != _lib.NST_OK:
        raise ValueError(f"no flow workspace for {h}x{w} planes and scales={scales}")
    return floats.value, used.value


def flow_tvl1_workspace(h: int, w: int, scales: int = 0) -> Tuple[int, int]:
    floats, used = C.c_size_t(), C.c_int()
    if _lib.load().nst_flow_tvl1_workspace(int(h), int(w), int(scales), C.byref(floats), C.byref(used)) != _lib.NST_OK:
        raise ValueError(f"no TV-L1 flow workspace for {h}x{w} planes and scales={scales}")
    return floats.value, used.value


class StyleEngine:

    def __init__(self, weights: Sequence[Tuple[torch.Tensor, torch.Tensor]], device: int | str | torch.device = 0,
                 conv_mode: Optional[str] = None, batched: Optional[bool] = None, single_stream: Optional[bool] = None,
                 use_graph: Optional[bool] = None, h2_band_rows: Optional[int] = None, lbfgs_gram: Optional[bool] = None,
                 h2_mfma16: Optional[bool] = None, h2_wg256: Optional[bool] = None,
                 h2_tile_rows: Optional[int] = None, gram_overlap: Optional[bool] = None,
                 h2_persist: Optional[bool] = None, level_split: Optional[bool] = None,
                 h2_winograd: Optional[bool] = None, keep_all_maps: Optional[bool] = None,
                 forward_pack: Optional[bool] = None, gram_pack: Optional[bool] = None):
        self.lib = _lib.load()
        if not torch.cuda.is_available():
            raise NstError("no GPU visible: the style-transfer hot path runs only on the HIP device")
        self.device = torch.device(device if not isinstance(device, int) else f"cuda:{device}")
        if self.device.type != "cuda":
            raise NstError("StyleEngine needs a cuda (HIP) device; there is no CPU fallback")
        idx = self.device.index if self.device.index is not None else torch.cuda.current_device()
        self.device = torch.device("cuda", idx)
        if len(weights) != _lib.NST_VGG19_CONVS:
            raise NstError("expected 13 (weight, bias) pairs conv1_1..conv5_1")
        ws = [np.ascontiguousarray(w.detach().cpu().numpy(), dtype=np.float32) for w, _ in weights]
        bs = [np.ascontiguousarray(b.detach().cpu().numpy(), dtype=np.float32) for _, b in weights]
        wp = (C.c_void_p * 13)(*[a.ctypes.data for a in ws])
        bp = (C.c_void_p * 13)(*[a.ctypes.data for a in bs])
        opts = _lib.Options()
        self.lib.nst_options_default(C.byref(opts))
        if conv_mode is not None:
            if conv_mode not in _lib.CONV_MODES:
                raise NstError(f"conv_mode must be one of {sorted(_lib.CONV_MODES)}")
            opts.conv_mode = _lib.CONV_MODES[conv_mode]
        for name, val in (("batched", batched), ("single_stream", single_stream), ("use_graph", use_graph),
                          ("h2_band_rows", h2_band_rows), ("lbfgs_gram", lbfgs_gram), ("h2_mfma16", h2_mfma16),
                          ("h2_wg256", h2_wg256), ("h2_tile_rows", h2_tile_rows),
                          ("gram_overlap", gram_overlap), ("h2_persist", h2_persist), ("level_split", level_split), ("h2_winograd", h2_winograd)):
            if val is not None:
                setattr(opts, name, int(val))
        ctx = C.c_void_p()
        _lib.check(None, self.lib.nst_ctx_create_ex(idx, wp, bp, C.byref(opts), C.byref(ctx)), "nst_ctx_create_ex")
        self.ctx = ctx
        if keep_all_maps is not None:
            _lib.check(self.ctx, self.lib.nst_ctx_set_keep_all_maps(self.ctx, int(bool(keep_all_maps))), "nst_ctx_set_keep_all_maps")
        if forward_pack is not None:
            _lib.check(self.ctx, self.lib.nst_ctx_set_forward_pack(self.ctx, int(bool(forward_pack))), "nst_ctx_set_forward_pack")
        if gram_pack is not None:
            _lib.check(self.ctx, self.lib.nst_ctx_set_gram_pack(self.ctx, int(bool(gram_pack))), "nst_ctx_set_gram_pack")
        self.weights_id = id(weights)
        self.levels = 0
        self.shape = None
        self.taps = DEFAULT_TAPS
        self.channels = 3
        self.pooling = "max"
        self.layer_weights = _style.UNIT_WEIGHTS
        self.laplacian = None
        self.matting = None
        self.gram_shift = None
        self.moment_loss = None

    def close(self):
        if getattr(self, "ctx", None):
            self.lib.nst_ctx_destroy(self.ctx)
            self.ctx = None

    def __del__(self):
        try:
            self.close()
        except Exception:
            pass

    def configure(self, levels_num: int, H0: int, W0: int) -> None:
        _lib.check(self.ctx, self.lib.nst_job_configure(self.ctx, levels_num, H0, W0), "nst_job_configure")
        self.levels = levels_num
        self.shape = (H0, W0)
        for attr, _, _, cleared in _JOB_SETTINGS:
            if cleared:
                setattr(self, attr, None)

    def _set_native(self, attr: str, fn: str, *args) -> None:
        try:
            _lib.check(self.ctx, getattr(self.lib, fn)(self.ctx, *args), fn)
        finally:
            setattr(self, attr, getattr(self, _READER[attr])())

    def reset_job_settings(self) -> None:
        for _, _, reset, _ in _JOB_SETTINGS:
            getattr(self, reset)()

    def set_taps(self, content_index, style_indices, use_relu: bool = True) -> None:
        content, style = _taps.normalize_taps(content_index, style_indices, use_relu)
        _lib.check(self.ctx, self.lib.nst_job_set_taps(self.ctx, content, _taps.style_mask(style), int(use_relu)),
                   "nst_job_set_taps")
        self.taps = (content, style, bool(use_relu))

    def reset_taps(self) -> None:
        if self.taps != DEFAULT_TAPS:
            self.set_taps(*DEFAULT_TAPS)

    def set_color(self, mode) -> None:
        if mode not in (None, "rgb", "luminance"):
            raise ValueError(f"colour mode must be 'rgb' or 'luminance', not {mode!r}")
        self._set_native("channels", "nst_job_set_color", _lib.NST_COLOR_LUMINANCE if mode == "luminance" else _lib.NST_COLOR_RGB)

    def _channels(self) -> int:
        return 1 if self.lib.nst_job_color(self.ctx) == _lib.NST_COLOR_LUMINANCE else 3

    def reset_color(self) -> None:
        if self.channels != 3:
            self.set_color("rgb")

    def set_pooling(self, mode) -> None:
        check_pooling(mode)
        self._set_native("pooling", "nst_job_set_pooling", _lib.NST_POOL_AVG if mode == "avg" else _lib.NST_POOL_MAX)

    def _pooling(self) -> str:
        return "avg" if self.lib.nst_job_pooling(self.ctx) == _lib.NST_POOL_AVG else "max"

    def reset_pooling(self) -> None:
        if self.pooling != "max":
            self.set_pooling("max")

    def set_style_weights(self, w) -> None:
        w = _style.check_style_layer_weights(w, style_indices=self.taps[1])
        self._set_native("layer_weights", "nst_job_set_style_weights", (C.c_float * _style.NUM_MAPS)(*w))

    def style_weights(self) -> Tuple[float, ...]:
        arr = (C.c_float * _style.NUM_MAPS)()
        _lib.check(self.ctx, self.lib.nst_job_style_weights(self.ctx, arr), "nst_job_style_weights")
        return tuple(float(v) for v in arr)

    def reset_style_weights(self) -> None:
        if self.layer_weights != _style.UNIT_WEIGHTS:
            self.set_style_weights(_style.UNIT_WEIGHTS)

    def set_laplacian(self, pools, weights) -> None:
        entries = _lap.normalize_laplacian(weights, pools)
        if entries is None:
            self.reset_laplacian()
            return
        if not self.levels:
            raise NstError("set_laplacian needs a configured job (configure first)")
        _lap.check_levels(entries[0], self.levels, *self.shape)
        k = len(entries[0])
        pool = (C.c_int * k)(*entries[0])
        gamma = (C.c_float * k)(*entries[1])
        self._set_native("laplacian", "nst_job_set_laplacian", k, pool, gamma)

    def laplacian_setting(self):
        k = C.c_int()
        pool = (C.c_int * _lib.NST_MAX_LAPLACIAN)()
        gamma = (C.c_float * _lib.NST_MAX_LAPLACIAN)()
        _lib.check(self.ctx, self.lib.nst_job_laplacian(self.ctx, C.byref(k), pool, gamma), "nst_job_laplacian")
        if k.value == 0:
            return None
        return tuple(int(v) for v in pool[:k.value]), tuple(float(v) for v in gamma[:k.value])

    def reset_laplacian(self) -> None:
        if self.laplacian is not None:
            self._set_native("laplacian", "nst_job_set_laplacian", 0, None, None)

    def laplacian_losses(self) -> torch.Tensor:
        out = torch.empty((self.levels, _lib.NST_MAX_LAPLACIAN), dtype=torch.float32, device=self.device)
        _lib.check(self.ctx, self.lib.nst_job_laplacian_losses(self.ctx, _ptr(out), _stream(self.device)),
                   "nst_job_laplacian_losses")
        return out

    def set_matting(self, gamma, epsilon=_mat.DEFAULT_EPSILON) -> None:
        setting = _mat.normalize_matting(gamma, epsilon)
        if setting is None:
            self.reset_matting()
            return
        if not self.levels:
            raise NstError("set_matting needs a configured job (configure first)")
        _mat.check_levels(self.levels, *self.shape)
        self._set_native("matting", "nst_job_set_matting", setting[0], setting[1])

    def matting_setting(self):
        gamma, eps = C.c_float(), C.c_double()
        _lib.check(self.ctx, self.lib.nst_job_matting(self.ctx, C.byref(gamma), C.byref(eps)), "nst_job_matting")
        return (float(gamma.value), float(eps.value)) if gamma.value > 0 else None

    def reset_matting(self) -> None:
        if self.matting is not None:
            self._set_native("matting", "nst_job_set_matting", 0.0, self.matting[1])

    def matting_losses(self) -> torch.Tensor:
        out = torch.empty((self.levels,), dtype=torch.float32, device=self.device)
        _lib.check(self.ctx, self.lib.nst_job_matting_losses(self.ctx, _ptr(out), _stream(self.device)),
                   "nst_job_matting_losses")
        return out

    def set_gram_shift(self, shift, center_mask: int = 0) -> None:
        setting = _gram.normalize_gram_shift(shift)
        mask = int(center_mask)
        if mask < 0 or mask >> _gram.NUM_MAPS:
            raise ValueError(f"center_mask must be a set of bits 0..{_gram.NUM_MAPS - 1}, got {center_mask!r}")
        if mask:
            s6, m0 = setting if setting is not None else ((0.0,) * _gram.NUM_MAPS, 0)
            if any(s6[i] != 0.0 for i in range(_gram.NUM_MAPS) if (mask >> i) & 1):
                raise ValueError("a centred map takes no constant shift: its entry must be 0")
# ... 1035 lines not shown
```

### include/nst_hip.h

```cpp
#ifndef NST_HIP_H
#define NST_HIP_H

#include <stddef.h>
#include <stdint.h>

#ifdef __cplusplus
extern "C" {
#endif

#define NST_OK 0
#define NST_E_ARG (-1)
#define NST_E_STATE (-2)
#define NST_E_HIP (-3)
#define NST_E_NOMEM (-4)
#define NST_E_UNAVAILABLE (-5)

#define NST_VGG19_CONVS 13
#define NST_MAX_LEVELS 8
#define NST_LOSS_ROW 4
#define NST_MAX_STYLES 8
#define NST_MAX_REGIONS 4
#define NST_MAX_LAPLACIAN 4
#define NST_MAX_FLOW_SCALES 12

// ... 8 lines not shown
int nst_ctx_create(int device, const float* const* weights, const float* const* biases, nst_ctx** out);
void nst_ctx_destroy(nst_ctx* ctx);

#define NST_CONV_F32 0
#define NST_CONV_BF16X3 1
#define NST_CONV_F16X2 2
typedef struct nst_options {
    int struct_size;
    int conv_mode;
    int batched;
    int single_stream;
    int use_graph;
    int h2_band_rows;
    int lbfgs_gram;
    int h2_mfma16;
    int h2_wg256;
    int h2_tile_rows;
    int gram_overlap;
    int h2_persist;
    int level_split;
    int h2_winograd;
} nst_options;
void nst_options_default(nst_options* opts);
int nst_ctx_create_ex(int device, const float* const* weights, const float* const* biases, const nst_options* opts,
                      nst_ctx** out);

int nst_job_configure(nst_ctx* ctx, int levels_num, int H0, int W0);

int nst_job_set_taps(nst_ctx* ctx, int content_index, unsigned style_mask, int use_relu);

#define NST_COLOR_RGB 0
#define NST_COLOR_LUMINANCE 1
int nst_job_set_color(nst_ctx* ctx, int mode);
int nst_job_color(const nst_ctx* ctx);

#define NST_POOL_MAX 0
#define NST_POOL_AVG 1
int nst_job_set_pooling(nst_ctx* ctx, int mode);
int nst_job_pooling(const nst_ctx* ctx);

int nst_job_set_style_weights(nst_ctx* ctx, const float w[6]);
int nst_job_style_weights(const nst_ctx* ctx, float w[6]);

int nst_job_set_laplacian(nst_ctx* ctx, int K, const int* pool, const float* gamma);
int nst_job_laplacian(const nst_ctx* ctx, int* K, int pool[NST_MAX_LAPLACIAN], float gamma[NST_MAX_LAPLACIAN]);
int nst_job_laplacian_losses(nst_ctx* ctx, float* out , void* stream);

int nst_job_set_matting(nst_ctx* ctx, float gamma, double epsilon);
int nst_job_matting(const nst_ctx* ctx, float* gamma, double* epsilon);
int nst_job_matting_losses(nst_ctx* ctx, float* out , void* stream);

int nst_job_set_gram_shift(nst_ctx* ctx, const float shift[6], unsigned center_mask);
int nst_job_gram_shift(const nst_ctx* ctx, float shift[6], unsigned* center_mask);
int nst_level_gram_offsets(nst_ctx* ctx, int level, int slot, float* out, void* stream);
int nst_gram_shifted(nst_ctx* ctx, const float* f, int C, int h, int w, int normalize, int center, float shift, float* gram,
                     float* offset_out , void* stream);

int nst_job_set_moments(nst_ctx* ctx, const float mean_w[6], const float std_w[6], float epsilon);
int nst_job_moments(const nst_ctx* ctx, float mean_w[6], float std_w[6], float* epsilon);
int nst_job_moment_losses(nst_ctx* ctx, float* out , void* stream);
int nst_moments(nst_ctx* ctx, const float* f, int C, int h, int w, float epsilon, float* mean_out, float* std_out, void* stream);

int nst_level_set_targets(nst_ctx* ctx, int level, const float* content, const float* style,
                          int hs, int ws, void* stream);

int nst_level_set_targets_blend(nst_ctx* ctx, int level, const float* content, int K, const float* const* styles,
                                const int* hs, const int* ws, const float* blend , void* stream);

int nst_level_set_guidance(nst_ctx* ctx, int level, int R, const float* planes ,
                           const float* lambda , void* stream);
int nst_level_set_targets_guided(nst_ctx* ctx, int level, const float* content, const float* style, int hs, int ws,
                                 const float* style_planes , void* stream);
int nst_level_guidance(const nst_ctx* ctx, int level, int* R, float lambda[NST_MAX_REGIONS], double mass[5 * NST_MAX_REGIONS]);
int nst_level_guidance_planes(nst_ctx* ctx, int level, int scale, float* out, void* stream);

int nst_level_set_anchor(nst_ctx* ctx, int level, const float* anchor ,
                         const float* weights , float gamma, void* stream);
int nst_level_anchor(const nst_ctx* ctx, int level, float* gamma, int* weighted);
int nst_job_temporal_losses(nst_ctx* ctx, float* out , void* stream);

#define NST_MAX_ANCHOR_SOURCES 8
int nst_anchor_fold(nst_ctx* ctx, int J, const float* const* sources ,
                    const float* const* weights , int C, int h, int w,
                    float* anchor , float* weight ,
                    float* parts , void* stream);

int nst_closure(nst_ctx* ctx, const float* x, float content_weight, float style_weight,
                float tv_weight, float* grad, float* losses, void* stream);

int nst_closure_levels(nst_ctx* ctx, const float* x, float content_weight, float style_weight,
                       float tv_weight, unsigned level_mask, float* grad, float* losses, void* stream);

int nst_closure_forward(nst_ctx* ctx, const float* x, float content_weight, float style_weight, float tv_weight,
                        unsigned level_mask, float* losses, void* stream);
int nst_closure_backward(nst_ctx* ctx, const float* x, float content_weight, float style_weight, float tv_weight,
                         unsigned level_mask, float* grad, void* stream);

#define NST_OPT_ADAM 0
#define NST_OPT_LBFGS 1
int nst_opt_create(nst_ctx* ctx, int kind, float lr_start, int lbfgs_max_eval, nst_opt** out);
void nst_opt_destroy(nst_opt* opt);

typedef struct nst_step_info {
    int closures;
    int total_closures;
    int accepted;
    float loss;
    float lr;
    float t;
    int history;
} nst_step_info;

int nst_opt_step(nst_opt* opt, float* x, float content_weight, float style_weight, float tv_weight,
                 float* losses_host, int closures_capacity, nst_step_info* info, void* stream);

typedef void (*nst_reduce_hook)(void* user);
int nst_opt_shard_levels(nst_opt* opt, unsigned level_mask, float* grad, float* losses, nst_reduce_hook hook,
                         void* user);

int nst_opt_shard_levels_comm(nst_opt* opt, unsigned level_mask, nst_comm* comm);

int nst_opt_history(const nst_opt* opt, int* pairs, int* n_iter);

int nst_opt_set_closure_reuse(nst_opt* opt, int enabled);
int nst_opt_closure_stats(const nst_opt* opt, long* evaluated, long* served);

int nst_opt_set_lazy_backward(nst_opt* opt, int enabled);
int nst_opt_backward_stats(const nst_opt* opt, long* forward_only, long* skipped);

#define NST_COMM_ID_BYTES 128
int nst_comm_unique_id(void* id);
int nst_comm_create(int device, int rank, int world, const void* id, nst_comm** out);
void nst_comm_destroy(nst_comm* comm);
int nst_comm_info(const nst_comm* comm, int* rank, int* world, long* calls, double* bytes);
int nst_comm_allreduce_sum(nst_comm* comm, float* buf, size_t n, void* stream);

int nst_adam_step(nst_ctx* ctx, float* x, const float* g, float* m, float* v, size_t n, int k, double lr, void* stream);
int nst_lbfgs_direction(nst_ctx* ctx, const float* g, const float* const* y, const float* const* s, const float* ro, int m,
                        float h_diag, size_t n, int form, float* d, void* stream);


int nst_vgg_features(nst_ctx* ctx, const float* x, int h, int w, float* const* outs, void* stream);
int nst_vgg_activations(nst_ctx* ctx, const float* x, int h, int w, float* const* outs, void* stream);
int nst_vgg_features_backward(nst_ctx* ctx, const float* x, int h, int w, const float* const* gouts,
                              float* gx, void* stream);
int nst_level_activation(nst_ctx* ctx, int level, int layer, float* out, void* stream);
int nst_job_map_stats(nst_ctx* ctx, int level, unsigned* stored_mask);
int nst_ctx_set_keep_all_maps(nst_ctx* ctx, int enabled);
int nst_ctx_keep_all_maps(const nst_ctx* ctx);
int nst_ctx_set_forward_pack(nst_ctx* ctx, int enabled);
int nst_ctx_forward_pack(const nst_ctx* ctx);
int nst_ctx_set_gram_pack(nst_ctx* ctx, int enabled);
int nst_ctx_gram_pack(const nst_ctx* ctx);
int nst_level_image(nst_ctx* ctx, int level, float* out, void* stream);
int nst_gram(nst_ctx* ctx, const float* f, int C, int h, int w, int normalize, float* gram, void* stream);
int nst_guided_gram_backward(nst_ctx* ctx, const float* f, size_t N, int C, int R, const float* planes, const float* S,
                             const float* addend, const unsigned* relu_bits, float* out, unsigned* amax_slots, void* stream);
int nst_total_variation(nst_ctx* ctx, const float* y, int C, int h, int w, float* value, float* grad,
                        void* stream);
int nst_laplacian_loss(nst_ctx* ctx, const float* y, const float* content, int C, int h, int w, int p, float* value,
                       float* grad , void* stream);
int nst_matting_loss(nst_ctx* ctx, const float* y, const float* guide, int C, int h, int w, double epsilon, float* value,
                     float* grad , void* stream);
int nst_anchor_loss(nst_ctx* ctx, const float* y, const float* anchor, const float* weights , int C, int h, int w,
                    float* value, float* grad , void* stream);
int nst_anchor_geometry(int* blocks, int* block_elems);

int nst_level_set_patches(nst_ctx* ctx, int level, const float* style , int hs, int ws,
                          const float* weights , int stride, double epsilon, void* stream);
int nst_level_patches(const nst_ctx* ctx, int level, float* weights , int* stride, double* epsilon);
int nst_job_patch_losses(nst_ctx* ctx, float* out , void* stream);
int nst_level_patch_matches(nst_ctx* ctx, int level, int map, int* idx_out , void* stream);
int nst_patch_match(nst_ctx* ctx, const float* f, int h, int w, int C, const float* fs, int hs, int ws, int stride, double epsilon,
                    int* idx_out , float* score_out , void* stream);
int nst_patch_term(nst_ctx* ctx, const float* f, int h, int w, int C, const float* fs, int hs, int ws, int stride, const int* idx,
                   float coef, float* value_out , float* grad_out , void* stream);
int nst_warp_bilinear(nst_ctx* ctx, const float* src, const float* flow, int C, int h, int w, float* out,
                      float* valid , void* stream);
int nst_flow_weights(nst_ctx* ctx, const float* fwd, const float* bwd, int h, int w, float* out, void* stream);
int nst_flow_workspace(int h, int w, int scales, size_t* floats, int* scales_used);
int nst_flow_estimate(nst_ctx* ctx, const float* from, const float* to, int h, int w, float alpha, int scales, int warps,
                      int iterations, float* flow , float* workspace, size_t workspace_floats, void* stream);
int nst_flow_reduce(nst_ctx* ctx, const float* in, int h, int w, float* out, void* stream);
int nst_flow_prolong(nst_ctx* ctx, const float* coarse, int h, int w, float* fine, void* stream);
int nst_flow_linearize(nst_ctx* ctx, const float* from, const float* to, const float* flow, int h, int w, float* ix, float* iy,
                       float* rho, void* stream);
int nst_flow_sweeps(nst_ctx* ctx, const float* ix, const float* iy, const float* rho, const float* flow_in, int h, int w,
                    float alpha, int n, float* flow_out, float* scratch , void* stream);
int nst_flow_tvl1_workspace(int h, int w, int scales, size_t* floats, int* scales_used);
int nst_flow_tvl1_estimate(nst_ctx* ctx, const float* from, const float* to, int h, int w, float lambda, float theta, float tau,
                           int scales, int warps, int iterations, float* flow , float* workspace,
                           size_t workspace_floats, void* stream);
int nst_flow_tvl1_iterations(nst_ctx* ctx, const float* ix, const float* iy, const float* rho, const float* flow_in,
                             const float* dual_in, int h, int w, float lambda, float theta, float tau, int n, float* flow_out,
                             float* dual_out, float* scratch , void* stream);
int nst_bicubic_half(nst_ctx* ctx, const float* x, int C, int h, int w, float* y, void* stream);
int nst_bicubic_half_backward(nst_ctx* ctx, const float* gy, int C, int h, int w, float* gx, void* stream);
int nst_prepare_img(nst_ctx* ctx, const float* hwc, int h, int w, float* chw, void* stream);
int nst_unprepare_img(nst_ctx* ctx, const float* chw, int h, int w, float* hwc, void* stream);


int nst_resize_bicubic(nst_ctx* ctx, const float* src, int h, int w, int channels, float* dst, int nh, int nw, void* stream);
int nst_gather_rows(nst_ctx* ctx, const float* src, const long long* perm, size_t rows, int channels, float* dst, void* stream);
int nst_gaussian_mask_accumulate(nst_ctx* ctx, float* acc, const float* src, int h, int w, int channels, double central,
                                 double peripheral, double dispersion, void* stream);
int nst_noise_blend(nst_ctx* ctx, const float* content, const float* noise, int h, int w, int channels, double noise_factor,
                    float* out, void* stream);
int nst_scale(nst_ctx* ctx, const float* src, float alpha, size_t n, float* dst, void* stream);

int nst_color_stats(nst_ctx* ctx, const float* hwc, int h, int w, double* mean, double* cov, void* stream);
int nst_color_transfer_matrix(const double* mean_c, const double* cov_c, const double* mean_s, const double* cov_s, double* A,
                              double* b);
int nst_color_affine(nst_ctx* ctx, const float* src, int h, int w, const double* A, const double* b, float* dst, void* stream);
int nst_luminance(nst_ctx* ctx, const float* hwc, int h, int w, double alpha, double beta, float* out, void* stream);
int nst_luminance_recombine(nst_ctx* ctx, const float* u, const float* content, int h, int w, float* out, void* stream);

int nst_window_sums_count(size_t* count);
int nst_window_begin(nst_ctx* ctx, const float* xs, int row0, int rows, int H0, float* sums, void* stream);
int nst_window_end(nst_ctx* ctx, const float* xs, int row0, int rows, int H0, float content_weight, float style_weight,
                   float tv_weight, float* sums, float* gxs, float* losses, void* stream);

int nst_conv_mode(const nst_ctx* ctx);

int nst_ctx_bytes(const nst_ctx* ctx, size_t* bytes);

int nst_set_timing(nst_ctx* ctx, int enabled);
int nst_last_closure_ms(nst_ctx* ctx, float* ms);
int nst_last_closure_class(nst_ctx* ctx, int cls, float* ms, int* launches, double* flops);
int nst_timing_totals(nst_ctx* ctx, int cls, double* ms, long* launches, double* flops, int reset);
int nst_timing_mfma_flops(nst_ctx* ctx, int cls, double* mfma_flops);
typedef struct nst_launch_info {
    int cls;
    int h, w, cin, cout;
    int layer;
    int h2_rows, h2_bn, h2_ntw, h2_chunk;
    int h2_mfma16;
    int h2_persist;
    int h2_second, h2_unpool;
    int h2_bands;
} nst_launch_info;
int nst_last_closure_launches(nst_ctx* ctx, nst_launch_info* out, int capacity, int* count);
int nst_last_closure_schedule(const nst_ctx* ctx, int* side_forks, int* level_streams, int* graph_replay);
int nst_dump_last_closure(nst_ctx* ctx);

#ifdef __cplusplus
}
#endif
#endif
```

Measured before the change: 485.9 iters/s.

## Stream pre-fragmented conv weights from global into registers, skipping LDS staging

Adds a host-side repack of forward h2 weights into per-lane MFMA fragment order, plus a DIRECT kernel path. For 16-channel-chunk forward launches with NTW=2, this path loads B fragments with buffer loads straight into a register ring and keeps only the activation tile, double-buffered, in LDS. The aim is to remove LDS traffic and barriers for weights, cut LDS footprint to raise occupancy, and overlap weight fetch with MFMAs through explicit scheduling barriers. The costs are a second copy of forward weights in device memory and higher register pressure from the ring. Every wavefront also fetches weights from global/L2 rather than sharing them through LDS.

```diff
diff --git a/artstyletransfer_amd/_lib.py b/artstyletransfer_amd/_lib.py
--- a/artstyletransfer_amd/_lib.py
+++ b/artstyletransfer_amd/_lib.py
@@ -161,6 +161,9 @@
     "nst_ctx_forward_pack": (C.c_int, [c_void]),
     "nst_ctx_set_gram_pack": (C.c_int, [c_void, C.c_int]),
     "nst_ctx_gram_pack": (C.c_int, [c_void]),
+    "nst_ctx_set_h2_direct_weights": (C.c_int, [c_void, C.c_int]),
+    "nst_ctx_h2_direct_weights": (C.c_int, [c_void]),
+    "nst_ctx_h2_direct_launches": (C.c_longlong, [c_void]),
     "nst_level_image": (C.c_int, [c_void, C.c_int, c_void, c_void]),
     "nst_gram": (C.c_int, [c_void, c_void, C.c_int, C.c_int, C.c_int, C.c_int, c_void, c_void]),
     "nst_guided_gram_backward": (C.c_int, [c_void, c_void, C.c_size_t, C.c_int, C.c_int, c_void, c_void, c_void, c_void, c_void,
diff --git a/artstyletransfer_amd/csrc/conv_h2.hip b/artstyletransfer_amd/csrc/conv_h2.hip
--- a/artstyletransfer_amd/csrc/conv_h2.hip
+++ b/artstyletransfer_amd/csrc/conv_h2.hip
@@ -22,6 +22,9 @@
 #endif
 #ifndef NST_H2_WEIGHT_SETS4
 #define NST_H2_WEIGHT_SETS4 1
+#endif
+#ifndef NST_H2_DIRECT_RING
+#define NST_H2_DIRECT_RING 3
 #endif
 #ifndef NST_H2_ABLATE
 #define NST_H2_ABLATE 0
@@ -84,14 +87,14 @@
 
 }
 
-template <int TH, int BN, int NTW, int KC, bool UNPOOL, bool M16, class Tiles>
+template <int TH, int BN, int NTW, int KC, bool UNPOOL, bool M16, bool DIRECT, class Tiles>
 __device__ __forceinline__ void conv_h2_body(const Tiles& tiles, const int slot_seed) {
     static_assert(!M16 || KC == 32, "the 16x16x32 form takes a whole 32-channel chunk per MFMA");
     using C = H2Cfg<TH, BN, NTW, KC>;
     constexpr int ROWB = C::ROWB, WROWB = C::WROWB, QP = C::QP, PIECEB = C::PIECEB, KS = C::KS;
     extern __shared__ __attribute__((aligned(16))) unsigned char smem[];
     unsigned char* ldsB = smem;
-    unsigned char* ldsA = smem + 3 * C::B_BYTES;
+    unsigned char* ldsA = smem + (DIRECT ? 0 : 3 * C::B_BYTES);
 
     const int tid = threadIdx.x;
     const int lane = tid & 63;
@@ -438,6 +441,99 @@
             }
         };
         auto tap_off = [](int t) { return (t / 3) * C::PROWB + (t % 3) * ROWB; };
+
+        if constexpr (DIRECT) {
+            static_assert(KC == 16 && NTW == 2 && !UNPOOL && !M16 && !Tiles::REFETCH, "the 16-channel-chunk forward launches, one tile per workgroup");
+            constexpr int RING = NST_H2_DIRECT_RING;
+            constexpr int NB = (RING % 3 == 0) ? 2 : 4;
+            static_assert((9 * NB) % RING == 0 && RING >= 2, "the ring position of a stage is a constant of the loop body");
+            const int nct = p.Cout >> 5;
+            const __amdgpu_buffer_rsrc_t rsrc_f = __builtin_amdgcn_make_buffer_rsrc(
+                const_cast<void*>(p.wt_h2_frag), 0, (unsigned)((size_t)9 * nch * nct * 2048) * ABL_W, 0x00020000);
+            const unsigned f_voff = (unsigned)(lane * 16 + ((n0 >> 5) + wn * NTW) * 2048);
+            struct BF { f16x8 v[NTW][2]; };
+            struct AF { f16x8 v[2][2]; };
+            auto load_f = [&](BF& f, const int chunk, const int tap) {
+                const int soff = (chunk * 9 + tap) * nct * 2048;
+#pragma unroll
+                for (int nt = 0; nt < NTW; ++nt)
+#pragma unroll
+                    for (int s = 0; s < 2; ++s)
+                        f.v[nt][s] = __builtin_bit_cast(f16x8, __builtin_amdgcn_raw_buffer_load_b128(rsrc_f, f_voff + (nt * 2 + s) * 1024, soff, 0));
+            };
+            auto request_a = [&](AF& f, const unsigned char* abase) {
+#pragma unroll
+                for (int s = 0; s < 2; ++s) {
+                    f.v[0][s] = *reinterpret_cast<const f16x8*>(abase + a_off0 + s * PIECEB);
+                    f.v[1][s] = *reinterpret_cast<const f16x8*>(abase + a_off1 + s * PIECEB);
+                }
+            };
+            auto multiply_d = [&](const AF& a, const BF& w) {
+#pragma unroll
+                for (int mt = 0; mt < 2; ++mt)
+#pragma unroll
+                    for (int nt = 0; nt < NTW; ++nt) {
+                        accx[mt][nt] = __builtin_amdgcn_mfma_f32_32x32x16_f16(a.v[mt][1], w.v[nt][0], accx[mt][nt], 0, 0, 0);
+                        accm[mt][nt] = __builtin_amdgcn_mfma_f32_32x32x16_f16(a.v[mt][0], w.v[nt][0], accm[mt][nt], 0, 0, 0);
+                        accx[mt][nt] = __builtin_amdgcn_mfma_f32_32x32x16_f16(a.v[mt][0], w.v[nt][1], accx[mt][nt], 0, 0, 0);
+                    }
+            };
+            static_assert(C::PROWB - C::PW * ROWB >= PIECEB + 8, "the row pitch leaves a pad to drop unused units into");
+            auto store_a_d = [&](unsigned char* dstA, const f32x4* r, const int i0, const int i1, const int to) {
+#pragma unroll
+                for (int i = i0; i < i1; ++i) {
+                    const int off_v = a_lds_of(i, to);
+                    const int off = off_v >= 0 ? off_v : C::PW * ROWB;
+                    u32x2 hi, lo;
+                    cut2x4(r[i - i0], sa, hi, lo);
+                    *reinterpret_cast<u32x2*>(dstA + off) = hi;
+                    *reinterpret_cast<u32x2*>(dstA + off + PIECEB) = lo;
+                }
+            };
+            BF B[RING];
+            AF A[2];
+            load_a(ra, here, 0, 0, C::A_PER_T, tid);
+#pragma unroll
+            for (int j = 0; j < RING - 1; ++j) load_f(B[j], j / 9, j % 9);
+            store_a_d(ldsA, ra, 0, C::A_PER_T, tid);
+            __syncthreads();
+            request_a(A[0], ldsA + tap_off(0));
+            constexpr int AP = (C::A_PER_T + 1) / 2;
+            for (int c0 = 0; c0 < nch; c0 += NB) {
+                const int to = opaque(tid);
+#pragma unroll
+                for (int j = 0; j < 9 * NB; ++j) {
+                    const int c = c0 + j / 9, t = j % 9;
+                    unsigned char* acur = ldsA + (c & 1) * C::A_BYTES;
+                    unsigned char* anext = ldsA + ((c + 1) & 1) * C::A_BYTES;
+                    const int cn = (c + 1 < nch) ? c + 1 : c;
+                    {
+                        const int ja = j + RING - 1, ca = c0 + ja / 9;
+                        load_f(B[ja % RING], ca < nch ? ca : nch - 1, ja % 9);
+                    }
+                    if (t == 0) load_a(ra, here, cn, 0, AP, to);
+                    if (t == 4) load_a(ra, here, cn, AP, C::A_PER_T, to);
+                    __builtin_amdgcn_sched_barrier(0);
+                    if (t == 3) store_a_d(anext, ra, 0, AP, to);
+                    if (t == 7) store_a_d(anext, ra, AP, C::A_PER_T, to);
+                    if (t < 8) {
+                        request_a(A[(j + 1) & 1], acur + tap_off(t + 1));
+                        multiply_d(A[j & 1], B[j % RING]);
+#pragma unroll
+                        for (int g = 0; g < 4; ++g) {
+                            __builtin_amdgcn_sched_group_barrier(0x008, 1, 0);
+                            __builtin_amdgcn_sched_group_barrier(0x100, 1, 0);
+                        }
+                        __builtin_amdgcn_sched_group_barrier(0x008, 8, 0);
+                    } else {
+                        multiply_d(A[j & 1], B[j % RING]);
+                        __syncthreads();
+                        request_a(A[(j + 1) & 1], anext + tap_off(0));
+                    }
+                }
+            }
+            return;
+        }
 
         if (!primed) {
             u32x4 r0[C::B_PER_T], r1[C::B_PER_T];
@@ -567,12 +663,12 @@
         }
     };
 
-    const bool has_main = p.Cin > 0;
+    const bool has_main = DIRECT || p.Cin > 0;
     float sa1 = 1.f, ia1 = 1.f;
     if (has_main) tensor_scale(p.amax_in, lane, sa1, ia1);
     const float w1_inv = has_main ? p.wt_h2_inv : 1.f;
     const float inv = ia1 * w1_inv;
-    if (p.in2) {
+    if (!DIRECT && p.in2) {
         float sa2, ia2, sw2, iw2;
         tensor_scale(p.amax_in2, lane, sa2, ia2);
         tensor_scale(p.amax_w2, lane, sw2, iw2);
@@ -1085,7 +1181,7 @@
         p.tiles_x = im.tiles_x; p.tiles_y = 0; p.partial = nullptr; p.partial_floats = 0; p.ksplit = 1;
         p.in2 = im.in2; p.Cin2 = b.Cin2; p.wt2_bf = nullptr; p.bits_out = im.bits_out; p.bits_in = im.bits_in;
         p.pool_out = im.pool_out;
-        p.wt_h2 = b.wt_h2; p.wt_h2_inv = b.wt_h2_inv; p.wt2_f32 = im.wt2_f32;
+        p.wt_h2 = b.wt_h2; p.wt_h2_inv = b.wt_h2_inv; p.wt2_f32 = im.wt2_f32; p.wt_h2_frag = b.wt_h2_frag;
         p.amax_in = im.amax_in; p.amax_in2 = im.amax_in2; p.amax_w2 = im.amax_w2; p.amax_out = im.amax_out;
         p.pcode_in = im.pcode_in; p.pcode_out = im.pcode_out; p.pool_avg = b.pool_avg;
         p.in2_row0 = im.in2_row0; p.in2_rows = im.in2_rows; p.ty0 = im.ty0;
@@ -1094,10 +1190,14 @@
     }
 };
 
-template <int TH, int BN, int NTW, int KC, bool UNPOOL, bool M16, bool PERSIST>
+template <int TH, int BN, int NTW, int KC, bool UNPOOL, bool M16, bool PERSIST, bool DIRECT = false>
 __global__ __launch_bounds__((H2Cfg<TH, BN, NTW, KC>::NT), (H2Cfg<TH, BN, NTW, KC>::WAVES_PER_EU)) void conv_h2_batch_kernel(ConvBatch b) {
-    conv_h2_body<TH, BN, NTW, KC, UNPOOL, M16>(H2BatchTiles<PERSIST>{b, b.Cout / BN}, blockIdx.x);
-}
+    conv_h2_body<TH, BN, NTW, KC, UNPOOL, M16, DIRECT>(H2BatchTiles<PERSIST>{b, b.Cout / BN}, blockIdx.x);
+}
+template <int NTW, int KC>
+constexpr bool h2_direct_shape = (KC == 16 && NTW == 2);
+template <int TH, int BN, int NTW, int KC>
+constexpr int h2_direct_lds = 2 * H2Cfg<TH, BN, NTW, KC>::A_BYTES;
 template <int TH, int BN, int NTW, int KC>
 constexpr bool h2_persist_shape = (KC == 16) || (TH == 16 && NTW == 2 && KC == 32);
 template <int NTW, int KC>
@@ -1112,6 +1212,11 @@
         if (e == hipSuccess)
             e = hipFuncSetAttribute(reinterpret_cast<const void*>(&conv_h2_batch_kernel<TH, BN, NTW, KC, UNPOOL, false, true>),
                                     hipFuncAttributeMaxDynamicSharedMemorySize, lds);
+    }
+    if constexpr (h2_direct_shape<NTW, KC> && !M16 && !UNPOOL) {
+        if (e == hipSuccess)
+            e = hipFuncSetAttribute(reinterpret_cast<const void*>(&conv_h2_batch_kernel<TH, BN, NTW, KC, false, false, false, true>),
+                                    hipFuncAttributeMaxDynamicSharedMemorySize, h2_direct_lds<TH, BN, NTW, KC>);
     }
     return e;
 }
@@ -1177,6 +1282,11 @@
     return sh;
 }
 
+static int h2_takes_direct(const ConvBatch& b, const H2Shape& sh) {
+    constexpr int body = ((NST_H2_DIRECT_RING % 3 == 0) ? 2 : 4) * 16;
+    return (sh.chunk == 16 && sh.ntw == 2 && b.wt_h2_frag && !b.unpool && !sh.second && !sh.persist && b.Cin > 0 && b.Cin % body == 0) ? 1 : 0;
+}
+
 template <int TH, int BN, int NTW, int KC>
 static void launch_batch_cfg(const ConvBatch& b, const H2Shape& sh, int blocks, hipStream_t stream) {
     constexpr int lds = H2Cfg<TH, BN, NTW, KC>::LDS_BYTES;
@@ -1185,6 +1295,13 @@
         if (sh.m16) {
             if (b.unpool) hipLaunchKernelGGL((conv_h2_batch_kernel<TH, BN, NTW, KC, true, true, false>), dim3(blocks), dim3(nt), lds, stream, b);
             else hipLaunchKernelGGL((conv_h2_batch_kernel<TH, BN, NTW, KC, false, true, false>), dim3(blocks), dim3(nt), lds, stream, b);
+            return;
+        }
+    }
+    if constexpr (h2_direct_shape<NTW, KC>) {
+        constexpr int lds_direct = h2_direct_lds<TH, BN, NTW, KC>;
+        if (sh.direct) {
+            hipLaunchKernelGGL((conv_h2_batch_kernel<TH, BN, NTW, KC, false, false, false, true>), dim3(blocks), dim3(nt), lds_direct, stream, b);
             return;
         }
     }
@@ -1234,7 +1351,8 @@
         second = second || (im.in2 != nullptr);
     }
     int blocks = 0;
-    const H2Shape sh = h2_launch_shape(H, W, b.n, b.Cin, b.Cout, b.unpool != 0, second, b.tile_rows, b.mfma16, b.wg256, b.persist, &blocks);
+    H2Shape sh = h2_launch_shape(H, W, b.n, b.Cin, b.Cout, b.unpool != 0, second, b.tile_rows, b.mfma16, b.wg256, b.persist, &blocks);
+    sh.direct = h2_takes_direct(b, sh);
     int tiles = 0;
     for (int i = 0; i < b.n; ++i) {
         b.img[i].tiles_x = (b.img[i].W + 15) / 16;
@@ -1272,10 +1390,11 @@
     b.n = 1;
     b.bias = p.bias;
     b.Cin = p.Cin; b.Cout = p.Cout; b.Cin2 = p.Cin2; b.relu = p.relu;
-    b.wt_h2 = p.wt_h2; b.wt_h2_inv = p.wt_h2_inv;
+    b.wt_h2 = p.wt_h2; b.wt_h2_inv = p.wt_h2_inv; b.wt_h2_frag = p.wt_h2_frag;
     b.unpool = (p.pcode_in != nullptr);
     b.persist = 0;
     b.pool_avg = p.pool_avg;
+    sh.direct = h2_takes_direct(b, sh);
     int bands = 0;
     for (int r0 = 0; r0 < p.H; r0 += band_rows) {
         const int r1 = (r0 + band_rows < p.H) ? r0 + band_rows : p.H;
diff --git a/artstyletransfer_amd/csrc/nst_closure.cpp b/artstyletransfer_amd/csrc/nst_closure.cpp
--- a/artstyletransfer_amd/csrc/nst_closure.cpp
+++ b/artstyletransfer_amd/csrc/nst_closure.cpp
@@ -21,6 +21,7 @@
         H2Shape sh{};
         const hipError_t e = launch_conv_h2(p, s, &sh);
         t.shape(sh);
+        ctx->h2_direct_launches += sh.direct ? sh.bands : 0;
         return e;
     }
     hipError_t e = launch_conv_mfma(p, 9, s);
@@ -35,11 +36,13 @@
     return !(p.partial && S > 1 && (size_t)S * p.H * p.W * p.Cout <= p.partial_floats);
 }
 
+static int h2_direct_bit(int l) { return kCout[l] % 128 == 0 ? 2 : 1; }
 void conv_setup(const nst_ctx* ctx, ConvParams& p, const ActSet& a, int l, bool dgrad) {
     p.wt = dgrad ? ctx->wd[l] : ctx->wf[l]; p.wt_bf = dgrad ? ctx->wd_bf[l] : ctx->wf_bf[l];
     p.partial = a.splitk; p.partial_floats = a.splitk_floats;
     if (ctx->conv_mode != 2) return;
     p.wt_h2 = dgrad ? ctx->wd_h2[l] : ctx->wf_h2[l]; p.wt_h2_inv = dgrad ? ctx->wd_h2_inv[l] : ctx->wf_h2_inv[l];
+    p.wt_h2_frag = (!dgrad && (ctx->h2_direct_weights & h2_direct_bit(l))) ? ctx->wf_h2_frag[l] : nullptr;
     p.band_rows = ctx->band_rows; p.mfma16 = ctx->mfma16; p.wg256 = ctx->wg256; p.tile_rows = ctx->tile_rows;
 }
 void conv_setup(const nst_ctx* ctx, ConvBatch& b, int l, bool dgrad) {
@@ -47,6 +50,7 @@
     if (l < 1) { b.wt_h2_inv = 1.f; return; }
     b.wt_bf = dgrad ? ctx->wd_bf[l] : ctx->wf_bf[l];
     b.wt_h2 = dgrad ? ctx->wd_h2[l] : ctx->wf_h2[l]; b.wt_h2_inv = dgrad ? ctx->wd_h2_inv[l] : ctx->wf_h2_inv[l];
+    b.wt_h2_frag = (!dgrad && (ctx->h2_direct_weights & h2_direct_bit(l))) ? ctx->wf_h2_frag[l] : nullptr;
     b.wt_wino = dgrad ? ctx->wd_wino[l] : ctx->wf_wino[l]; b.wt_wino_inv = dgrad ? ctx->wd_wino_inv[l] : ctx->wf_wino_inv[l];
 }
 int launch_conv_batch(nst_ctx* ctx, const ConvBatch& b, hipStream_t s, Timer* t, bool allow_wino) {
@@ -56,6 +60,7 @@
         H2Shape sh{};
         const hipError_t e = launch_conv_h2_batch(b, s, &sh);
         if (t) t->shape(sh);
+        ctx->h2_direct_launches += sh.direct;
         HIPCHK(ctx, e);
     } else HIPCHK(ctx, launch_conv_bf3_batch(b, s));
     return NST_OK;
diff --git a/artstyletransfer_amd/csrc/nst_ctx.cpp b/artstyletransfer_amd/csrc/nst_ctx.cpp
--- a/artstyletransfer_amd/csrc/nst_ctx.cpp
+++ b/artstyletransfer_amd/csrc/nst_ctx.cpp
@@ -154,8 +154,9 @@
     return r;
 }
 
+static int h2_chunk(int rows, int K) { return (rows % 128 == 0 && K > NST_H2_SHORTK_CIN) ? 32 : 16; }
 void make_h2(const float* w, int taps, int rows, int K, std::vector<uint16_t>& out, float* inv) {
-    const int kc = (rows % 128 == 0 && K > NST_H2_SHORTK_CIN) ? 32 : 16;
+    const int kc = h2_chunk(rows, K);
     const size_t n = (size_t)taps * rows * K;
     float mx = 0.f;
     for (size_t i = 0; i < n; ++i) mx = std::max(mx, std::fabs(w[i]));
@@ -174,6 +175,21 @@
                 const size_t base = (((size_t)t * rows + r) * nch + k / kc) * 2 * kc + (k % kc);
                 out[base] = uh; out[base + kc] = ul;
             }
+}
+
+void make_h2_frag(const std::vector<uint16_t>& h2, int rows, int K, std::vector<uint16_t>& out) {
+    const int nch = K / 16, nct = rows / 32;
+    out.assign(h2.size(), 0);
+    for (int ch = 0; ch < nch; ++ch)
+        for (int t = 0; t < 9; ++t)
+            for (int ct = 0; ct < nct; ++ct)
+                for (int s = 0; s < 2; ++s)
+                    for (int lane = 0; lane < 64; ++lane) {
+                        const int r = lane & 31, h = lane >> 5;
+                        const uint16_t* src = h2.data() + ((((size_t)t * rows + ct * 32 + r) * nch + ch) * 2 + s) * 16 + 8 * h;
+                        uint16_t* dst = out.data() + ((((((size_t)ch * 9 + t) * nct + ct) * 2 + s) * 64) + lane) * 8;
+                        for (int j = 0; j < 8; ++j) dst[j] = src[j];
+                    }
 }
 
 void make_wino(const float* w, int rows, int K, std::vector<uint16_t>& out, float* inv) {
@@ -434,6 +450,7 @@
     ctx->keep_all_maps = env_flag("NST_KEEP_ALL_MAPS", 0) ? 1 : 0;
     ctx->forward_pack = env_flag("NST_FORWARD_PACK", 1) ? 1 : 0;
     ctx->gram_pack = env_flag("NST_GRAM_PACK", 1) ? 1 : 0;
+    ctx->h2_direct_weights = env_flag("NST_H2_DIRECT_WEIGHTS", NST_H2_DIRECT_DEFAULT) & 3;
     if (ctx->use_graph && hipStreamCreateWithFlags(&ctx->gstream, hipStreamNonBlocking) != hipSuccess) { ctx->err = "stream creation failed"; return bail(NST_E_HIP); }
     if (e != hipSuccess) { ctx->err = std::string("kernel attribute setup: ") + hipGetErrorString(e); return bail(NST_E_HIP); }
 
@@ -444,7 +461,8 @@
         if (hipMemcpy(dst, src, bytes, hipMemcpyHostToDevice) != hipSuccess) { ctx->err = std::string(what) + " upload failed"; return NST_E_HIP; }
         return NST_OK;
     };
-    auto pieces = [&](int rows, int K, void*& bf, void*& h2, float& h2_inv, void*& wino, float& wino_inv) -> int {
+    std::vector<uint16_t> frag16;
+    auto pieces = [&](int rows, int K, void*& bf, void*& h2, float& h2_inv, void*& wino, float& wino_inv, void** frag) -> int {
         if (ctx->conv_mode == 1) {
             make_bf3(tmp.data(), 9, rows, K, tmp16);
             return upload(bf, tmp16.data(), tmp16.size() * 2, "weight");
@@ -452,6 +470,10 @@
         if (ctx->conv_mode != 2) return NST_OK;
         make_h2(tmp.data(), 9, rows, K, tmp16, &h2_inv);
         NSTCHK(upload(h2, tmp16.data(), tmp16.size() * 2, "weight"));
+        if (frag && h2_chunk(rows, K) == 16 && rows % 64 == 0 && K % 16 == 0) {
+            make_h2_frag(tmp16, rows, K, frag16);
+            NSTCHK(upload(*frag, frag16.data(), frag16.size() * 2, "weight"));
+        }
         if (ctx->winograd && K >= 256 && K % 64 == 0 && rows % 128 == 0) {
             make_wino(tmp.data(), rows, K, tmp16, &wino_inv);
             NSTCHK(upload(wino, tmp16.data(), tmp16.size() * 2, "weight"));
@@ -483,14 +505,14 @@
             for (int o = 0; o < co; ++o)
                 for (int c = 0; c < ci; ++c) tmp[((size_t)t * co + o) * ci + c] = W[((size_t)o * ci + c) * 9 + t];
         if (int r = upload(ctx->wf[l], tmp.data(), n * 4, "weight")) return bail(r);
-        if (int r = pieces(co, ci, ctx->wf_bf[l], ctx->wf_h2[l], ctx->wf_h2_inv[l], ctx->wf_wino[l], ctx->wf_wino_inv[l])) return bail(r);
+        if (int r = pieces(co, ci, ctx->wf_bf[l], ctx->wf_h2[l], ctx->wf_h2_inv[l], ctx->wf_wino[l], ctx->wf_wino_inv[l], &ctx->wf_h2_frag[l])) return bail(r);
         for (int t = 0; t < 9; ++t) {
             const int ky = 2 - t / 3, kx = 2 - t % 3;
             for (int c = 0; c < ci; ++c)
                 for (int o = 0; o < co; ++o) tmp[((size_t)t * ci + c) * co + o] = W[((size_t)o * ci + c) * 9 + ky * 3 + kx];
         }
         if (int r = upload(ctx->wd[l], tmp.data(), n * 4, "weight")) return bail(r);
-        if (int r = pieces(ci, co, ctx->wd_bf[l], ctx->wd_h2[l], ctx->wd_h2_inv[l], ctx->wd_wino[l], ctx->wd_wino_inv[l])) return bail(r);
+        if (int r = pieces(ci, co, ctx->wd_bf[l], ctx->wd_h2[l], ctx->wd_h2_inv[l], ctx->wd_wino[l], ctx->wd_wino_inv[l], nullptr)) return bail(r);
     }
     if (ctx->level_split) ctx->gram_overlap = 0;
     if ((ctx->gram_overlap || ctx->level_split) && ctx->conv_mode == 2 &&
@@ -658,6 +680,17 @@
     return NST_OK;
 }
 int nst_ctx_gram_pack(const nst_ctx* ctx) { return ctx ? ctx->gram_pack : -1; }
+
+int nst_ctx_set_h2_direct_weights(nst_ctx* ctx, int enabled) {
+    NSTCHK(bind(ctx));
+    ++ctx->ws_seq;
+    drop_closure_state(ctx, false);
+    if (enabled < 0 || enabled > 3) return fail(ctx, NST_E_ARG, "h2_direct_weights must be 0 .. 3");
+    ctx->h2_direct_weights = enabled;
+    return NST_OK;
+}
+int nst_ctx_h2_direct_weights(const nst_ctx* ctx) { return ctx ? ctx->h2_direct_weights : -1; }
+long long nst_ctx_h2_direct_launches(const nst_ctx* ctx) { return ctx ? (long long)ctx->h2_direct_launches : -1; }
 
 int nst_job_map_stats(nst_ctx* ctx, int level, unsigned* stored_mask) {
     NSTCHK(bind(ctx));
diff --git a/artstyletransfer_amd/csrc/nst_ctx.h b/artstyletransfer_amd/csrc/nst_ctx.h
--- a/artstyletransfer_amd/csrc/nst_ctx.h
+++ b/artstyletransfer_amd/csrc/nst_ctx.h
@@ -236,6 +236,9 @@
     int keep_all_maps = 0;
     int forward_pack = 1;
     int gram_pack = 1;
+    int h2_direct_weights = NST_H2_DIRECT_DEFAULT;
+    unsigned long long h2_direct_launches = 0;
+    void* wf_h2_frag[nst::NL] = {};
     unsigned long long fwd_pass = 0;
     hipStream_t side = nullptr;
     hipEvent_t side_fork = nullptr, side_join = nullptr;
diff --git a/artstyletransfer_amd/csrc/nst_kernels.h b/artstyletransfer_amd/csrc/nst_kernels.h
--- a/artstyletransfer_amd/csrc/nst_kernels.h
+++ b/artstyletransfer_amd/csrc/nst_kernels.h
@@ -40,8 +40,12 @@
     int wg256;
     int tile_rows;
     int pool_avg;
-};
-
+    const void* wt_h2_frag;
+};
+
+#ifndef NST_H2_DIRECT_DEFAULT
+#define NST_H2_DIRECT_DEFAULT 3
+#endif
 constexpr int NST_AMAX_SLOTS = 64;
 #ifndef NST_H2_SHORTK_CIN_VALUE
 #define NST_H2_SHORTK_CIN_VALUE 128
@@ -86,6 +90,7 @@
     const void* wt_wino;
     float wt_wino_inv;
     int pool_avg;
+    const void* wt_h2_frag;
 };
 
 hipError_t conv_wino_init_device();
@@ -110,6 +115,7 @@
     int persist;
     int second, unpool;
     int bands;
+    int direct;
 };
 hipError_t launch_conv_h2(const ConvParams& p, hipStream_t stream, H2Shape* shape = nullptr);
 hipError_t launch_conv_h2_batch(const ConvBatch& b, hipStream_t stream, H2Shape* shape = nullptr);
diff --git a/artstyletransfer_amd/engine.py b/artstyletransfer_amd/engine.py
--- a/artstyletransfer_amd/engine.py
+++ b/artstyletransfer_amd/engine.py
@@ -77,7 +77,8 @@
                  h2_tile_rows: Optional[int] = None, gram_overlap: Optional[bool] = None,
                  h2_persist: Optional[bool] = None, level_split: Optional[bool] = None,
                  h2_winograd: Optional[bool] = None, keep_all_maps: Optional[bool] = None,
-                 forward_pack: Optional[bool] = None, gram_pack: Optional[bool] = None):
+                 forward_pack: Optional[bool] = None, gram_pack: Optional[bool] = None,
+                 h2_direct_weights: Optional[bool] = None):
         self.lib = _lib.load()
         if not torch.cuda.is_available():
             raise NstError("no GPU visible: the style-transfer hot path runs only on the HIP device")
@@ -113,6 +114,10 @@
             _lib.check(self.ctx, self.lib.nst_ctx_set_forward_pack(self.ctx, int(bool(forward_pack))), "nst_ctx_set_forward_pack")
         if gram_pack is not None:
             _lib.check(self.ctx, self.lib.nst_ctx_set_gram_pack(self.ctx, int(bool(gram_pack))), "nst_ctx_set_gram_pack")
+        if h2_direct_weights is not None:
+            _lib.check(self.ctx, self.lib.nst_ctx_set_h2_direct_weights(
+                self.ctx, 3 if h2_direct_weights is True else int(h2_direct_weights)),
+                       "nst_ctx_set_h2_direct_weights")
         self.weights_id = id(weights)
         self.levels = 0
         self.shape = None
diff --git a/include/nst_hip.h b/include/nst_hip.h
--- a/include/nst_hip.h
+++ b/include/nst_hip.h
@@ -184,6 +184,9 @@
 int nst_ctx_forward_pack(const nst_ctx* ctx);
 int nst_ctx_set_gram_pack(nst_ctx* ctx, int enabled);
 int nst_ctx_gram_pack(const nst_ctx* ctx);
+int nst_ctx_set_h2_direct_weights(nst_ctx* ctx, int enabled);
+int nst_ctx_h2_direct_weights(const nst_ctx* ctx);
+long long nst_ctx_h2_direct_launches(const nst_ctx* ctx);
 int nst_level_image(nst_ctx* ctx, int level, float* out, void* stream);
 int nst_gram(nst_ctx* ctx, const float* f, int C, int h, int w, int normalize, float* gram, void* stream);
 int nst_guided_gram_backward(nst_ctx* ctx, const float* f, size_t N, int C, int R, const float* planes, const float* S,
```

New measurement: 492.9 iters/s, median of 6. 1.01x the previous value.
